# ktncktnc/diffusion-forcing-transformer

Hardware: AMD Instinct MI355X
Metric: denoised latent frames/sec, DFoT RE10K 8f & 200f rollout @1/2/4/8 GPU (higher is better)
Workload: dtype bf16

## Files before the change

### diffusion-forcing-transformer_amd/backbone.py

```python
from __future__ import annotations

import ctypes as C
import math
from typing import Dict, Optional, Sequence, Tuple

import torch
from torch import nn

from . import capi, ops


def _get(cfg, key, default=None):
    if isinstance(cfg, dict):
        return cfg.get(key, default)
    return getattr(cfg, key, default) if not hasattr(cfg, "get") else cfg.get(key, default)


class _Node(nn.Module):
    """Anonymous container so that dotted reference key names map onto a module tree."""


class UViT3DPose(nn.Module):
    def __init__(self, cfg, x_shape: Sequence[int], max_tokens: int, external_cond_dim: int = 0,
                 external_cond_type: str = "action", external_cond_num_classes: Optional[int] = None,
                 use_causal_mask: bool = False, **kwargs):
        super().__init__()
        block_types = list(_get(cfg, "block_types", ["ResBlock", "ResBlock", "TransformerBlock", "TransformerBlock"]))
        if block_types != ["ResBlock", "ResBlock", "TransformerBlock", "TransformerBlock"]:
            raise ValueError(f"unsupported block_types {block_types}")
        if _get(cfg, "pos_emb_type", "rope") != "rope":
            raise ValueError("only pos_emb_type='rope' is supported")
        if not _get(cfg, "use_fourier_noise_embedding", True):
            raise ValueError("only the Fourier noise-level embedding (continuous diffusion) is supported")
        cond = _get(cfg, "conditioning", None)
        cond_dim = _get(cond, "dim", None) if cond is not None else None
        self.cfg = cfg
        self.x_shape = tuple(x_shape)
        self.max_tokens = self.temporal_length = int(max_tokens)
        self.external_cond_dim = int(cond_dim or 180)
        self.use_causal_mask = use_causal_mask
        c = capi.UViTConfig()
        c.channels[:] = list(_get(cfg, "channels"))
        c.emb_channels = int(_get(cfg, "emb_channels"))
        c.num_updown_blocks[:] = list(_get(cfg, "num_updown_blocks"))
        c.num_mid_blocks = int(_get(cfg, "num_mid_blocks"))
        c.num_heads = int(_get(cfg, "num_heads"))
        c.in_channels = int(self.x_shape[0])
        c.resolution = int(self.x_shape[-1])
        c.max_tokens = self.max_tokens
        c.cond_dim = self.external_cond_dim
        c.noise_dim = 256
        c.rope_theta = 10000.0
        c.eps = 1e-6
        if int(_get(cfg, "patch_size", 2)) != 2:
            raise ValueError("only patch_size=2 is supported")
        self._ccfg = c
        self._handle = C.c_void_p()
        capi.check(capi.lib.dfot_uvit_create(C.byref(c), C.byref(self._handle)))
        self._names = []
        self._persistent_buffers = {"noise_level_pos_embedding.timesteps.freqs",
                                    "noise_level_pos_embedding.timesteps.phases"}
        shape = (C.c_int64 * 4)()
        ndim = C.c_int()
        for i in range(capi.lib.dfot_uvit_num_params(self._handle)):
            name = capi.lib.dfot_uvit_param_name(self._handle, i).decode()
            capi.check(capi.lib.dfot_uvit_param_shape(self._handle, i, shape, C.byref(ndim)))
            self._register(name, tuple(shape[k] for k in range(ndim.value)))
            self._names.append(name)
        self._synced: Optional[Tuple] = None
        self._reserved = 0
        self._op_key: Optional[int] = None
        self._cond_key = None
        self._cond_refs = None
        self._cond_gen = None
        self._cond_flag = None
        self.cond_cache_stats = {"builds": 0, "identity_hits": 0, "content_hits": 0}
        self._train_names = None
        self._trainer = None
        self._trainer_sig = None
        self.live_frames = None
        self.fresh_frames = None
        self._fresh_key = None
        self._train_stamp = 0
        self._dropout_generator: Optional[torch.Generator] = None

    def _register(self, name: str, shape: Tuple[int, ...]) -> None:
        *path, leaf = name.split(".")
        node: nn.Module = self
        for part in path:
            if part not in node._modules:
                node.add_module(part, _Node())
            node = node._modules[part]
        t = torch.zeros(shape, dtype=torch.float32)
        if name in self._persistent_buffers:
            node.register_buffer(leaf, t, persistent=True)
        else:
            node.register_parameter(leaf, nn.Parameter(t))

    def _tensors(self) -> Dict[str, torch.Tensor]:
        sd = dict(self.named_parameters())
        sd.update(dict(self.named_buffers()))
        return sd

    def reset_parameters(self, seed: int = 0) -> None:
        g = torch.Generator().manual_seed(seed)
        with torch.no_grad():
            for name, t in self._tensors().items():
                leaf = name.rsplit(".", 1)[-1]
                if leaf == "freqs":
                    t.copy_(2 * math.pi * torch.randn(t.shape, generator=g))
                elif leaf == "phases":
                    t.copy_(2 * math.pi * torch.rand(t.shape, generator=g))
                elif any(s in name for s in (".attn_out.", ".mlp_out.2.", ".out_rest.1.", "project_output")):
                    t.zero_()
                elif leaf == "bias":
                    t.zero_()
                elif t.ndim == 1:
                    t.fill_(1.0)
                else:
                    fan_in = math.prod(t.shape[1:])
                    bound = 1.0 / math.sqrt(fan_in)
                    t.copy_((torch.rand(t.shape, generator=g) * 2 - 1) * bound)

    def _signature(self) -> Tuple:
        return tuple((t.data_ptr(), t._version) for t in self._tensors().values())

    def sync_weights(self, force: bool = False) -> None:
        sig = self._signature()
        if not force and sig == self._synced:
            return
        tensors = self._tensors()
        s = capi.stream_ptr()
        for name in self._names:
            t = tensors[name]
            if not t.is_cuda:
                raise RuntimeError(f"parameter {name} is on {t.device}; move the module to the GPU first")
            src = t.detach().to(torch.float32).contiguous()
            shape = (C.c_int64 * src.ndim)(*src.shape)
            capi.check(capi.lib.dfot_uvit_load_weight(self._handle, name.encode(), capi.ptr(src), shape, src.ndim, s))
        capi.check(capi.lib.dfot_uvit_finalize(self._handle, s))
        self._synced = sig
        self.reserve_generation = getattr(self, "reserve_generation", 0) + 1

    def set_option(self, key: str, value: int) -> None:
        self.reserve_generation = getattr(self, "reserve_generation", 0) + 1
        capi.check(capi.lib.dfot_uvit_set_option(self._handle, key.encode(), int(value)))

    def query(self, key: str) -> float:
        self.sync_weights()
        val = C.c_double()
        capi.check(capi.lib.dfot_uvit_query(self._handle, key.encode(), C.byref(val)))
        return float(val.value)

    def attn_timing(self):
        tot, n = C.c_double(), C.c_int64()
        capi.check(capi.lib.dfot_uvit_attn_timing(self._handle, C.byref(tot), C.byref(n)))
        return tot.value, n.value

    def init_random(self, seed: int = 0, zero_init_scale: float = 0.3) -> None:
        g = torch.Generator().manual_seed(seed)
        with torch.no_grad():
            for name, t in self._tensors().items():
                leaf = name.rsplit(".", 1)[-1]
                if leaf == "freqs":
                    v = 2 * math.pi * torch.randn(t.shape, generator=g)
                elif leaf == "phases":
                    v = 2 * math.pi * torch.rand(t.shape, generator=g)
                elif leaf == "bias":
                    v = 0.02 * torch.randn(t.shape, generator=g)
                elif t.ndim == 1:
                    v = 1.0 + 0.1 * torch.randn(t.shape, generator=g)
                else:
                    fan_in = t.shape[0] if name.startswith("project_output") else math.prod(t.shape[1:])
                    v = torch.randn(t.shape, generator=g) / math.sqrt(fan_in)
                    if any(s in name for s in (".attn_out.", ".mlp_out.2.", ".out_rest.1.", "project_output")):
                        v = v * zero_init_scale
                t.copy_(v.to(t.device))

    def reserve(self, batch: int) -> None:
        if batch > self._reserved:
            torch.cuda.synchronize()
            capi.check(capi.lib.dfot_uvit_reserve(self._handle, int(batch)))
            self._reserved = batch
            self.reserve_generation = getattr(self, "reserve_generation", 0) + 1
            self._cond_key = None

    def forward(self, x: torch.Tensor, noise_levels: torch.Tensor, external_cond: Optional[torch.Tensor] = None,
                external_cond_mask: Optional[torch.Tensor] = None) -> torch.Tensor:
        assert external_cond is not None, "External condition (camera pose) is required for U-ViT3DPose model."
        if self._op_key is None:
            self._op_key = ops.register_model(self)
        if torch.is_grad_enabled() and (x.requires_grad or any(p.requires_grad for p in self.parameters())):
            if self._train_names is None:
                self._train_names = [n for n, _ in self.named_parameters()]
            params = [p for _, p in self.named_parameters()]
            return torch.ops.dfot.uvit3d_pose_forward_train(x, noise_levels, external_cond, external_cond_mask, params, self._op_key)
        return torch.ops.dfot.uvit3d_pose_forward(x, noise_levels, external_cond, external_cond_mask, self._op_key)

    def _train_engine(self, params):
        from . import uvit_train
        sig = tuple((t.data_ptr(), t._version) for t in params) + tuple((b.data_ptr(), b._version) for _, b in self.named_buffers())
        if self._trainer is None:
            cfg = dict(channels=list(self._ccfg.channels), emb_channels=int(self._ccfg.emb_channels), patch_size=2,
                       block_types=["ResBlock", "ResBlock", "TransformerBlock", "TransformerBlock"],
                       num_updown_blocks=list(self._ccfg.num_updown_blocks), num_mid_blocks=int(self._ccfg.num_mid_blocks),
                       num_heads=int(self._ccfg.num_heads), in_channels=int(self._ccfg.in_channels), resolution=int(self._ccfg.resolution),
                       max_tokens=self.max_tokens, cond_dim=self.external_cond_dim, noise_dim=int(self._ccfg.noise_dim),
                       eps=float(self._ccfg.eps), rope_theta=float(self._ccfg.rope_theta),
                       block_dropouts=list(_get(self.cfg, "block_dropouts", [0.0] * 4) or [0.0] * 4))
            sd = {n: t for n, t in zip(self._train_names, params)}
            sd.update(dict(self.named_buffers()))
            ordered = {n: sd[n] for n in self._names}
            self._trainer = uvit_train.UViT3DPoseTrainer(ordered, cfg)
            self._trainer_sig = sig
        elif sig != self._trainer_sig:
            with torch.no_grad():
                for n, t in zip(self._train_names, params):
                    self._trainer.p[n].copy_(t)
                for n, b in self.named_buffers():
                    self._trainer.p[n].copy_(b)
            self._trainer.sync()
            self._trainer_sig = sig
        return self._trainer

    def _train_forward_impl(self, x, noise_levels, external_cond, external_cond_mask, params):
        assert x.shape[1] == self.temporal_length, (
            f"Temporal length of U-ViT is set to {self.temporal_length}, but input has temporal length {x.shape[1]}.")
        dev = params[0].device
        if dev.type != "cuda":
            raise RuntimeError(f"the backbone's parameters are on {dev}; move the module to the GPU first (there is no CPU path)")
        capi.require_device(dev, x=x, noise_levels=noise_levels, external_cond=external_cond, external_cond_mask=external_cond_mask)
        eng = self._train_engine(params)
        drop = external_cond_mask
        pdrop = float(_get(self.cfg, "external_cond_dropout", 0.0) or 0.0)
        if drop is None and self.training and pdrop > 0:
            drop = torch.rand(x.shape[0], device=dev) < pdrop
        eng.dropout_generator = self._dropout_generator if self.training else None
        self._train_stamp += 1
        with torch.no_grad():
            return eng.forward(x, noise_levels, external_cond, drop).to(x.dtype)

    def _train_backward_impl(self, grad_out, params, stamp=None, want_dx=False):
        eng = self._trainer
        if eng is None:
            raise RuntimeError("backward without a training forward")
        if stamp is not None and stamp != self._train_stamp:
            raise RuntimeError(
                f"UViT3DPose: backward of training forward #{stamp}, but forward #{self._train_stamp} has run since and overwritten the "
                "saved activations (one engine per module). Run backward after each forward (accumulate gradients as forward/backward "
                "pairs); two forwards of one module inside one loss are not supported.")
        with torch.no_grad():
            grads = eng.backward(grad_out, input_grad=want_dx)
        out = [grads[n].to(p.dtype).reshape(p.shape) if n in grads else torch.zeros_like(p) for n, p in zip(self._train_names, params)]
        if want_dx:
            out.append(eng.dx_in.to(grad_out.dtype))
        return out

    def _cond_content_equal(self, cond: torch.Tensor, mask: Optional[torch.Tensor]) -> bool:
        if self._cond_key is None or self._cond_refs is None:
            return False
        kept, kept_mask = self._cond_refs
        _, version, shape, synced, mask_key = self._cond_key
        if synced != self._synced or self._cond_gen != self.reserve_generation:
            return False
        if kept._version != version or (kept_mask is not None and kept_mask._version != mask_key[1]):
            return False
        for t in (cond, kept):
            if t.dtype != torch.float32 or not t.is_contiguous():
                return False
        if cond.device != kept.device or tuple(cond.shape) != shape:
            return False
        if (mask is None) != (kept_mask is None):
            return False
        if mask is not None and (mask.dtype != kept_mask.dtype or mask.shape != kept_mask.shape or mask.device != kept_mask.device
                                 or not mask.is_contiguous() or not kept_mask.is_contiguous()):
            return False
        if torch.cuda.is_current_stream_capturing():
            return False
        if self._cond_flag is None or self._cond_flag.device != cond.device:
            self._cond_flag = torch.zeros(1, dtype=torch.int32, device=cond.device)
        flag = self._cond_flag
        flag.zero_()
        s = capi.stream_ptr()
        capi.check(capi.lib.dfot_op_equal_bits(capi.ptr(kept), capi.ptr(cond), cond.numel() * cond.element_size(), capi.ptr(flag), s))
        if mask is not None:
            capi.check(capi.lib.dfot_op_equal_bits(capi.ptr(kept_mask), capi.ptr(mask), mask.numel() * mask.element_size(), capi.ptr(flag), s))
        return int(flag.item()) == 0

    def _forward_impl(self, x: torch.Tensor, noise_levels: torch.Tensor, external_cond: Optional[torch.Tensor] = None,
                      external_cond_mask: Optional[torch.Tensor] = None) -> torch.Tensor:
        assert x.shape[1] == self.temporal_length, (
            f"Temporal length of U-ViT is set to {self.temporal_length}, but input has temporal length {x.shape[1]}.")
        assert external_cond is not None, "External condition (camera pose) is required for U-ViT3DPose model."
        b = x.shape[0]
        if tuple(x.shape[2:]) != self.x_shape:
            raise ValueError(f"x has frame shape {tuple(x.shape[2:])}, expected {self.x_shape}")
        if tuple(external_cond.shape) != (b, self.temporal_length, self.external_cond_dim, *self.x_shape[1:]):
            raise ValueError(f"external_cond has shape {tuple(external_cond.shape)}")
        if external_cond_mask is not None:
            assert external_cond_mask.ndim == 1, "embedding mask should be of shape (B,)"
        if tuple(noise_levels.shape) != (b, self.temporal_length):
            raise ValueError(f"noise_levels has shape {tuple(noise_levels.shape)}, expected {(b, self.temporal_length)}")
        dev = next(self.parameters()).device
        if dev.type != "cuda":
            raise RuntimeError(f"the backbone's parameters are on {dev}; move the module to the GPU first (there is no CPU path)")
        capi.require_device(dev, x=x, noise_levels=noise_levels, external_cond=external_cond, external_cond_mask=external_cond_mask)
        self.sync_weights()
        self.reserve(b)
        xf = x.detach().to(torch.float32).contiguous()
        kf = noise_levels.detach().to(torch.float32).contiguous()
        key = (external_cond.data_ptr(), external_cond._version, tuple(external_cond.shape), self._synced,
               None if external_cond_mask is None else (external_cond_mask.data_ptr(), external_cond_mask._version))
        if key == self._cond_key:
            self.cond_cache_stats["identity_hits"] += 1
        else:
            if self._cond_content_equal(external_cond, external_cond_mask):
                self.cond_cache_stats["content_hits"] += 1
            else:
                cf = external_cond.detach().to(torch.float32).contiguous()
                mf = None if external_cond_mask is None else external_cond_mask.to(torch.uint8).contiguous()
                capi.check(capi.lib.dfot_uvit_set_conditions(self._handle, capi.ptr(cf, torch.float32, "external_cond"),
                                                             capi.ptr(mf, torch.uint8, "external_cond_mask"), b, capi.stream_ptr()))
                self.cond_cache_stats["builds"] += 1
            self._cond_key = key
            self._cond_refs = (external_cond, external_cond_mask)
            self._cond_gen = self.reserve_generation
        out = torch.empty_like(xf)
        live = self.live_frames
        if live is not None:
            if tuple(live.shape) != (b, self.temporal_length) or live.dtype != torch.uint8 or not live.is_contiguous():
                raise ValueError(f"live_frames must be a contiguous uint8 tensor of shape {(b, self.temporal_length)}")
            capi.require_device(dev, live_frames=live)
        fresh = self.fresh_frames
        if fresh is not None:
            if tuple(fresh.shape) != (b, self.temporal_length) or fresh.dtype != torch.uint8 or not fresh.is_contiguous():
                raise ValueError(f"fresh_frames must be a contiguous uint8 tensor of shape {(b, self.temporal_length)}")
            capi.require_device(dev, fresh_frames=fresh)
            if key != self._fresh_key:
                fresh = None
        capi.check(capi.lib.dfot_uvit_forward_cached_masks(self._handle, capi.ptr(xf, torch.float32, "x"),
                                                           capi.ptr(kf, torch.float32, "noise_levels"), capi.ptr(out), b,
                                                           capi.ptr(live, torch.uint8, "live_frames"),
                                                           capi.ptr(fresh, torch.uint8, "fresh_frames"), capi.stream_ptr()))
        self._fresh_key = key
        return out.to(x.dtype)

    def read_tap(self, name: str, channels: int, level: int, batch: int) -> torch.Tensor:
        r = self.x_shape[-1] // 2 // (2 ** level)
        out = torch.empty(batch * self.temporal_length, channels, r, r, device="cuda", dtype=torch.float32)
        capi.check(capi.lib.dfot_uvit_read_tap(self._handle, name.encode(), capi.ptr(out), out.numel(), capi.stream_ptr()))
        return out

    def __del__(self):
        try:
            if getattr(self, "_handle", None) and self._handle.value:
                capi.lib.dfot_uvit_destroy(self._handle)
                self._handle = C.c_void_p()
        except Exception:
            pass
```

### diffusion-forcing-transformer_amd/capi.py

```python
from __future__ import annotations

import ctypes as C
import os

_HERE = os.path.dirname(os.path.abspath(__file__))
LIB_PATH = os.environ.get("DFOT_LIB", os.path.join(_HERE, "libdfot_hip.so"))

OK, ERR_ARG, ERR_SHAPE, ERR_HIP, ERR_STATE, ERR_NAME = range(6)


class DfotError(RuntimeError):
    def __init__(self, code: int, message: str):
        super().__init__(f"libdfot_hip error {code}: {message}")
        self.code = code


class UViTConfig(C.Structure):
    _fields_ = [
        ("channels", C.c_int32 * 4), ("emb_channels", C.c_int32), ("num_updown_blocks", C.c_int32 * 3),
        ("num_mid_blocks", C.c_int32), ("num_heads", C.c_int32), ("in_channels", C.c_int32),
        ("resolution", C.c_int32), ("max_tokens", C.c_int32), ("cond_dim", C.c_int32), ("noise_dim", C.c_int32),
        ("rope_theta", C.c_float), ("eps", C.c_float),
    ]


class DiTConfig(C.Structure):
    _fields_ = [
        ("hidden_size", C.c_int32), ("depth", C.c_int32), ("num_heads", C.c_int32), ("patch_size", C.c_int32),
        ("in_channels", C.c_int32), ("height", C.c_int32), ("width", C.c_int32), ("max_tokens", C.c_int32),
        ("mlp_hidden", C.c_int32), ("noise_dim", C.c_int32), ("timesteps", C.c_int32),
        ("rope_theta", C.c_float), ("eps", C.c_float),
        ("variant", C.c_int32), ("embed_col_dim", C.c_int32), ("num_col_heads", C.c_int32), ("num_row_heads", C.c_int32),
        ("temporal_mlp_hidden", C.c_int32), ("use_bias", C.c_int32),
        ("cond_type", C.c_int32), ("cond_dim", C.c_int32), ("num_classes", C.c_int32), ("cond_dropout", C.c_int32),
        ("use_temporal_rope", C.c_int32),
    ]


COND_NONE, COND_ACTION, COND_LABEL = 0, 1, 2


_P, _I, _L, _F = C.c_void_p, C.c_int, C.c_int64, C.c_float
_I32 = C.c_int32


class GemmDesc(C.Structure):
    _fields_ = [
        ("amode", _I32), ("epi", _I32), ("variant", _I32),
        ("A", _P), ("lda", _L), ("W", _P), ("ldw", _L),
        ("M", _I32), ("N", _I32), ("K", _I32), ("H", _I32), ("Wd", _I32), ("Cin", _I32),
        ("live", _P), ("bias", _P), ("bias_rows", _I32),
        ("out_f32", _P), ("out_bf16", _P), ("ldo", _L),
        ("resid", _P), ("resid_bf", _P),
        ("gate", _P), ("gate_index", _P), ("ldg", _L), ("gate_rows", _I32),
        ("act", _I32), ("pre_act", _P), ("raw", _P), ("ldraw", _L), ("tr_rows", _I32),
        ("gn_part", _P), ("gn_rows_per_bt", _I32), ("gn_cpg", _I32),
        ("out2", _P), ("ldo2", _L), ("split", _I32),
        ("q", _P), ("k", _P), ("v", _P),
        ("qw", _P), ("kw", _P), ("rope_cs", _P),
        ("heads", _I32), ("d", _I32), ("ntok", _I32), ("qscale", _F), ("dstride", _I32), ("eps", _F),
        ("ksplit", _I32), ("slice_stride", _L),
    ]


SIGNATURES = {
    "dfot_last_error": (C.c_char_p, []),
    "dfot_version": (_I, []),
    "dfot_uvit_create": (_I, [C.POINTER(UViTConfig), C.POINTER(_P)]),
    "dfot_uvit_destroy": (_I, [_P]),
    "dfot_uvit_num_params": (_I, [_P]),
    "dfot_uvit_param_name": (C.c_char_p, [_P, _I]),
    "dfot_uvit_param_shape": (_I, [_P, _I, C.POINTER(_L), C.POINTER(_I)]),
    "dfot_uvit_load_weight": (_I, [_P, C.c_char_p, _P, C.POINTER(_L), _I, _P]),
    "dfot_uvit_finalize": (_I, [_P, _P]),
    "dfot_uvit_reserve": (_I, [_P, _I]),
    "dfot_uvit_workspace_bytes": (C.c_size_t, [_P]),
    "dfot_uvit_set_option": (_I, [_P, C.c_char_p, _I]),
    "dfot_uvit_query": (_I, [_P, C.c_char_p, C.POINTER(C.c_double)]),
    "dfot_uvit_attn_timing": (_I, [_P, C.POINTER(C.c_double), C.POINTER(_L)]),
    "dfot_uvit_forward": (_I, [_P, _P, _P, _P, _P, _P, _I, _P]),
    "dfot_uvit_set_conditions": (_I, [_P, _P, _P, _I, _P]),
    "dfot_uvit_forward_cached": (_I, [_P, _P, _P, _P, _I, _P]),
    "dfot_uvit_forward_cached_live": (_I, [_P, _P, _P, _P, _I, _P, _P]),
    "dfot_uvit_forward_cached_masks": (_I, [_P, _P, _P, _P, _I, _P, _P, _P]),
    "dfot_uvit_read_tap": (_I, [_P, C.c_char_p, _P, C.c_size_t, _P]),
    "dfot_dit_create": (_I, [C.POINTER(DiTConfig), C.POINTER(_P)]),
    "dfot_dit_destroy": (_I, [_P]),
    "dfot_dit_num_params": (_I, [_P]),
    "dfot_dit_param_name": (C.c_char_p, [_P, _I]),
    "dfot_dit_param_shape": (_I, [_P, _I, C.POINTER(_L), C.POINTER(_I)]),
    "dfot_dit_load_weight": (_I, [_P, C.c_char_p, _P, C.POINTER(_L), _I, _P]),
    "dfot_dit_finalize": (_I, [_P, _P]),
    "dfot_dit_reserve": (_I, [_P, _I]),
    "dfot_dit_workspace_bytes": (C.c_size_t, [_P]),
    "dfot_dit_set_option": (_I, [_P, C.c_char_p, _I]),
    "dfot_dit_attn_timing": (_I, [_P, C.POINTER(C.c_double), C.POINTER(_L)]),
    "dfot_dit_forward": (_I, [_P, _P, _P, _P, _I, _I, _P]),
    "dfot_dit_forward_cond": (_I, [_P, _P, _P, _P, _P, _P, _P, _I, _I, _P]),
    "dfot_dit_read_tap": (_I, [_P, C.c_char_p, _P, C.c_size_t, _P]),
    "dfot_dit_train_create": (_I, [C.POINTER(DiTConfig), C.POINTER(_P)]),
    "dfot_dit_train_destroy": (_I, [_P]),
    "dfot_dit_train_num_params": (_I, [_P]),
    "dfot_dit_train_param_name": (C.c_char_p, [_P, _I]),
    "dfot_dit_train_param_shape": (_I, [_P, _I, C.POINTER(_L), C.POINTER(_I)]),
    "dfot_dit_train_param_offset": (_L, [_P, _I]),
    "dfot_dit_train_total_numel": (_L, [_P]),
    "dfot_dit_train_workspace_bytes": (C.c_size_t, [_P]),
    "dfot_dit_train_attach": (_I, [_P, _P, _P]),
    "dfot_dit_train_reserve": (_I, [_P, _I]),
    "dfot_dit_train_sync_weights": (_I, [_P, _P]),
    "dfot_dit_train_forward": (_I, [_P, _P, _P, _P, _I, _I, _P]),
    "dfot_dit_train_forward_cond": (_I, [_P, _P, _P, _P, _P, _P, _P, _I, _I, _P]),
    "dfot_dit_train_input_grad": (_I, [_P, _P, _P]),
    "dfot_dit_train_backward": (_I, [_P, _P, _P]),
    "dfot_vloss_grad": (_I, [_P] * 7 + [_I, _I, _L, _I, _P]),
    "dfot_sumsq": (_I, [_P, _L, _P, _P]),
    "dfot_adamw_step": (_I, [_P, _P, _P, _P, _L, _F, _F, _F, _F, _F, _I, _P, _F, _P, _F, _P]),
    "dfot_ray_encode": (_I, [_P, _P, _I, _I, _I, _P]),
    "dfot_ray_encode_normalized": (_I, [_P, _P, _I, _I, _I, _P]),
    "dfot_hg_prepare": (_I, [_P, _P, _P, _P, _P, _I, _I, _I, _L, _P]),
    "dfot_ddim_compose": (_I, [_P] * 11 + [_I, _I, _I, _L, _P]),
    "dfot_ddim_compose_tokw": (_I, [_P] * 11 + [_I, _I, _I, _L, _P]),
    "dfot_ddim_noise": (_I, [_P] * 5 + [_I, _I, _I, _L, _I, _P]),
    "dfot_vpred_loss": (_I, [_P] * 9 + [_I, _I, _L, _P]),
    "dfot_vpred_loss_scratch_floats": (_L, [_I, _I, _L]),
    "dfot_vspace_loss": (_I, [_P] * 9 + [_I, _I, _L, _P]),
    "dfot_op_gemm": (_I, [_P, _I, _P, _P, _P, _I, _I, _I, _I, _P]),
    "dfot_op_conv3x3": (_I, [_P, _P, _P, _P, _I, _I, _I, _I, _I, _I, _P]),
    "dfot_op_gemm_ex": (_I, [C.POINTER(GemmDesc), _P]),
    "dfot_op_gemm_desc_bytes": (_L, []),
    "dfot_op_attention": (_I, [_P, _P, _P, _P, _I, _I, _I, _I, _I, _I, _P]),
    "dfot_op_attention_padded": (_I, [_P, _P, _P, _P, _I, _I, _I, _I, _I, _P]),
    "dfot_op_attention_temporal": (_I, [_P, _P, _P, _P, _I, _I, _I, _I, _I, _I, _P]),
    "dfot_op_matrix_attention_rope": (_I, [_P, _P, _P, _I, _I, _I, _I, _I, _I, _F, _P]),
    "dfot_op_matrix_attention": (_I, [_P, _P, _I, _I, _I, _I, _I, _I, _F, _P]),
    "dfot_op_attention_bwd": (_I, [_P, _P, _P, _P, _P, _I, _P, _P, _P, _I, _I, _I, _I, _P]),
    "dfot_op_conv3x3_bwd": (_I, [_P, _P, _P, _P, _P, _P, _I, _I, _I, _I, _I, _P]),
    "dfot_op_conv3x3_bwd2": (_I, [_P, _P, _P, _P, _P, _P, _P, _I, _I, _I, _I, _I, _P]),
    "dfot_op_gn_silu_bwd": (_I, [_P, _P, _P, _P, _P, _F, _P, _P, _P, _P, _I, _I, _I, _P]),
    "dfot_op_rms_film_bwd": (_I, [_P, _P, _P, _P, _F, _P, _P, _P, _L, _I, _I, _P]),
    "dfot_op_rms_film_bwd_res": (_I, [_P, _P, _P, _P, _F, _P, _P, _P, _P, _P, _L, _I, _P]),
    "dfot_op_qknorm_rope_bwd": (_I, [_P, _I, _P, _P, _P, _P, _P, _P, _F, _P, _I, _P, _P, _L, _I, _I, _I, _P]),
    "dfot_op_wgrad_nt": (_I, [_P, _I, _P, _I, _P, _I, _I, _L, _I, _P]),
    "dfot_op_gemm_bf16": (_I, [_P, _I, _P, _P, _P, _I, _I, _I, _I, _P]),
    "dfot_op_gemm_f32": (_I, [_P, _I, _P, _P, _P, _P, _I, _I, _I, _I, _P]),
    "dfot_op_transpose_bf16": (_I, [_P, _P, _I, _I, _P]),
    "dfot_op_colsum_bf16": (_I, [_P, _I, _P, _L, _I, _P]),
    "dfot_op_rms_film_fwd": (_I, [_P, _P, _P, _F, _P, _L, _I, _P]),
    "dfot_op_qknorm_rope_fwd": (_I, [_P, _I, _P, _P, _P, _F, _F, _P, _P, _P, _L, _I, _I, _I, _P]),
    "dfot_op_fused_proj_train": (_I, [_P, _I, _P, _P, _P, _P, _P, _F, _F, _P, _P, _P, _P, _P, _I, _I, _L, _I, _I, _I, _P]),
    "dfot_op_silu_cols": (_I, [_P, _I, _I, _P, _I, _I, _P, _I, _I, _L, _I, _P]),
    "dfot_op_attention_fwd_lse": (_I, [_P, _P, _P, _P, _I, _P, _I, _I, _I, _I, _P]),
    "dfot_op_attention_fwd_lse_bounded": (_I, [_P, _P, _P, _P, _I, _P, _I, _I, _I, _I, C.c_float, _P, C.c_size_t, _P]),
    "dfot_op_attention_scratch_bytes": (C.c_size_t, [_I, _I, _I, _I]),
    "dfot_op_attention_bwd_lse": (_I, [_P, _P, _P, _P, _P, _I, _P, _P, _P, _P, _P, _I, _I, _I, _I, _P]),
    "dfot_op_gn_silu_fwd": (_I, [_P, _P, _P, _P, _F, _P, _P, _I, _I, _I, _P]),
    "dfot_op_gn_silu_bwd5": (_I, [_P, _P, _P, _P, _P, _P, _P, _P, _P, _P, _L, _P, _P, _I, _I, _I, _P]),
    "dfot_op_gn_silu_fwd2": (_I, [_P, _P, _P, _P, _L, _F, _P, _P, _I, _I, _I, _P]),
    "dfot_op_gn_silu_bwd6": (_I, [_P, _P, _P, _P, _P, _P, _L, _P, _P, _P, _P, _L, _P, _P, _I, _I, _I, _P]),
    "dfot_op_gemm_bf16_frame_bias": (_I, [_P, _I, _P, _P, _I, _P, _I, _I, _I, _I, _P]),
    "dfot_op_split_bf16": (_I, [_P, _P, _P, _L, _P]),
    "dfot_op_frame_sums_bf16": (_I, [_P, _L, _P, _I, _I, _I, _P]),
    "dfot_op_sgemm": (_I, [_P, _L, _L, _P, _L, _L, _P, _L, _I, _I, _I, _I, _P]),
    "dfot_op_pack_conv3": (_I, [_P, _P, _I, _I, _I, _P]),
    "dfot_op_conv3x3_f32": (_I, [_P, _P, _P, _P, _P, _I, _I, _I, _I, _I, _P]),
    "dfot_op_pool2_bf16": (_I, [_P, _P, _I, _I, _I, _I, _P]),
    "dfot_op_pool2_bwd": (_I, [_P, _P, _I, _I, _I, _I, _P]),
    "dfot_op_sub_bf16": (_I, [_P, _P, _P, _L, _P]),
    "dfot_op_upsample_add": (_I, [_P, _P, _P, _I, _I, _I, _I, _P]),
    "dfot_op_upsample_bwd": (_I, [_P, _P, _I, _I, _I, _I, _P]),
    "dfot_op_axpy": (_I, [_P, _P, _F, _L, _P]),
    "dfot_op_mul_cols": (_I, [_P, _I, _I, _P, _L, _I, _P]),
    "dfot_op_emb_pyramid": (_I, [_P, _P, _P, _P, _I, _I, _I, _P]),
    "dfot_op_cond_repack": (_I, [_P, _P, _I, _I, _I, _I, _P]),
    "dfot_op_embed_input": (_I, [_P, _P, _P, _P, _I, _I, _I, _I, _P]),
    "dfot_op_embed_input_wgrad": (_I, [_P, _P, _P, _P, _I, _I, _I, _I, _I, _P]),
    "dfot_op_embed_input_dgrad": (_I, [_P, _P, _P, _I, _I, _I, _I, _I, _P]),
    "dfot_op_project_output": (_I, [_P, _P, _P, _P, _I, _I, _I, _I, _P]),
    "dfot_op_outgrad_gather": (_I, [_P, _P, _I, _I, _I, _I, _P]),
    "dfot_op_groupnorm_scratch_floats": (_L, [_I, _I]),
    "dfot_op_groupnorm": (_I, [_P, _P, _P, _F, _P, _P, _I, _I, _I, _I, _P]),
    "dfot_op_frame_shift": (_I, [_P, _P, _I, _I, _L, _I, _P]),
    "dfot_op_upsample3d": (_I, [_P, _P, _I, _I, _I, _I, _I, _I, _P]),
    "dfot_op_softmax_rows": (_I, [_P, _P, _L, _I, _F, _P]),
    "dfot_op_conv3t_f32": (_I, [_P, _P, _P, _P, _P] + [_I] * 9 + [_P]),
    "dfot_op_vae_pixels": (_I, [_P, _L, _L, _L, _L, _L, _F, _F, _P, _I, _I, _I, _I, _P]),
    "dfot_op_vae_posterior": (_I, [_P, _I, _P, _P, _P, _P, _P, _P, _P, _I, _I, _I, _I, _P]),
    "dfot_op_f32_to_bf16": (_I, [_P, _P, _L, _P]),
    "dfot_op_bf16_to_f32": (_I, [_P, _P, _L, _P]),
    "dfot_op_equal_bits": (_I, [_P, _P, _L, _P, _P]),
}


def _load() -> C.CDLL:
    import torch
    if not os.path.exists(LIB_PATH):
        raise ImportError(
            f"{LIB_PATH} is missing: the HIP extension has not been built. There is no CPU fallback; "
            "run `python -c 'import __graft_entry__ as g; g.build()'` (needs hipcc).")
    lib = C.CDLL(LIB_PATH)
    for name, (res, args) in SIGNATURES.items():
        fn = getattr(lib, name)
        fn.restype, fn.argtypes = res, args
    return lib


lib = _load()


def check(code: int) -> None:
    if code != OK:
        raise DfotError(code, (lib.dfot_last_error() or b"").decode())


def ptr(t, dtype=None, name: str = "tensor") -> C.c_void_p:
    if t is None:
        return C.c_void_p(0)
    if not t.is_cuda:
        raise ValueError(f"{name} is on {t.device}: libdfot_hip takes GPU memory only (there is no CPU path)")
    if not t.is_contiguous():
        raise ValueError(f"{name} with shape {tuple(t.shape)} and strides {tuple(t.stride())} is not contiguous")
    if dtype is not None and t.dtype != dtype:
        raise ValueError(f"{name} has dtype {t.dtype}, expected {dtype}")
    return C.c_void_p(t.data_ptr())


def ptr_rows(t, dtype=None, name: str = "tensor") -> C.c_void_p:
    if t is None:
        return C.c_void_p(0)
    if not t.is_cuda:
        raise ValueError(f"{name} is on {t.device}: libdfot_hip takes GPU memory only (there is no CPU path)")
    if t.dim() != 2 or t.stride(1) != 1 or t.stride(0) < t.shape[1]:
        raise ValueError(f"{name} with shape {tuple(t.shape)} and strides {tuple(t.stride())} is not a row-strided matrix")
    if dtype is not None and t.dtype != dtype:
        raise ValueError(f"{name} has dtype {t.dtype}, expected {dtype}")
    return C.c_void_p(t.data_ptr())

# ... 11 lines not shown
```

### diffusion-forcing-transformer_amd/csrc/kernels.h

```cpp
#pragma once
#include "common.h"

namespace dfot {

int launch_noise_emb(const float* k, const float* freqs, const float* phases, const float* w1, const float* b1,
                     const float* w2, const float* b2, float* hidden, float* out, int bt, int ndim, int e, hipStream_t s);
int launch_embed_input(const float* x, const float* w, const float* b, float* out, int bt, int res, int cin, int c0,
                       hipStream_t s);
int launch_cond_repack(const float* cond, bf16* a, int bt, int res, int cdim, int kpad, hipStream_t s);
int launch_emb_pyramid(const bf16* emb0, bf16* emb1, bf16* emb2, bf16* emb3, int bt, int r0, int e, hipStream_t s);
int launch_project_output(const float* x0, const float* w, const float* b, float* out, int bt, int res, int c0, int cout,
                          hipStream_t s, const uint8_t* live = nullptr);
int launch_gn_partial_f32(const float* x, float* partial, int bt, int pixels, int c, hipStream_t s);
int launch_gn_partial_bf16(const bf16* x, float* partial, int bt, int pixels, int c, hipStream_t s);
int launch_gn_finalize(const float* partial, float* stats, int bt, int nblk, int pixels, int c, float eps, hipStream_t s);
int gn_partial_blocks(int pixels);
int launch_gn_apply_silu(const float* x, const float* stats, const float* gamma, const float* beta, bf16* out, int bt,
                         int pixels, int c, hipStream_t s, const uint8_t* live = nullptr);
struct FilmChunk {
  const bf16* w;
  const float* b;
  long out_off;
  int rows;
};
int launch_film_vec(const FilmChunk* table, int chunks, const float* nemb, float* sv, int bt, int e, hipStream_t s);
int launch_gn_film_silu(const bf16* h, const float* stats, const float* gamma, const float* beta, const bf16* fcache,
                        const float* sv, const uint8_t* cond_mask, bf16* out, int bt, int pixels, int c, int tokens,
                        hipStream_t s, const uint8_t* live = nullptr);
struct RmsPending {
  void* x;
  const float* bias;
  const float* s0;
  const float* s1;
  const float* s2;
};
int launch_rms_film(const float* x, const float* w, const bf16* fcache, const float* sv, const uint8_t* cond_mask, bf16* out,
                    long m, int c, int rows_per_bt, int tokens, float eps, hipStream_t s, const RmsPending* pend = nullptr);
int launch_rms_film_bf16(const bf16* x, const float* w, const bf16* fcache, const float* sv, const uint8_t* cond_mask, bf16* out,
                         long m, int c, int rows_per_bt, int tokens, float eps, hipStream_t s, const RmsPending* pend = nullptr);

int launch_pool2_bf16(const float* x, bf16* out, int bt, int h, int w, int c, hipStream_t s);
int launch_pool2_bf16_bf16in(const bf16* x, bf16* out, int bt, int h, int w, int c, hipStream_t s);
int launch_sub_bf16_bf16in(const bf16* a, const float* b, bf16* out, long n, hipStream_t s, const uint8_t* live = nullptr, long frame_elems = 0);
int launch_upsample_add_bf16(const float* t, const bf16* skip, bf16* out, int bt, int h, int w, int c, hipStream_t s, const uint8_t* live = nullptr);
int launch_gn_apply_silu_bf16in(const bf16* x, const float* stats, const float* gamma, const float* beta, bf16* out, int bt, int pixels, int c,
                                hipStream_t s, const uint8_t* live = nullptr);
int launch_embed_input_bf16(const float* x, const float* w, const float* b, bf16* out, int bt, int res, int cin, int c0, hipStream_t s);
int launch_project_output_bf16(const bf16* x0, const float* w, const float* b, float* out, int bt, int res, int c0, int cout, hipStream_t s,
                               const uint8_t* live = nullptr);
int launch_sub_bf16(const float* a, const float* b, bf16* out, long n, hipStream_t s, const uint8_t* live = nullptr, long frame_elems = 0);
int launch_upsample_add(const float* t, const float* skip, float* out, int bt, int h, int w, int c, hipStream_t s, const uint8_t* live = nullptr);
int launch_ray_encode(const float* poses, float* out, int b, int t, int res, int normalized, hipStream_t s);
int launch_hg_prepare(const float* x, const float* noise, const float* qa, const float* qb, float* x_in, int batch,
                      int nfe, int tokens, long f, hipStream_t s);
int launch_ddim_compose(const float* x, const float* x_in, const float* v, const float* sa, const float* s1,
                        const float* an, const float* cn, const float* keep, const float* weight, const uint8_t* gen,
                        float* x_next, int batch, int nfe, int tokens, long f, bool weight_per_token, hipStream_t s);
int launch_ddim_noise(const float* noise, const float* sigma, const float* weight, const uint8_t* gen, float* x_next, int batch, int nfe,
                      int tokens, long f, bool weight_per_token, hipStream_t s);
int vloss_chunks(long f);
int launch_vloss(const float* x, const float* noise, const float* v, const float* a, const float* sg, const float* w,
                 float* x_pred, float* partial, float* loss, int bt, long f, bool vspace, hipStream_t s);
int launch_wgrad_nt(const bf16* a, long lda, const bf16* b, long ldb, float* out, int m, int n, long rows, int slices, hipStream_t s, int img_h = 0,
                    int img_w = 0, int sdy = 0, int sdx = 0, int all_taps = 0);
struct WgradPlan {
  int form, slices;
};
WgradPlan wgrad_plan(int m, int n, long rows, long max_slices);
int launch_wgrad_conv_taps(const bf16* dy, const bf16* x, float* out, int co, int ci, long pix, int slices, int img_h, int img_w, hipStream_t s);
int wgrad_conv_tiles(int co, int ci, int* target);
int launch_wgrad_nt_plan(const bf16* a, long lda, const bf16* b, long ldb, float* out, int m, int n, long rows, WgradPlan plan, hipStream_t s);
int launch_vloss_grad(const float* x, const float* noise, const float* v, const float* a, const float* sg, const float* coef, float* dv,
                      int bt, long f, bool vspace, hipStream_t s);
int launch_sumsq(const float* x, long n, float* out, hipStream_t s);
int launch_adamw(float* p, const float* g, float* m, float* v, long n, float lr, float b1, float b2, float eps, float wd, int step,
                 const float* sumsq, float max_norm, float* ema, float ema_decay, hipStream_t s);
int launch_f32_to_bf16(const float* src, bf16* dst, long n, hipStream_t s);
int launch_bf16_to_f32(const bf16* src, float* dst, long n, hipStream_t s);
int launch_equal_bits(const void* a, const void* b, long bytes, int* differs, hipStream_t s);
int launch_pack_rows(const float* src, bf16* dst, const int* map, int rows, int k, int kpad, long ldd, int col0,
                     hipStream_t s);
int launch_pack_conv3(const float* src, bf16* dst, int co, int ci, hipStream_t s);
int launch_gather_f32(const float* src, float* dst, const int* map, int n, hipStream_t s);
int launch_nhwc_to_nchw(const float* src, float* dst, int bt, int p, int c, hipStream_t s);
int launch_bf16_nhwc_to_nchw(const bf16* src, float* dst, int bt, int p, int c, hipStream_t s);

struct AttnScratch {
  float* p = nullptr;
  size_t bytes = 0;
};
int launch_attention(const bf16* q, const bf16* k, const bf16* v, bf16* o, long ldo, int batch, int heads, int n, int d,
                     int variant, hipStream_t stream, AttnScratch* scratch = nullptr);
int launch_attention_v3(const bf16* q, const bf16* k, const bf16* v, bf16* o, long ldo, int batch, int heads, int n, bool nomax,
                        hipStream_t stream, AttnScratch* scratch = nullptr);
bool attention_v5_applies(int n, int d, float score_bound);
int launch_attention_v5(const bf16* q, const bf16* k, const bf16* v, bf16* o, long ldo, int batch, int heads, int n, hipStream_t stream,
                        AttnScratch* scratch = nullptr, float* lse = nullptr);
bool attention_ks_applies(int batch, int heads, int n, int d);
size_t attention_ks_scratch_bytes(int batch, int heads, int n, int d);
int launch_attention_ks(const bf16* q, const bf16* k, const bf16* v, bf16* o, long ldo, int batch, int heads, int n, hipStream_t stream,
                        AttnScratch* scratch = nullptr);
int attention_dstride(int d);
int launch_attention_padded(const bf16* q, const bf16* k, const bf16* v, bf16* o, long ldo, int batch, int heads, int n, int d,
                            hipStream_t stream, float* lse = nullptr);
int launch_attention_temporal(const bf16* q, const bf16* k, const bf16* v, bf16* o, long ldo, int batch, int tokens, int patches, int heads,
                              int d, hipStream_t s);
int launch_matrix_attn_rope(const bf16* z, bf16* o, const float* rope_cs, int batch, int L, int E, int h, int cc, int rr, float scale,
                            hipStream_t s);
struct AttnSplit {
  int tiles, full, rem, nsplit;
  int slots;
};
AttnSplit attn_plan_split(int batch, int heads, int n, int qrows, int wgs_per_cu);
size_t attn_partial_bytes(const AttnSplit& sp, int qrows, int dcols);
size_t attention_scratch_bytes(int batch, int heads, int n, int d);
int attn_partials(const AttnSplit& sp, int qrows, int dcols, float** po, float** pml, AttnScratch* scratch);
int attn_launch_merge(const AttnSplit& sp, int qrows, int dcols, const float* po, const float* pml, bf16* o, long ldo, int n, int heads,
                      hipStream_t stream, float* lse = nullptr);
int launch_attention_bwd_delta(const bf16* o, const bf16* d_o, long ldo, float* delta, int batch, int heads, int n, int d, hipStream_t s);
int launch_attention_bwd(const bf16* q, const bf16* k, const bf16* v, const bf16* d_o, long ldo, const float* l2, const float* delta,
                         bf16* dq, bf16* dk, bf16* dv, int batch, int heads, int n, int d, hipStream_t s);

}
```

### diffusion-forcing-transformer_amd/csrc/kernels.hip

```cpp
#include "kernels.h"
#include "dfot_hip.h"

namespace dfot {

typedef __attribute__((ext_vector_type(4))) float float4v;
typedef __attribute__((ext_vector_type(2))) float float2v;

__device__ __forceinline__ float wave_sum(float v) {
#pragma unroll
  for (int o = 32; o > 0; o >>= 1) v += __shfl_xor(v, o);
  return v;
}

template <bool FOURIER>
__global__ __launch_bounds__(256) void noise_mlp_kernel(const float* __restrict__ in, const float* __restrict__ freqs,
                                                        const float* __restrict__ phases, const float* __restrict__ w,
                                                        const float* __restrict__ b, float* __restrict__ out, int kdim,
                                                        int e) {
  const int lane = threadIdx.x & 63, wave = threadIdx.x >> 6;
  const int row = blockIdx.x * 4 + wave;
  const int bt = blockIdx.y;
  if (row >= e) return;
  float acc = 0.f;
  for (int i = lane; i < kdim; i += 64) {
    float f;
    if constexpr (FOURIER) {
      f = cosf(__fadd_rn(__fmul_rn(in[bt], freqs[i]), phases[i])) * 1.41421356237309515f;
    } else {
      f = in[(long)bt * kdim + i];
    }
    acc += w[(long)row * kdim + i] * f;
  }
  acc = wave_sum(acc);
  if (lane == 0) out[(long)bt * e + row] = FOURIER ? silu_f(acc + b[row]) : acc + b[row];
}

int launch_noise_emb(const float* k, const float* freqs, const float* phases, const float* w1, const float* b1,
                     const float* w2, const float* b2, float* hidden, float* out, int bt, int ndim, int e, hipStream_t s) {
  hipLaunchKernelGGL(noise_mlp_kernel<true>, dim3(cdiv(e, 4), bt), dim3(256), 0, s, k, freqs, phases, w1, b1, hidden, ndim, e);
  DFOT_CHECK_HIP(hipGetLastError());
  hipLaunchKernelGGL(noise_mlp_kernel<false>, dim3(cdiv(e, 4), bt), dim3(256), 0, s, hidden, nullptr, nullptr, w2, b2, out, e, e);
  DFOT_CHECK_HIP(hipGetLastError());
  return DFOT_OK;
}

template <typename T>
__device__ __forceinline__ void stream_ld8(const T* p, float (&v)[8]) {
  if constexpr (sizeof(T) == 4) {
    const float4v a = *reinterpret_cast<const float4v*>(p), b = *reinterpret_cast<const float4v*>(p + 4);
#pragma unroll
    for (int j = 0; j < 4; ++j) { v[j] = a[j]; v[4 + j] = b[j]; }
  } else {
    const bf16x8 a = *reinterpret_cast<const bf16x8*>(p);
#pragma unroll
    for (int j = 0; j < 8; ++j) v[j] = bf2f(a[j]);
  }
}
template <typename T>
__device__ __forceinline__ float4v stream_ld4(const T* p) {
  if constexpr (sizeof(T) == 4) {
    return *reinterpret_cast<const float4v*>(p);
  } else {
    const bf16x4 a = *reinterpret_cast<const bf16x4*>(p);
    return float4v{bf2f(a[0]), bf2f(a[1]), bf2f(a[2]), bf2f(a[3])};
  }
}
template <typename T>
__device__ __forceinline__ void stream_st8(T* p, const float (&v)[8]) {
  if constexpr (sizeof(T) == 4) {
    *reinterpret_cast<float4v*>(p) = float4v{v[0], v[1], v[2], v[3]};
    *reinterpret_cast<float4v*>(p + 4) = float4v{v[4], v[5], v[6], v[7]};
  } else {
    bf16x8 o;
#pragma unroll
    for (int j = 0; j < 8; ++j) o[j] = f2bf(v[j]);
    *reinterpret_cast<bf16x8*>(p) = o;
  }
}
template <typename T>
__device__ __forceinline__ void stream_st4(T* p, float4v v) {
  if constexpr (sizeof(T) == 4) {
    *reinterpret_cast<float4v*>(p) = v;
  } else {
    *reinterpret_cast<bf16x4*>(p) = bf16x4{f2bf(v[0]), f2bf(v[1]), f2bf(v[2]), f2bf(v[3])};
  }
}

__global__ __launch_bounds__(256) void embed_input_kernel(const float* __restrict__ x, const float* __restrict__ w,
                                                          const float* __restrict__ b, float* __restrict__ out, long total4,
                                                          int res, int cin, int c0) {
  extern __shared__ float wt[];
  const int taps = cin * 4;
  for (int i = threadIdx.x; i < taps * c0; i += blockDim.x) {
    const int c = i % c0, t = i / c0;
    wt[i] = w[(long)c * taps + t];
  }
  __syncthreads();
  const long idx = (long)blockIdx.x * blockDim.x + threadIdx.x;
  if (idx >= total4) return;
  const unsigned q = c0 / 4, r0 = res / 2, iu = (unsigned)idx;
  const int c4 = (int)(iu % q) * 4;
  const unsigned pix = iu / q;
  const int px = (int)(pix % r0), py = (int)((pix / r0) % r0);
  const long bt = pix / (r0 * r0);
  float4v acc = *reinterpret_cast<const float4v*>(b + c4);
  for (int ci = 0; ci < cin; ++ci) {
    const float* xp = x + ((bt * cin + ci) * res + 2 * py) * (long)res + 2 * px;
    const float2v top = *reinterpret_cast<const float2v*>(xp);
    const float2v bot = *reinterpret_cast<const float2v*>(xp + res);
    const float* wp = wt + (ci * 4) * c0 + c4;
    acc += *reinterpret_cast<const float4v*>(wp) * top[0] + *reinterpret_cast<const float4v*>(wp + c0) * top[1] +
           *reinterpret_cast<const float4v*>(wp + 2 * c0) * bot[0] + *reinterpret_cast<const float4v*>(wp + 3 * c0) * bot[1];
  }
  *reinterpret_cast<float4v*>(out + (long)pix * c0 + c4) = acc;
}

template <int CIN, typename TOUT>
__global__ __launch_bounds__(256) void embed_input_reg_kernel(const float* __restrict__ x, const float* __restrict__ w,
                                                              const float* __restrict__ b, TOUT* __restrict__ out, unsigned total4,
                                                              int res, int c0) {
  constexpr int TAPS = CIN * 4;
  const unsigned q = c0 / 4, r0 = res / 2;
  const unsigned nthreads = gridDim.x * 256u;
  unsigned iu = blockIdx.x * 256u + threadIdx.x;
  const int c4 = (int)(iu % q) * 4;
  float4v wt[TAPS];
#pragma unroll
  for (int t = 0; t < TAPS; ++t)
#pragma unroll
    for (int j = 0; j < 4; ++j) wt[t][j] = w[(long)(c4 + j) * TAPS + t];
  const float4v bias = *reinterpret_cast<const float4v*>(b + c4);
  for (; iu < total4; iu += nthreads) {
    const unsigned pix = iu / q;
    const int px = (int)(pix % r0), py = (int)((pix / r0) % r0);
    const long bt = pix / (r0 * r0);
    float4v acc = bias;
#pragma unroll
    for (int ci = 0; ci < CIN; ++ci) {
      const float* xp = x + ((bt * CIN + ci) * res + 2 * py) * (long)res + 2 * px;
      const float2v top = *reinterpret_cast<const float2v*>(xp);
      const float2v bot = *reinterpret_cast<const float2v*>(xp + res);
      acc += wt[ci * 4] * top[0] + wt[ci * 4 + 1] * top[1] + wt[ci * 4 + 2] * bot[0] + wt[ci * 4 + 3] * bot[1];
    }
    stream_st4(out + (long)pix * c0 + c4, acc);
  }
}

int launch_embed_input(const float* x, const float* w, const float* b, float* out, int bt, int res, int cin, int c0,
                       hipStream_t s) {
  DFOT_REQUIRE(c0 % 4 == 0 && res % 2 == 0, DFOT_ERR_SHAPE, "embed_input: channels %d / resolution %d unsupported", c0, res);
  const long total4 = (long)bt * (res / 2) * (res / 2) * (c0 / 4);
  DFOT_REQUIRE(total4 < (1L << 31), DFOT_ERR_SHAPE, "embed_input: %ld work items exceed the 32-bit index range", total4);
  if (cin == 3 && 256 % (c0 / 4) == 0) {
    const long wgs = cdiv(total4, 256);
    hipLaunchKernelGGL((embed_input_reg_kernel<3, float>), dim3((unsigned)(wgs < 4096 ? wgs : 4096)), dim3(256), 0, s, x, w, b, out, (unsigned)total4, res, c0);
    DFOT_CHECK_HIP(hipGetLastError());
    return DFOT_OK;
  }
  hipLaunchKernelGGL(embed_input_kernel, dim3(cdiv(total4, 256)), dim3(256), (size_t)cin * 4 * c0 * sizeof(float), s, x, w, b,
                     out, total4, res, cin, c0);
  DFOT_CHECK_HIP(hipGetLastError());
  return DFOT_OK;
}
int launch_embed_input_bf16(const float* x, const float* w, const float* b, bf16* out, int bt, int res, int cin, int c0, hipStream_t s) {
  DFOT_REQUIRE(c0 % 4 == 0 && res % 2 == 0 && cin == 3 && 256 % (c0 / 4) == 0, DFOT_ERR_SHAPE,
               "embed_input (bf16 stream): %d input channels / %d channels / resolution %d unsupported", cin, c0, res);
  const long total4 = (long)bt * (res / 2) * (res / 2) * (c0 / 4);
  DFOT_REQUIRE(total4 < (1L << 31), DFOT_ERR_SHAPE, "embed_input: %ld work items exceed the 32-bit index range", total4);
  const long wgs = cdiv(total4, 256);
  hipLaunchKernelGGL((embed_input_reg_kernel<3, bf16>), dim3((unsigned)(wgs < 4096 ? wgs : 4096)), dim3(256), 0, s, x, w, b, out, (unsigned)total4, res, c0);
  DFOT_CHECK_HIP(hipGetLastError());
  return DFOT_OK;
}

constexpr int RP_CC = 20;
__global__ __launch_bounds__(256) void cond_repack_kernel(const float* __restrict__ cond, bf16* __restrict__ a, int res,
                                                          int cdim, int kpad) {
  extern __shared__ __attribute__((aligned(16))) bf16 tile[];
  const int r0 = res / 2;
  constexpr int ld = RP_CC * 4 + 4;
  const int chunk = blockIdx.x, py = blockIdx.y, bt = blockIdx.z;
  const int c0 = chunk * RP_CC;
  const int xq = res / 4;
  for (int e = threadIdx.x; e < RP_CC * 2 * xq; e += blockDim.x) {
    const int x4 = e % xq;
    const int dy = (e / xq) & 1;
    const int cc = e / (2 * xq);
    const float4v v = *reinterpret_cast<const float4v*>(cond + (((long)bt * cdim + c0 + cc) * res + 2 * py + dy) * res + x4 * 4);
    typedef __attribute__((ext_vector_type(2))) __bf16 bf16x2;
    bf16x2 lo, hi;
    lo[0] = f2bf(v[0]); lo[1] = f2bf(v[1]); hi[0] = f2bf(v[2]); hi[1] = f2bf(v[3]);
// ... 235 lines not shown

__global__ __launch_bounds__(256) void gn_finalize_kernel(const float* __restrict__ partial, float* __restrict__ stats,
                                                          int nblk, float inv_count, float eps) {
  const int bt = blockIdx.x >> 2, g = (blockIdx.x & 3) * 8 + (threadIdx.x >> 5), part = threadIdx.x & 31;
  float s = 0.f, ss = 0.f;
  for (int b = part; b < nblk; b += 32) {
    const float2 v = *reinterpret_cast<const float2*>(partial + (((long)bt * nblk + b) * 32 + g) * 2);
    s += v.x;
    ss += v.y;
  }
#pragma unroll
  for (int o = 1; o < 32; o <<= 1) {
    s += __shfl_xor(s, o);
    ss += __shfl_xor(ss, o);
  }
  if (part == 0) {
    const float mean = s * inv_count;
    const float var = fmaxf(ss * inv_count - mean * mean, 0.f);
    stats[(bt * 32 + g) * 2 + 0] = mean;
    stats[(bt * 32 + g) * 2 + 1] = rsqrtf(var + eps);
  }
}

int launch_gn_finalize(const float* partial, float* stats, int bt, int nblk, int pixels, int c, float eps, hipStream_t s) {
  const float inv = 1.f / ((float)pixels * (float)(c / 32));
  hipLaunchKernelGGL(gn_finalize_kernel, dim3(bt * 4), dim3(256), 0, s, partial, stats, nblk, inv, eps);
  DFOT_CHECK_HIP(hipGetLastError());
  return DFOT_OK;
}

template <typename T>
static int launch_gn_partial_t(const T* x, float* partial, int bt, int pixels, int c, hipStream_t s) {
  DFOT_REQUIRE(c == 128 || c == 256 || c == 512 || c == 1024, DFOT_ERR_SHAPE, "group_norm: channels %d not in {128,256,512,1024}", c);
  hipLaunchKernelGGL(gn_partial_kernel<T>, dim3(gn_partial_blocks(pixels), bt), dim3(256), 0, s, x, partial, pixels, c);
  DFOT_CHECK_HIP(hipGetLastError());
  return DFOT_OK;
}
int launch_gn_partial_f32(const float* x, float* partial, int bt, int pixels, int c, hipStream_t s) {
  return launch_gn_partial_t<float>(x, partial, bt, pixels, c, s);
}
int launch_gn_partial_bf16(const bf16* x, float* partial, int bt, int pixels, int c, hipStream_t s) {
  return launch_gn_partial_t<bf16>(x, partial, bt, pixels, c, s);
}

__global__ void gn_apply_silu_kernel(const float* __restrict__ x, const float* __restrict__ stats,
                                     const float* __restrict__ gamma, const float* __restrict__ beta,
                                     bf16* __restrict__ out, long total8, int pixels, int c, const uint8_t* __restrict__ live) {
  const long idx = (long)blockIdx.x * blockDim.x + threadIdx.x;
  if (idx >= total8) return;
  const unsigned iu = (unsigned)idx, cq = (unsigned)(c / 8);
  const int c8 = (int)(iu % cq);
  const long pix = iu / cq;
  const int bt = (int)((unsigned)pix / (unsigned)pixels);
  if (live && !live[bt]) return;
  const int cpg = c / 32;
  const float* src = x + pix * c + c8 * 8;
  const float4v a = *reinterpret_cast<const float4v*>(src);
  const float4v b = *reinterpret_cast<const float4v*>(src + 4);
  float v[8] = {a[0], a[1], a[2], a[3], b[0], b[1], b[2], b[3]};
  bf16x8 o;
#pragma unroll
  for (int j = 0; j < 8; ++j) {
    const int ch = c8 * 8 + j;
    const int g = ch / cpg;
    const float mean = stats[(bt * 32 + g) * 2], rs = stats[(bt * 32 + g) * 2 + 1];
    const float y = (v[j] - mean) * rs * gamma[ch] + beta[ch];
    o[j] = f2bf(silu_f(y));
  }
  *reinterpret_cast<bf16x8*>(out + pix * c + c8 * 8) = o;
}

constexpr int GN_ROWS_IT = 8;
template <int C>
struct GnRowConsts {
  float mean[8], rsg[8], gam[8], bet[8];
  __device__ __forceinline__ void load(const float* __restrict__ stats, const float* __restrict__ gamma, const float* __restrict__ beta, int bt,
                                       int c0) {
    constexpr int CPG = C / 32;
    const float4v g0 = *reinterpret_cast<const float4v*>(gamma + c0), g1 = *reinterpret_cast<const float4v*>(gamma + c0 + 4);
    const float4v b0 = *reinterpret_cast<const float4v*>(beta + c0), b1 = *reinterpret_cast<const float4v*>(beta + c0 + 4);
    const float* st = stats + ((long)bt * 32 + c0 / CPG) * 2;
    float m0, r0, m1, r1;
    if constexpr (CPG == 4) {
      const float4v t = *reinterpret_cast<const float4v*>(st);
      m0 = t[0], r0 = t[1], m1 = t[2], r1 = t[3];
    } else {
      m0 = m1 = st[0];
      r0 = r1 = st[1];
    }
#pragma unroll
    for (int j = 0; j < 8; ++j) {
      mean[j] = j < 4 ? m0 : m1;
      rsg[j] = j < 4 ? r0 : r1;
      gam[j] = j < 4 ? g0[j] : g1[j - 4];
      bet[j] = j < 4 ? b0[j] : b1[j - 4];
    }
  }
  __device__ __forceinline__ float norm(float v, int j) const { return (v - mean[j]) * rsg[j] * gam[j] + bet[j]; }
};

template <int C, typename TIN>
__global__ __launch_bounds__(256) void gn_apply_silu_rows_kernel(const TIN* __restrict__ x, const float* __restrict__ stats,
                                                                 const float* __restrict__ gamma, const float* __restrict__ beta,
                                                                 bf16* __restrict__ out, int pixels, const uint8_t* __restrict__ live) {
  constexpr int TPP = C / 8, PPI = 256 / TPP;
  const int wg_per_bt = pixels / (PPI * GN_ROWS_IT);
  const int bt = blockIdx.x / wg_per_bt;
  if (live && !live[bt]) return;
  const int c0 = (threadIdx.x % TPP) * 8;
  GnRowConsts<C> k;
  k.load(stats, gamma, beta, bt, c0);
  long pix = (long)bt * pixels + (long)(blockIdx.x % wg_per_bt) * (PPI * GN_ROWS_IT) + threadIdx.x / TPP;
#pragma unroll 4
  for (int it = 0; it < GN_ROWS_IT; ++it, pix += PPI) {
    float v[8];
    stream_ld8(x + pix * C + c0, v);
    bf16x8 o;
#pragma unroll
    for (int j = 0; j < 8; ++j) o[j] = f2bf(silu_f(k.norm(v[j], j)));
    *reinterpret_cast<bf16x8*>(out + pix * C + c0) = o;
  }
}

int launch_gn_apply_silu_bf16in(const bf16* x, const float* stats, const float* gamma, const float* beta, bf16* out, int bt, int pixels, int c,
                                hipStream_t s, const uint8_t* live) {
  DFOT_REQUIRE((c == 128 || c == 256) && pixels % ((256 / (c / 8)) * GN_ROWS_IT) == 0, DFOT_ERR_SHAPE,
               "groupnorm apply (bf16 stream): %d channels / %d pixels per frame unsupported", c, pixels);
  const int grid = bt * (pixels / ((256 / (c / 8)) * GN_ROWS_IT));
  if (c == 128) hipLaunchKernelGGL((gn_apply_silu_rows_kernel<128, bf16>), dim3(grid), dim3(256), 0, s, x, stats, gamma, beta, out, pixels, live);
  else hipLaunchKernelGGL((gn_apply_silu_rows_kernel<256, bf16>), dim3(grid), dim3(256), 0, s, x, stats, gamma, beta, out, pixels, live);
  DFOT_CHECK_HIP(hipGetLastError());
  return DFOT_OK;
}

int launch_gn_apply_silu(const float* x, const float* stats, const float* gamma, const float* beta, bf16* out, int bt,
                         int pixels, int c, hipStream_t s, const uint8_t* live) {
  if ((c == 128 || c == 256) && pixels % ((256 / (c / 8)) * GN_ROWS_IT) == 0) {
    const int grid = bt * (pixels / ((256 / (c / 8)) * GN_ROWS_IT));
    if (c == 128) hipLaunchKernelGGL((gn_apply_silu_rows_kernel<128, float>), dim3(grid), dim3(256), 0, s, x, stats, gamma, beta, out, pixels, live);
    else hipLaunchKernelGGL((gn_apply_silu_rows_kernel<256, float>), dim3(grid), dim3(256), 0, s, x, stats, gamma, beta, out, pixels, live);
    DFOT_CHECK_HIP(hipGetLastError());
    return DFOT_OK;
  }
  const long total8 = (long)bt * pixels * (c / 8);
  DFOT_REQUIRE(total8 < (1L << 31), DFOT_ERR_SHAPE, "groupnorm apply: %ld work items exceed the 32-bit index range", total8);
  hipLaunchKernelGGL(gn_apply_silu_kernel, dim3(cdiv(total8, 256)), dim3(256), 0, s, x, stats, gamma, beta, out, total8,
                     pixels, c, live);
  DFOT_CHECK_HIP(hipGetLastError());
  return DFOT_OK;
}


__global__ __launch_bounds__(256) void film_vec_kernel(const FilmChunk* __restrict__ table, const float* __restrict__ nemb,
                                                       float* __restrict__ sv, int e, int nbt) {
  const FilmChunk ck = table[blockIdx.x >> 4];
  const int lane = threadIdx.x & 63, wave = threadIdx.x >> 6;
  const int r = (blockIdx.x & 15) * 4 + wave;
  const bf16* wr = ck.w + (long)r * e;
  float wv[2][8];
#pragma unroll
  for (int k = 0; k < 2; ++k) {
    const int i = lane * 8 + k * 512;
    if (i < e) {
      const bf16x8 t = *reinterpret_cast<const bf16x8*>(wr + i);
#pragma unroll
      for (int j = 0; j < 8; ++j) wv[k][j] = bf2f(t[j]);
    } else {
#pragma unroll
      for (int j = 0; j < 8; ++j) wv[k][j] = 0.f;
    }
  }
  const float bias = ck.b[r];
  for (int bt = 0; bt < nbt; ++bt) {
    const float* ne = nemb + (long)bt * e;
    float acc = 0.f;
#pragma unroll
    for (int k = 0; k < 2; ++k) {
      const int i = lane * 8 + k * 512;
      if (i < e) {
        const float4v a = *reinterpret_cast<const float4v*>(ne + i);
        const float4v b = *reinterpret_cast<const float4v*>(ne + i + 4);
        acc += wv[k][0] * a[0] + wv[k][1] * a[1] + wv[k][2] * a[2] + wv[k][3] * a[3] + wv[k][4] * b[0] + wv[k][5] * b[1] +
               wv[k][6] * b[2] + wv[k][7] * b[3];
      }
    }
    acc = wave_sum(acc);
    if (lane == 0) sv[ck.out_off + (long)bt * ck.rows + r] = acc + bias;
  }
}
template <int EQ>
__global__ __launch_bounds__(256, 2) void film_vec_lds_kernel(const FilmChunk* __restrict__ table, const float* __restrict__ nemb,
                                                           float* __restrict__ sv, int nbt) {
  constexpr int E = EQ * 256;
  __shared__ float4v ne[16][E / 4];
  const FilmChunk ck = table[blockIdx.x >> 1];
  const int lane = threadIdx.x & 63, wave = threadIdx.x >> 6;
  for (int bt0 = 0; bt0 < nbt; bt0 += 16) {
    __syncthreads();
    for (int i = threadIdx.x; i < 16 * (E / 4); i += 256) {
      const int f = i / (E / 4);
      float4v v = {0.f, 0.f, 0.f, 0.f};
      if (bt0 + f < nbt) v = reinterpret_cast<const float4v*>(nemb + (long)(bt0 + f) * E)[i % (E / 4)];
      ne[f][i % (E / 4)] = v;
    }
    __syncthreads();
#pragma unroll 1
    for (int pass = 0; pass < 4; ++pass) {
      const int r0 = (blockIdx.x & 1) * 32 + pass * 8 + wave * 2;
      float wv[2][EQ][4];
#pragma unroll
      for (int r = 0; r < 2; ++r)
#pragma unroll
        for (int k = 0; k < EQ; ++k) {
          const bf16x4 t = *reinterpret_cast<const bf16x4*>(ck.w + (long)(r0 + r) * E + k * 256 + lane * 4);
#pragma unroll
          for (int j = 0; j < 4; ++j) wv[r][k][j] = bf2f(t[j]);
        }
      float acc[32];
#pragma unroll
      for (int f = 0; f < 16; ++f) {
        float4v x[EQ];
#pragma unroll
        for (int k = 0; k < EQ; ++k) x[k] = ne[f][k * 64 + lane];
#pragma unroll
        for (int r = 0; r < 2; ++r) {
          float a = 0.f;
#pragma unroll
          for (int k = 0; k < EQ; ++k) a += wv[r][k][0] * x[k][0] + wv[r][k][1] * x[k][1] + wv[r][k][2] * x[k][2] + wv[r][k][3] * x[k][3];
          acc[r * 16 + f] = a;
        }
        if ((f & 3) == 3) __builtin_amdgcn_sched_barrier(0);
      }
      halve_exchange<16, 32>(acc, lane);
      halve_exchange<8, 16>(acc, lane);
      halve_exchange<4, 8>(acc, lane);
      halve_exchange<2, 4>(acc, lane);
      halve_exchange<1, 2>(acc, lane);
      const float v = acc[0] + __shfl_xor(acc[0], 1);
      const int r = r0 + (lane >> 5), f = bt0 + ((lane >> 1) & 15);
      if (f < nbt && (lane & 1) == 0) sv[ck.out_off + (long)f * ck.rows + r] = v + ck.b[r];
    }
  }
}
int launch_film_vec(const FilmChunk* table, int chunks, const float* nemb, float* sv, int bt, int e, hipStream_t s) {
  DFOT_REQUIRE(e % 8 == 0 && e <= 1024, DFOT_ERR_SHAPE, "film_vec: emb dim %d must be a multiple of 8 and <= 1024", e);
  if (e == 1024 || e == 512) {
    if (e == 1024) hipLaunchKernelGGL(film_vec_lds_kernel<4>, dim3(chunks * 2), dim3(256), 0, s, table, nemb, sv, bt);
    else hipLaunchKernelGGL(film_vec_lds_kernel<2>, dim3(chunks * 2), dim3(256), 0, s, table, nemb, sv, bt);
    DFOT_CHECK_HIP(hipGetLastError());
    return DFOT_OK;
  }
  hipLaunchKernelGGL(film_vec_kernel, dim3(chunks * 16), dim3(256), 0, s, table, nemb, sv, e, bt);
  DFOT_CHECK_HIP(hipGetLastError());
  return DFOT_OK;
}

__global__ void gn_film_silu_kernel(const bf16* __restrict__ h, const float* __restrict__ stats,
                                    const float* __restrict__ gamma, const float* __restrict__ beta,
                                    const bf16* __restrict__ fcache, const float* __restrict__ sv,
                                    const uint8_t* __restrict__ cond_mask, bf16* __restrict__ out, long total8, int pixels,
                                    int c, int tokens, const uint8_t* __restrict__ live) {
  const long idx = (long)blockIdx.x * blockDim.x + threadIdx.x;
  if (idx >= total8) return;
  const unsigned iu = (unsigned)idx, cq = (unsigned)(c / 8);
  const int c8 = (int)(iu % cq);
  const long pix = iu / cq;
  const int bt = (int)((unsigned)pix / (unsigned)pixels);
  if (live && !live[bt]) return;
  const int cpg = c / 32;
  const int c0 = c8 * 8;
  const int col = (c0 >> 5) * 64 + (c0 & 31);
  const bf16x8 hv = *reinterpret_cast<const bf16x8*>(h + pix * c + c0);
  const float* svp = sv + (long)bt * 2 * c + col;
  float sc[8], sh[8];
#pragma unroll
  for (int j = 0; j < 8; ++j) {
    sc[j] = svp[j];
    sh[j] = svp[32 + j];
  }
  const bool use_pose = !(cond_mask && cond_mask[(unsigned)bt / (unsigned)tokens]);
  if (use_pose) {
    const bf16x8 fs = *reinterpret_cast<const bf16x8*>(fcache + pix * 2 * c + col);
    const bf16x8 fh = *reinterpret_cast<const bf16x8*>(fcache + pix * 2 * c + col + 32);
#pragma unroll
    for (int j = 0; j < 8; ++j) {
      sc[j] += bf2f(fs[j]);
      sh[j] += bf2f(fh[j]);
    }
  }
  bf16x8 o;
#pragma unroll
  for (int j = 0; j < 8; ++j) {
    const int ch = c0 + j;
    const int g = ch / cpg;
    const float mean = stats[(bt * 32 + g) * 2], rs = stats[(bt * 32 + g) * 2 + 1];
    const float y = ((bf2f(hv[j]) - mean) * rs * gamma[ch] + beta[ch]) * (1.f + sc[j]) + sh[j];
    o[j] = f2bf(silu_f(y));
  }
  *reinterpret_cast<bf16x8*>(out + pix * c + c0) = o;
}
template <int C>
__global__ __launch_bounds__(256) void gn_film_silu_rows_kernel(const bf16* __restrict__ h, const float* __restrict__ stats,
                                                                const float* __restrict__ gamma, const float* __restrict__ beta,
                                                                const bf16* __restrict__ fcache, const float* __restrict__ sv,
                                                                const uint8_t* __restrict__ cond_mask, bf16* __restrict__ out, int pixels,
                                                                int tokens, const uint8_t* __restrict__ live) {
  constexpr int TPP = C / 8, PPI = 256 / TPP;
  const int wg_per_bt = pixels / (PPI * GN_ROWS_IT);
  const int bt = blockIdx.x / wg_per_bt;
  if (live && !live[bt]) return;
  const int c0 = (threadIdx.x % TPP) * 8;
  const int col = (c0 >> 5) * 64 + (c0 & 31);
  GnRowConsts<C> k;
  k.load(stats, gamma, beta, bt, c0);
  const float* svp = sv + (long)bt * 2 * C + col;
  float svs[8], svh[8];
  {
    const float4v s0 = *reinterpret_cast<const float4v*>(svp), s1 = *reinterpret_cast<const float4v*>(svp + 4);
    const float4v h0 = *reinterpret_cast<const float4v*>(svp + 32), h1 = *reinterpret_cast<const float4v*>(svp + 36);
#pragma unroll
    for (int j = 0; j < 8; ++j) {
      svs[j] = j < 4 ? s0[j] : s1[j - 4];
      svh[j] = j < 4 ? h0[j] : h1[j - 4];
    }
  }
  const bool use_pose = !(cond_mask && cond_mask[(unsigned)bt / (unsigned)tokens]);
  long pix = (long)bt * pixels + (long)(blockIdx.x % wg_per_bt) * (PPI * GN_ROWS_IT) + threadIdx.x / TPP;
  if (use_pose) {
#pragma unroll 4
    for (int it = 0; it < GN_ROWS_IT; ++it, pix += PPI) {
      const bf16x8 hv = *reinterpret_cast<const bf16x8*>(h + pix * C + c0);
      const bf16x8 fs = *reinterpret_cast<const bf16x8*>(fcache + pix * 2 * C + col);
      const bf16x8 fh = *reinterpret_cast<const bf16x8*>(fcache + pix * 2 * C + col + 32);
      bf16x8 o;
#pragma unroll
      for (int j = 0; j < 8; ++j) {
        const float sc = svs[j] + bf2f(fs[j]), sh = svh[j] + bf2f(fh[j]);
        o[j] = f2bf(silu_f(k.norm(bf2f(hv[j]), j) * (1.f + sc) + sh));
      }
      *reinterpret_cast<bf16x8*>(out + pix * C + c0) = o;
    }
  } else {
#pragma unroll 4
    for (int it = 0; it < GN_ROWS_IT; ++it, pix += PPI) {
      const bf16x8 hv = *reinterpret_cast<const bf16x8*>(h + pix * C + c0);
      bf16x8 o;
#pragma unroll
      for (int j = 0; j < 8; ++j) o[j] = f2bf(silu_f(k.norm(bf2f(hv[j]), j) * (1.f + svs[j]) + svh[j]));
      *reinterpret_cast<bf16x8*>(out + pix * C + c0) = o;
    }
  }
}

int launch_gn_film_silu(const bf16* h, const float* stats, const float* gamma, const float* beta, const bf16* fcache,
                        const float* sv, const uint8_t* cond_mask, bf16* out, int bt, int pixels, int c, int tokens,
                        hipStream_t s, const uint8_t* live) {
  if ((c == 128 || c == 256) && pixels % ((256 / (c / 8)) * GN_ROWS_IT) == 0) {
    const int grid = bt * (pixels / ((256 / (c / 8)) * GN_ROWS_IT));
    if (c == 128)
      hipLaunchKernelGGL(gn_film_silu_rows_kernel<128>, dim3(grid), dim3(256), 0, s, h, stats, gamma, beta, fcache, sv, cond_mask, out, pixels, tokens, live);
    else
      hipLaunchKernelGGL(gn_film_silu_rows_kernel<256>, dim3(grid), dim3(256), 0, s, h, stats, gamma, beta, fcache, sv, cond_mask, out, pixels, tokens, live);
    DFOT_CHECK_HIP(hipGetLastError());
    return DFOT_OK;
  }
  const long total8 = (long)bt * pixels * (c / 8);
  DFOT_REQUIRE(total8 < (1L << 31), DFOT_ERR_SHAPE, "groupnorm apply: %ld work items exceed the 32-bit index range", total8);
  hipLaunchKernelGGL(gn_film_silu_kernel, dim3(cdiv(total8, 256)), dim3(256), 0, s, h, stats, gamma, beta, fcache, sv,
                     cond_mask, out, total8, pixels, c, tokens, live);
  DFOT_CHECK_HIP(hipGetLastError());
  return DFOT_OK;
}

template <int MAXCH, bool PEND, typename TS>
__global__ __launch_bounds__(256) void rms_film_kernel(const TS* x, const float* __restrict__ w,
                                                       const bf16* __restrict__ fcache, const float* __restrict__ sv,
                                                       const uint8_t* __restrict__ cond_mask, bf16* __restrict__ out,
                                                       long m, int c, int rows_per_bt, int tokens, float eps, TS* xw,
                                                       const float* __restrict__ pbias, const float* __restrict__ p0,
                                                       const float* __restrict__ p1, const float* __restrict__ p2) {
  const long row = (long)blockIdx.x * 4 + (threadIdx.x >> 6);
  if (row >= m) return;
  const int lane = threadIdx.x & 63;
  const int nch = c / 8;
  const TS* src = x + row * c;
  float v[MAXCH][8];
  float ss = 0.f;
#pragma unroll
  for (int k = 0; k < MAXCH; ++k) {
    const int ch = lane + 64 * k;
    if (ch < nch) {
      stream_ld8(src + ch * 8, v[k]);
      if constexpr (PEND) {
        const long o = row * c + ch * 8;
#pragma unroll
        for (int hf = 0; hf < 2; ++hf) {
          float4v add = *reinterpret_cast<const float4v*>(pbias + ch * 8 + 4 * hf) + *reinterpret_cast<const float4v*>(p0 + o + 4 * hf) +
                        *reinterpret_cast<const float4v*>(p1 + o + 4 * hf);
          if (p2) add += *reinterpret_cast<const float4v*>(p2 + o + 4 * hf);
#pragma unroll
          for (int j = 0; j < 4; ++j) v[k][4 * hf + j] += add[j];
        }
        stream_st8(xw + o, v[k]);
        if constexpr (sizeof(TS) == 2) {
#pragma unroll
          for (int j = 0; j < 8; ++j) v[k][j] = bf2f(f2bf(v[k][j]));
        }
// ... 630 lines not shown
```

### diffusion-forcing-transformer_amd/csrc/uvit.hip

```cpp
#include <algorithm>
#include <cmath>
#include <cstdarg>
#include <cstdlib>
#include <cstring>
#include <functional>
#include <map>
#include <string>
#include <vector>

#include "dfot_hip.h"
#include "gemm.h"
#include "kernels.h"

namespace dfot {

static thread_local char g_err[1024] = "";
void set_error(const char* fmt, ...) {
  va_list ap;
  va_start(ap, fmt);
  vsnprintf(g_err, sizeof(g_err), fmt, ap);
  va_end(ap);
}
const char* get_error() { return g_err; }

int tuning_flag(const char* name, int dflt) {
  std::string key = std::string("DFOT_") + name;
  const char* v = getenv(key.c_str());
  return v ? atoi(v) : dflt;
}

struct ResW {
  int c = 0;
  bf16* fcache = nullptr;
  long sv_off = 0;
  bf16 *w_film = nullptr, *w1 = nullptr, *w2 = nullptr;
  float *b_film_raw = nullptr, *b_film = nullptr, *g1 = nullptr, *be1 = nullptr, *bias1 = nullptr, *g2 = nullptr,
        *be2 = nullptr, *bias2 = nullptr;
};
struct TrW {
  int c = 0;
  bf16* fcache = nullptr;
  long sv_off = 0;
  bf16 *w_film = nullptr, *w_fused = nullptr, *w_out = nullptr;
  float *b_film_raw = nullptr, *b_film = nullptr, *nw = nullptr, *b_fused = nullptr, *qw = nullptr, *kw = nullptr,
        *b_attn = nullptr, *b_mlp = nullptr, *b_out = nullptr;
  float score_bound = INFINITY;
};
struct ConvW {
  int cin = 0, cout = 0;
  bf16* w = nullptr;
  float* b = nullptr;
};

struct Param {
  std::string name;
  std::vector<int64_t> shape;
  std::function<int(const float*, hipStream_t)> load;
  bool loaded = false;
};

}

using namespace dfot;

struct dfot_uvit_s {
  dfot_uvit_config cfg{};
  int T = 0, E = 0, heads = 0, r[4] = {0, 0, 0, 0}, ch[4] = {0, 0, 0, 0};
  int kpose = 0;
  std::vector<Param> params;
  std::map<std::string, int> index;
  std::vector<void*> owned;

  float *ne_freqs = nullptr, *ne_phases = nullptr, *ne_w1 = nullptr, *ne_b1 = nullptr, *ne_w2 = nullptr, *ne_b2 = nullptr;
  bf16* pose_w = nullptr;
  float* pose_b = nullptr;
  float *ein_w = nullptr, *ein_b = nullptr, *pout_w = nullptr, *pout_b = nullptr;
  std::vector<ResW> down_res[2], up_res[2];
  std::vector<TrW> down_tr, mid_tr, up_tr;
  ConvW down_conv[3], up_conv[3];
  int* film_map[4] = {nullptr, nullptr, nullptr, nullptr};
  float* rope_cs[4] = {nullptr, nullptr, nullptr, nullptr};
  bf16* zeros = nullptr;
  bool finalized = false;

  int max_batch = 0;
  size_t ws_bytes = 0;
  std::vector<void*> ws_owned;
  float *nemb = nullptr, *nhid = nullptr, *X[4] = {nullptr, nullptr, nullptr, nullptr}, *HSA[3] = {nullptr, nullptr, nullptr}, *tmp = nullptr,
        *gn_partial = nullptr, *gn_partial2 = nullptr, *gn_stats = nullptr, *sv = nullptr;
  int gn1_nblk = 0;
  FilmChunk* film_table = nullptr;
  int film_chunks = 0;
  uint8_t* cond_mask = nullptr;
  bool have_mask = false;
  int cond_batch = 0;
  int64_t cond_builds = 0;
  bf16 *acond = nullptr, *emb[4] = {nullptr, nullptr, nullptr, nullptr}, *s1 = nullptr, *hbf = nullptr,
       *cat = nullptr, *q = nullptr, *k = nullptr, *v = nullptr;
  AttnScratch attn_scratch;
  const float* pend_part = nullptr;
  float* out_part = nullptr;
  size_t out_part_elems = 0;
  const float* pend_bias = nullptr;
  int pend_lvl = 0, pend_c = 0, pend_slices = 2;
  long pend_m = 0;
  int last_batch = 0;
  const float* xin[4] = {nullptr, nullptr, nullptr, nullptr};
  bf16* XB[4] = {nullptr, nullptr, nullptr, nullptr};
  bool xin_bf[4] = {false, false, false, false};
  int gemm_variant = GEMM_AUTO;
  int attn_variant = 2;
  bool attn_force_safe = false;
  bool time_attn = false;
  std::vector<hipEvent_t> ev_start, ev_stop;
  size_t ev_used = 0;
};

namespace dfot {

template <typename T>
static int dev_alloc(dfot_uvit_s* h, T** out, size_t count, bool workspace = false) {
  void* p = nullptr;
  const size_t bytes = count * sizeof(T);
  DFOT_CHECK_HIP(hipMalloc(&p, bytes ? bytes : 16));
  (workspace ? h->ws_owned : h->owned).push_back(p);
  if (workspace) h->ws_bytes += bytes;
  *out = reinterpret_cast<T*>(p);
  return DFOT_OK;
}

static int copy_f32(float* dst, const float* src, size_t n, hipStream_t s) {
  DFOT_CHECK_HIP(hipMemcpyAsync(dst, src, n * sizeof(float), hipMemcpyDeviceToDevice, s));
  return DFOT_OK;
}

static void add_param(dfot_uvit_s* h, const std::string& name, std::vector<int64_t> shape,
                      std::function<int(const float*, hipStream_t)> load) {
  h->index[name] = (int)h->params.size();
  h->params.push_back(Param{name, std::move(shape), std::move(load), false});
}

static int add_f32(dfot_uvit_s* h, const std::string& name, std::vector<int64_t> shape, float** dst) {
  size_t n = 1;
  for (auto d : shape) n *= (size_t)d;
  int rc = dev_alloc(h, dst, n);
  if (rc) return rc;
  float* d = *dst;
  add_param(h, name, shape, [d, n](const float* src, hipStream_t s) { return copy_f32(d, src, n, s); });
  return DFOT_OK;
}

static int add_res_block(dfot_uvit_s* h, const std::string& pre, int c, ResW* w) {
  const int e = h->E;
  w->c = c;
  int rc = 0;
  if ((rc = dev_alloc(h, &w->w_film, (size_t)2 * c * e))) return rc;
  if ((rc = dev_alloc(h, &w->b_film_raw, (size_t)2 * c))) return rc;
  if ((rc = dev_alloc(h, &w->b_film, (size_t)2 * c))) return rc;
  if ((rc = dev_alloc(h, &w->w1, (size_t)c * 9 * c))) return rc;
  if ((rc = dev_alloc(h, &w->w2, (size_t)c * 9 * c))) return rc;
  const int lvl = c == h->ch[0] ? 0 : 1;
  int* map = h->film_map[lvl];
  bf16* wf = w->w_film;
  add_param(h, pre + ".emb_layer.weight", {2 * c, e, 1, 1}, [=](const float* src, hipStream_t s) {
    return launch_pack_rows(src, wf, map, 2 * c, e, e, e, 0, s);
  });
  float *braw = w->b_film_raw, *bre = w->b_film;
  add_param(h, pre + ".emb_layer.bias", {2 * c}, [=](const float* src, hipStream_t s) {
    int r2 = copy_f32(braw, src, 2 * c, s);
    return r2 ? r2 : launch_gather_f32(braw, bre, map, 2 * c, s);
  });
  if ((rc = add_f32(h, pre + ".in_layers.0.weight", {c}, &w->g1))) return rc;
  if ((rc = add_f32(h, pre + ".in_layers.0.bias", {c}, &w->be1))) return rc;
  bf16* w1 = w->w1;
  add_param(h, pre + ".in_layers.2.weight", {c, c, 3, 3}, [=](const float* src, hipStream_t s) { return launch_pack_conv3(src, w1, c, c, s); });
  if ((rc = add_f32(h, pre + ".in_layers.2.bias", {c}, &w->bias1))) return rc;
  if ((rc = add_f32(h, pre + ".out_norm.weight", {c}, &w->g2))) return rc;
  if ((rc = add_f32(h, pre + ".out_norm.bias", {c}, &w->be2))) return rc;
  bf16* w2 = w->w2;
  add_param(h, pre + ".out_rest.1.weight", {c, c, 3, 3}, [=](const float* src, hipStream_t s) { return launch_pack_conv3(src, w2, c, c, s); });
  if ((rc = add_f32(h, pre + ".out_rest.1.bias", {c}, &w->bias2))) return rc;
  return DFOT_OK;
}

static int add_tr_block(dfot_uvit_s* h, const std::string& pre, int lvl, TrW* w) {
  const int e = h->E, c = h->ch[lvl], d = c / h->heads;
  w->c = c;
  int rc = 0;
  if ((rc = dev_alloc(h, &w->w_film, (size_t)2 * c * e))) return rc;
  if ((rc = dev_alloc(h, &w->b_film_raw, (size_t)2 * c))) return rc;
  if ((rc = dev_alloc(h, &w->b_film, (size_t)2 * c))) return rc;
  if ((rc = dev_alloc(h, &w->w_fused, (size_t)7 * c * c))) return rc;
  if ((rc = dev_alloc(h, &w->w_out, (size_t)c * 5 * c))) return rc;
  if ((rc = dev_alloc(h, &w->b_out, (size_t)c))) return rc;
  int* map = h->film_map[lvl];
  bf16* wf = w->w_film;
  add_param(h, pre + ".norm.emb_layer.weight", {2 * c, e}, [=](const float* src, hipStream_t s) {
    return launch_pack_rows(src, wf, map, 2 * c, e, e, e, 0, s);
  });
  float *braw = w->b_film_raw, *bre = w->b_film;
  add_param(h, pre + ".norm.emb_layer.bias", {2 * c}, [=](const float* src, hipStream_t s) {
    int r2 = copy_f32(braw, src, 2 * c, s);
    return r2 ? r2 : launch_gather_f32(braw, bre, map, 2 * c, s);
  });
  if ((rc = add_f32(h, pre + ".norm.norm.weight", {c}, &w->nw))) return rc;
  bf16* wfu = w->w_fused;
  add_param(h, pre + ".fused_attn_mlp_proj.weight", {7 * c, c}, [=](const float* src, hipStream_t s) {
    return launch_pack_rows(src, wfu, nullptr, 7 * c, c, c, c, 0, s);
  });
  if ((rc = add_f32(h, pre + ".fused_attn_mlp_proj.bias", {7 * c}, &w->b_fused))) return rc;
  if ((rc = add_f32(h, pre + ".q_norm.weight", {d}, &w->qw))) return rc;
  if ((rc = add_f32(h, pre + ".k_norm.weight", {d}, &w->kw))) return rc;
  bf16* wo = w->w_out;
  add_param(h, pre + ".attn_out.weight", {c, c}, [=](const float* src, hipStream_t s) {
    return launch_pack_rows(src, wo, nullptr, c, c, c, 5 * c, 0, s);
  });
  if ((rc = add_f32(h, pre + ".attn_out.bias", {c}, &w->b_attn))) return rc;
  add_param(h, pre + ".mlp_out.2.weight", {c, 4 * c}, [=](const float* src, hipStream_t s) {
    return launch_pack_rows(src, wo, nullptr, c, 4 * c, 4 * c, 5 * c, c, s);
  });
  if ((rc = add_f32(h, pre + ".mlp_out.2.bias", {c}, &w->b_mlp))) return rc;
  return DFOT_OK;
}

static int add_conv(dfot_uvit_s* h, const std::string& pre, int cin, int cout, ConvW* w) {
  w->cin = cin;
  w->cout = cout;
  int rc = 0;
  if ((rc = dev_alloc(h, &w->w, (size_t)cout * 9 * cin))) return rc;
  bf16* dst = w->w;
  add_param(h, pre + ".weight", {cout, cin, 3, 3}, [=](const float* src, hipStream_t s) { return launch_pack_conv3(src, dst, cout, cin, s); });
  return add_f32(h, pre + ".bias", {cout}, &w->b);
}

static int build(dfot_uvit_s* h) {
  const dfot_uvit_config& c = h->cfg;
  h->T = c.max_tokens;
  h->E = c.emb_channels;
  h->heads = c.num_heads;
  for (int l = 0; l < 4; ++l) {
    h->ch[l] = c.channels[l];
    h->r[l] = c.resolution / 2 / (1 << l);
  }
  h->kpose = ((c.cond_dim * 4 + 63) / 64) * 64;
  int rc = 0;
  for (int l = 0; l < 4; ++l) {
    const int cc = h->ch[l];
    std::vector<int> m(2 * cc);
    for (int n = 0; n < 2 * cc; ++n) {
      const int g = n / 64, t = n % 64;
      m[n] = t < 32 ? 32 * g + t : cc + 32 * g + (t - 32);
    }
    if ((rc = dev_alloc(h, &h->film_map[l], (size_t)2 * cc))) return rc;
    DFOT_CHECK_HIP(hipMemcpy(h->film_map[l], m.data(), m.size() * sizeof(int), hipMemcpyHostToDevice));
  }
  if ((rc = dev_alloc(h, &h->zeros, 256))) return rc;
  DFOT_CHECK_HIP(hipMemset(h->zeros, 0, 256 * sizeof(bf16)));

  const int e = h->E, nd = c.noise_dim;
  const std::string ne = "noise_level_pos_embedding.";
  if ((rc = add_f32(h, ne + "timesteps.freqs", {nd}, &h->ne_freqs))) return rc;
  if ((rc = add_f32(h, ne + "timesteps.phases", {nd}, &h->ne_phases))) return rc;
  if ((rc = add_f32(h, ne + "embedding.linear_1.weight", {e, nd}, &h->ne_w1))) return rc;
  if ((rc = add_f32(h, ne + "embedding.linear_1.bias", {e}, &h->ne_b1))) return rc;
  if ((rc = add_f32(h, ne + "embedding.linear_2.weight", {e, e}, &h->ne_w2))) return rc;
  if ((rc = add_f32(h, ne + "embedding.linear_2.bias", {e}, &h->ne_b2))) return rc;
  if ((rc = dev_alloc(h, &h->pose_w, (size_t)e * h->kpose))) return rc;
  {
    bf16* pw = h->pose_w;
    const int k = c.cond_dim * 4, kp = h->kpose;
    add_param(h, "external_cond_embedding.patch_embedder.proj.weight", {e, c.cond_dim, 2, 2},
              [=](const float* src, hipStream_t s) { return launch_pack_rows(src, pw, nullptr, e, k, kp, kp, 0, s); });
  }
  if ((rc = add_f32(h, "external_cond_embedding.patch_embedder.proj.bias", {e}, &h->pose_b))) return rc;
  if ((rc = add_f32(h, "embed_input.proj.weight", {h->ch[0], c.in_channels, 2, 2}, &h->ein_w))) return rc;
  if ((rc = add_f32(h, "embed_input.proj.bias", {h->ch[0]}, &h->ein_b))) return rc;
  if ((rc = add_f32(h, "project_output.proj.weight", {h->ch[0], c.in_channels, 2, 2}, &h->pout_w))) return rc;
  if ((rc = add_f32(h, "project_output.proj.bias", {c.in_channels}, &h->pout_b))) return rc;

  for (int l = 0; l < 3; ++l) {
    const int n = c.num_updown_blocks[l];
    const std::string pre = "down_blocks." + std::to_string(l) + ".";
    if (l < 2) {
      h->down_res[l].resize(n);
      for (int i = 0; i < n; ++i)
        if ((rc = add_res_block(h, pre + std::to_string(i), h->ch[l], &h->down_res[l][i]))) return rc;
    } else {
      h->down_tr.resize(n);
      for (int i = 0; i < n; ++i)
        if ((rc = add_tr_block(h, pre + std::to_string(i), l, &h->down_tr[i]))) return rc;
    }
    if ((rc = add_conv(h, pre + std::to_string(n) + ".conv", h->ch[l], h->ch[l + 1], &h->down_conv[l]))) return rc;
  }
  h->mid_tr.resize(c.num_mid_blocks);
  for (int i = 0; i < c.num_mid_blocks; ++i)
    if ((rc = add_tr_block(h, "mid_blocks." + std::to_string(i), 3, &h->mid_tr[i]))) return rc;
  for (int j = 0; j < 3; ++j) {
    const int l = 2 - j;
    const int n = c.num_updown_blocks[l];
    const std::string pre = "up_blocks." + std::to_string(j) + ".";
    if ((rc = add_conv(h, pre + "0.conv", h->ch[l + 1], h->ch[l], &h->up_conv[l]))) return rc;
    if (l < 2) {
      h->up_res[l].resize(n);
      for (int i = 0; i < n; ++i)
        if ((rc = add_res_block(h, pre + std::to_string(i + 1), h->ch[l], &h->up_res[l][i]))) return rc;
    } else {
      h->up_tr.resize(n);
      for (int i = 0; i < n; ++i)
        if ((rc = add_tr_block(h, pre + std::to_string(i + 1), l, &h->up_tr[i]))) return rc;
    }
  }
  return DFOT_OK;
}

static int build_rope(dfot_uvit_s* h, int lvl) {
  const int d = h->ch[lvl] / h->heads, half = d / 2;
  const int q = half / 3, rem = half % 3;
  int parts[3] = {q, q, q};
  if (rem == 1) parts[0] = q + 1;
  if (rem == 2) parts[1] = parts[2] = q + 1;
  const int rr = h->r[lvl], n = h->T * rr * rr;
  std::vector<float> cs((size_t)n * half * 2);
  for (int tok = 0; tok < n; ++tok) {
    const int pos[3] = {tok / (rr * rr), (tok / rr) % rr, tok % rr};
    int pair = 0;
    for (int ax = 0; ax < 3; ++ax) {
      const int dim = 2 * parts[ax];
      for (int j = 0; j < parts[ax]; ++j, ++pair) {
        const float inv = 1.0f / powf(h->cfg.rope_theta, (float)(2 * j) / (float)dim);
        const float ang = (float)pos[ax] * inv;
        cs[((size_t)tok * half + pair) * 2 + 0] = cosf(ang);
        cs[((size_t)tok * half + pair) * 2 + 1] = sinf(ang);
      }
    }
  }
  int rc = dev_alloc(h, &h->rope_cs[lvl], cs.size());
  if (rc) return rc;
  DFOT_CHECK_HIP(hipMemcpy(h->rope_cs[lvl], cs.data(), cs.size() * sizeof(float), hipMemcpyHostToDevice));
  return DFOT_OK;
}

__global__ void add_vec_kernel(const float* a, const float* b, float* o, int n) {
  const int i = blockIdx.x * blockDim.x + threadIdx.x;
  if (i < n) o[i] = a[i] + b[i];
}

static int run_res_block(dfot_uvit_s* h, const ResW& w, int lvl, int bt, hipStream_t s, const uint8_t* live = nullptr) {
  const int c = w.c, rr = h->r[lvl], pix = rr * rr;
  const int m = bt * pix;
  const int slots = pix / 64;
  bf16* xb = h->XB[lvl];
  int rc = 0;
  if (!h->xin_bf[lvl]) {
    if ((rc = launch_f32_to_bf16(h->xin[lvl], xb, (long)m * c, s))) return rc;
    h->xin_bf[lvl] = true;
  }
  if (h->gn1_nblk == 0) {
    if ((rc = launch_gn_partial_bf16(xb, h->gn_partial, bt, pix, c, s))) return rc;
    h->gn1_nblk = gn_partial_blocks(pix);
  }
  if ((rc = launch_gn_finalize(h->gn_partial, h->gn_stats, bt, h->gn1_nblk, pix, c, h->cfg.eps, s))) return rc;
  h->gn1_nblk = 0;
  if ((rc = launch_gn_apply_silu_bf16in(xb, h->gn_stats, w.g1, w.be1, h->s1, bt, pix, c, s, live))) return rc;
  GemmArgs g;
  g.A = h->s1; g.W = w.w1; g.M = m; g.N = c; g.K = 9 * c; g.H = rr; g.Wd = rr; g.Cin = c; g.zeros = h->zeros;
  g.bias = w.bias1; g.out_bf16 = h->hbf; g.ldo = c; g.live = live;
  g.gn_part = h->gn_partial2; g.gn_rows_per_bt = pix; g.gn_cpg = c / 32;
  if ((rc = launch_gemm(A_CONV3, E_BF16, h->gemm_variant, g, s))) return rc;
  if ((rc = launch_gn_finalize(h->gn_partial2, h->gn_stats, bt, slots, pix, c, h->cfg.eps, s))) return rc;
  if ((rc = launch_gn_film_silu(h->hbf, h->gn_stats, w.g2, w.be2, w.fcache, h->sv + w.sv_off,
                                h->have_mask ? h->cond_mask : nullptr, h->s1, bt, pix, c, h->T, s, live)))
    return rc;
  GemmArgs o;
  o.A = h->s1; o.W = w.w2; o.M = m; o.N = c; o.K = 9 * c; o.H = rr; o.Wd = rr; o.Cin = c; o.zeros = h->zeros;
  o.bias = w.bias2; o.out_bf16 = xb; o.ldo = c; o.live = live;
  o.resid_bf = xb;
  o.gn_part = h->gn_partial; o.gn_rows_per_bt = pix; o.gn_cpg = c / 32;
  if ((rc = launch_gemm(A_CONV3, E_BF16, h->gemm_variant, o, s))) return rc;
  h->xin_bf[lvl] = true;
  h->gn1_nblk = slots;
  return DFOT_OK;
}

__global__ void out_reduce_kernel(bf16* x, const float* __restrict__ bias, const float* __restrict__ s0, const float* __restrict__ s1,
                                  const float* __restrict__ s2, long total4, int cq) {
  typedef __attribute__((ext_vector_type(4))) float f4;
  const long i = (long)blockIdx.x * blockDim.x + threadIdx.x;
  if (i >= total4) return;
  f4 b = reinterpret_cast<const f4*>(bias)[i % cq] + reinterpret_cast<const f4*>(s0)[i] + reinterpret_cast<const f4*>(s1)[i];
  if (s2) b += reinterpret_cast<const f4*>(s2)[i];
  const bf16x4 xv = reinterpret_cast<const bf16x4*>(x)[i];
  reinterpret_cast<bf16x4*>(x)[i] = bf16x4{f2bf(bf2f(xv[0]) + b[0]), f2bf(bf2f(xv[1]) + b[1]), f2bf(bf2f(xv[2]) + b[2]), f2bf(bf2f(xv[3]) + b[3])};
}
__global__ void add_f32_into_bf16_kernel(bf16* x, const float* __restrict__ y, long total4) {
  typedef __attribute__((ext_vector_type(4))) float f4;
  const long i = (long)blockIdx.x * blockDim.x + threadIdx.x;
  if (i >= total4) return;
  const f4 b = reinterpret_cast<const f4*>(y)[i];
  const bf16x4 xv = reinterpret_cast<const bf16x4*>(x)[i];
  reinterpret_cast<bf16x4*>(x)[i] = bf16x4{f2bf(bf2f(xv[0]) + b[0]), f2bf(bf2f(xv[1]) + b[1]), f2bf(bf2f(xv[2]) + b[2]), f2bf(bf2f(xv[3]) + b[3])};
}

static void swap_out_part(dfot_uvit_s* h) { h->pend_part = h->out_part; }

static int flush_pending(dfot_uvit_s* h, hipStream_t s) {
  if (!h->pend_bias) return DFOT_OK;
  const long total4 = h->pend_m * h->pend_c / 4;
  hipLaunchKernelGGL(out_reduce_kernel, dim3(cdiv(total4, 256)), dim3(256), 0, s, h->XB[h->pend_lvl], h->pend_bias, h->pend_part,
                     h->pend_part + h->pend_m * h->pend_c, h->pend_slices == 3 ? h->pend_part + 2 * h->pend_m * h->pend_c : nullptr, total4,
                     h->pend_c / 4);
  h->pend_bias = nullptr;
  DFOT_CHECK_HIP(hipGetLastError());
  return DFOT_OK;
}

static int run_tr_block(dfot_uvit_s* h, const TrW& w, int lvl, int batch, hipStream_t s) {
  const int c = w.c, rr = h->r[lvl], n = h->T * rr * rr, d = c / h->heads;
  const int m = batch * n;
  bf16* xb = h->XB[lvl];
  int rc = 0;
  if (h->pend_bias && (h->pend_lvl != lvl || h->pend_m != m || h->pend_c != c) && (rc = flush_pending(h, s))) return rc;
  if (!h->xin_bf[lvl]) {
    if ((rc = launch_f32_to_bf16(h->xin[lvl], xb, (long)m * c, s))) return rc;
    h->xin_bf[lvl] = true;
  }
  RmsPending pend{xb, h->pend_bias, h->pend_part, h->pend_part + (long)m * c, h->pend_slices == 3 ? h->pend_part + 2L * m * c : nullptr};
  if ((rc = launch_rms_film_bf16(xb, w.nw, w.fcache, h->sv + w.sv_off, h->have_mask ? h->cond_mask : nullptr, h->s1, m, c, rr * rr, h->T,
                                 h->cfg.eps, s, h->pend_bias ? &pend : nullptr)))
    return rc;
  h->pend_bias = nullptr;
  GemmArgs p;
  p.A = h->s1; p.lda = c; p.W = w.w_fused; p.M = m; p.N = 7 * c; p.K = c; p.bias = w.b_fused;
  p.out2 = h->cat + c; p.ldo2 = 5 * c; p.split = 3 * c;
  p.q = h->q; p.k = h->k; p.v = h->v; p.qw = w.qw; p.kw = w.kw; p.rope_cs = h->rope_cs[lvl]; p.heads = h->heads; p.d = d;
  p.ntok = n; p.qscale = 1.4426950408889634f / sqrtf((float)d); p.eps = h->cfg.eps;
  if ((rc = launch_gemm(A_DENSE, E_QKV, h->gemm_variant, p, s))) return rc;
  const bool timed = h->time_attn && lvl == 2 && h->ev_used < h->ev_start.size();
  if (timed) DFOT_CHECK_HIP(hipEventRecord(h->ev_start[h->ev_used], s));
  int av = h->attn_variant;
  if (av == 2 && d == 64 && n % 256 == 0) av = (attention_v5_applies(n, d, w.score_bound) && !h->attn_force_safe) ? 14 : 5;
  if ((rc = launch_attention(h->q, h->k, h->v, h->cat, 5 * c, batch, h->heads, n, d, av, s, &h->attn_scratch))) return rc;
  if (timed) DFOT_CHECK_HIP(hipEventRecord(h->ev_stop[h->ev_used++], s));
  GemmArgs o;
  o.A = h->cat; o.lda = 5 * c; o.W = w.w_out; o.M = m; o.N = c; o.K = 5 * c; o.bias = w.b_out; o.ldo = c;
  if (h->gemm_variant == GEMM_AUTO && h->out_part && (size_t)2 * m * c <= h->out_part_elems && m % 256 == 0 && c % 144 == 0 &&
      (long)(m / 256) * (c / 144) * 2 <= 256 && (5 * c / 64) >= 8) {
    GemmArgs p2 = o;
    p2.bias = nullptr; p2.out_f32 = h->out_part; p2.ksplit = 2; p2.slice_stride = (long)m * c;
    if ((rc = launch_gemm(A_DENSE, E_F32, GEMM_DMA3_256x144, p2, s))) return rc;
    h->pend_bias = w.b_out;
    h->pend_lvl = lvl; h->pend_m = m; h->pend_c = c; h->pend_slices = 2;
    swap_out_part(h);
    return DFOT_OK;
  }
  if (h->gemm_variant == GEMM_AUTO && c % 144 == 0 && m % 256 == 0 && (long)(m / 256) * ((c + 191) / 192) < 256 &&
      (long)(m / 256) * (c / 144) >= 200 && (long)(m / 256) * (c / 144) <= 256) {
    o.out_bf16 = xb;
    o.resid_bf = xb;
    return launch_gemm(A_DENSE, E_BF16, GEMM_DMA3_256x144, o, s);
  }
  o.out_f32 = h->X[lvl];
  if ((rc = launch_gemm(A_DENSE, E_F32, h->gemm_variant, o, s))) return rc;
  hipLaunchKernelGGL(add_f32_into_bf16_kernel, dim3(cdiv((long)m * c / 4, 256)), dim3(256), 0, s, xb, h->X[lvl], (long)m * c / 4);
  DFOT_CHECK_HIP(hipGetLastError());
  return DFOT_OK;
}


__global__ void slab_reduce_kernel(float* __restrict__ out, const float* __restrict__ bias, const float* __restrict__ slabs, int nslab, long stride4,
                                   long total4, int cq, const uint8_t* __restrict__ live, unsigned img4) {
  typedef __attribute__((ext_vector_type(4))) float f4;
  const long i = (long)blockIdx.x * blockDim.x + threadIdx.x;
  if (i >= total4) return;
  if (live && !live[(unsigned)i / img4]) return;
  f4 v = reinterpret_cast<const f4*>(bias)[i % cq];
  for (int sl = 0; sl < nslab; ++sl) v += reinterpret_cast<const f4*>(slabs)[sl * stride4 + i];
  reinterpret_cast<f4*>(out)[i] = v;
}

static int conv_between_levels(dfot_uvit_s* h, GemmArgs g, hipStream_t s) {
  const long px = (long)g.H * g.Wd;
  if (h->gemm_variant == GEMM_AUTO && h->out_part && !g.gn_part && g.M % 256 == 0 && px % 256 == 0 && (g.N % 144 == 0 || g.N == 256) &&
      (long)g.M * g.N < (1L << 31)) {
    const int bn = g.N % 144 == 0 ? 144 : 256;
    const int variant = bn == 144 ? GEMM_DMA3_256x144 : GEMM_DMA_256x256;
    const int tiles = (g.M / 256) * (g.N / bn);
    int ks = 1;
    while (tiles * ks * 2 <= 256 && g.K / 64 / (ks * 2) >= 16) ks *= 2;
    if (tiles * ks >= 192 && tiles * ks <= 256) {
      if (ks == 1) return launch_gemm(A_CONV3, E_F32, variant, g, s);
      if ((size_t)ks * g.M * g.N <= h->out_part_elems) {
        GemmArgs p = g;
        float* out = g.out_f32;
        const float* bias = g.bias;
        p.bias = nullptr; p.resid = nullptr; p.out_f32 = h->out_part; p.ksplit = ks; p.slice_stride = (long)g.M * g.N;
        int rc = launch_gemm(A_CONV3, E_F32, variant, p, s);
        if (rc) return rc;
        const long total4 = (long)g.M * g.N / 4;
        hipLaunchKernelGGL(slab_reduce_kernel, dim3(cdiv(total4, 256)), dim3(256), 0, s, out, bias, h->out_part, ks, total4, total4, g.N / 4, g.live,
                           (unsigned)(px * g.N / 4));
        DFOT_CHECK_HIP(hipGetLastError());
        return DFOT_OK;
      }
    }
  }
  return launch_gemm(A_CONV3, E_F32, h->gemm_variant, g, s);
}

static int run_down(dfot_uvit_s* h, int l, int bt, hipStream_t s, const uint8_t* live = nullptr) {
  const int rr = h->r[l], cin = h->ch[l], cout = h->ch[l + 1];
  int rc = 0;
  if ((rc = h->xin_bf[l] ? launch_pool2_bf16_bf16in(h->XB[l], h->s1, bt, rr, rr, cin, s) : launch_pool2_bf16(h->xin[l], h->s1, bt, rr, rr, cin, s)))
    return rc;
  GemmArgs g;
  g.A = h->s1; g.W = h->down_conv[l].w; g.M = bt * (rr / 2) * (rr / 2); g.N = cout; g.K = 9 * cin; g.H = rr / 2; g.Wd = rr / 2;
  g.Cin = cin; g.zeros = h->zeros; g.bias = h->down_conv[l].b; g.out_f32 = h->HSA[l]; g.ldo = cout;
  g.live = live;
  const bool next_is_res = l + 1 < 2;
  if (next_is_res) {
    g.gn_part = h->gn_partial; g.gn_rows_per_bt = (rr / 2) * (rr / 2); g.gn_cpg = cout / 32;
  }
  if ((rc = conv_between_levels(h, g, s))) return rc;
  h->gn1_nblk = next_is_res ? g.gn_rows_per_bt / 64 : 0;
  h->xin[l + 1] = h->HSA[l];
  h->xin_bf[l + 1] = false;
  return DFOT_OK;
}

static int run_up(dfot_uvit_s* h, int l, int bt, hipStream_t s, const uint8_t* live = nullptr) {
  const int rr = h->r[l + 1], cin = h->ch[l + 1], cout = h->ch[l];
  const long n_in = (long)bt * rr * rr * cin;
  int rc = 0;
  if ((rc = h->xin_bf[l + 1] ? launch_sub_bf16_bf16in(h->XB[l + 1], h->HSA[l], h->s1, n_in, s, live, (long)rr * rr * cin)
                             : launch_sub_bf16(h->xin[l + 1], h->HSA[l], h->s1, n_in, s, live, (long)rr * rr * cin)))
    return rc;
  GemmArgs g;
  g.A = h->s1; g.W = h->up_conv[l].w; g.M = bt * rr * rr; g.N = cout; g.K = 9 * cin; g.H = rr; g.Wd = rr; g.Cin = cin;
  g.zeros = h->zeros; g.bias = h->up_conv[l].b; g.out_f32 = h->tmp; g.ldo = cout;
  if (live && (rr * rr) % 256 == 0 && h->gemm_variant == GEMM_AUTO) g.live = live;
  if ((rc = conv_between_levels(h, g, s))) return rc;
  h->gn1_nblk = 0;
  if (!h->xin_bf[l]) {
    set_error("run_up: level %d stream is not in its bf16 buffer", l);
    return DFOT_ERR_STATE;
  }
  return launch_upsample_add_bf16(h->tmp, h->XB[l], h->XB[l], bt, rr, rr, cout, s, live);
}

}

extern "C" {

const char* dfot_last_error(void) { return get_error(); }
int dfot_version(void) { return 1; }

int dfot_uvit_create(const dfot_uvit_config* cfg, dfot_uvit_t* out) {
  DFOT_REQUIRE(cfg && out, DFOT_ERR_ARG, "dfot_uvit_create: null argument");
  DFOT_REQUIRE(cfg->resolution % 16 == 0 && cfg->resolution >= 32, DFOT_ERR_SHAPE, "resolution %d must be a multiple of 16", cfg->resolution);
  DFOT_REQUIRE(cfg->emb_channels % 64 == 0, DFOT_ERR_SHAPE, "emb_channels %d must be a multiple of 64", cfg->emb_channels);
  DFOT_REQUIRE(cfg->in_channels <= 3 && cfg->cond_dim % 20 == 0, DFOT_ERR_SHAPE, "in_channels %d / cond_dim %d unsupported", cfg->in_channels, cfg->cond_dim);
  for (int l = 0; l < 4; ++l)
    DFOT_REQUIRE(cfg->channels[l] % 64 == 0, DFOT_ERR_SHAPE, "channels[%d]=%d must be a multiple of 64", l, cfg->channels[l]);
  DFOT_REQUIRE(cfg->channels[0] % 128 == 0 && cfg->channels[1] % 128 == 0, DFOT_ERR_SHAPE, "ResBlock channels must be multiples of 128");
  for (int l = 2; l < 4; ++l) {
    const int d = cfg->channels[l] / cfg->num_heads;
    DFOT_REQUIRE(d * cfg->num_heads == cfg->channels[l] && (d == 64 || d == 128), DFOT_ERR_SHAPE,
                 "level %d head dim %d must be 64 or 128", l, d);
  }
  const int r3 = cfg->resolution / 16;
  DFOT_REQUIRE((cfg->max_tokens * r3 * r3) % 128 == 0, DFOT_ERR_SHAPE, "tokens at the coarsest level (%d) must be a multiple of 128", cfg->max_tokens * r3 * r3);
  auto* h = new dfot_uvit_s();
  h->cfg = *cfg;
  int rc = build(h);
  if (rc) {
    dfot_uvit_destroy(h);
    return rc;
  }
  *out = h;
  return DFOT_OK;
}

int dfot_uvit_destroy(dfot_uvit_t h) {
  if (!h) return DFOT_OK;
  for (void* p : h->owned) (void)hipFree(p);
  for (void* p : h->ws_owned) (void)hipFree(p);
  for (hipEvent_t e : h->ev_start) (void)hipEventDestroy(e);
  for (hipEvent_t e : h->ev_stop) (void)hipEventDestroy(e);
  delete h;
  return DFOT_OK;
}

int dfot_uvit_num_params(dfot_uvit_t h) { return h ? (int)h->params.size() : 0; }
const char* dfot_uvit_param_name(dfot_uvit_t h, int i) {
  return (h && i >= 0 && i < (int)h->params.size()) ? h->params[i].name.c_str() : nullptr;
}
int dfot_uvit_param_shape(dfot_uvit_t h, int i, int64_t shape[4], int* ndim) {
  DFOT_REQUIRE(h && shape && ndim && i >= 0 && i < (int)h->params.size(), DFOT_ERR_ARG, "param_shape: bad argument");
  *ndim = (int)h->params[i].shape.size();
  for (int k = 0; k < *ndim; ++k) shape[k] = h->params[i].shape[k];
  return DFOT_OK;
}

int dfot_uvit_load_weight(dfot_uvit_t h, const char* name, const float* data, const int64_t* shape, int ndim, void* stream) {
  DFOT_REQUIRE(h && name && data && shape, DFOT_ERR_ARG, "load_weight: null argument");
  auto it = h->index.find(name);
  DFOT_REQUIRE(it != h->index.end(), DFOT_ERR_NAME, "load_weight: unexpected key '%s'", name);
  Param& p = h->params[it->second];
  bool same = (int)p.shape.size() == ndim;
  for (int k = 0; same && k < ndim; ++k) same = p.shape[k] == shape[k];
  DFOT_REQUIRE(same, DFOT_ERR_SHAPE, "load_weight: size mismatch for '%s'", name);
  int rc = p.load(data, (hipStream_t)stream);
  if (rc) return rc;
  p.loaded = true;
  h->finalized = false;
  return DFOT_OK;
}

int dfot_uvit_finalize(dfot_uvit_t h, void* stream) {
  DFOT_REQUIRE(h, DFOT_ERR_ARG, "finalize: null handle");
  for (const Param& p : h->params) DFOT_REQUIRE(p.loaded, DFOT_ERR_STATE, "finalize: missing key '%s'", p.name.c_str());
  hipStream_t s = (hipStream_t)stream;
  auto fuse = [&](std::vector<TrW>& v) -> int {
    for (TrW& w : v) {
      hipLaunchKernelGGL(add_vec_kernel, dim3(cdiv(w.c, 256)), dim3(256), 0, s, w.b_attn, w.b_mlp, w.b_out, w.c);
      DFOT_CHECK_HIP(hipGetLastError());
    }
    return DFOT_OK;
  };
  int rc = 0;
  if ((rc = fuse(h->down_tr)) || (rc = fuse(h->mid_tr)) || (rc = fuse(h->up_tr))) return rc;
  for (int l = 2; l < 4; ++l)
    if (!h->rope_cs[l] && (rc = build_rope(h, l))) return rc;
  DFOT_CHECK_HIP(hipStreamSynchronize(s));
  auto bound = [&](std::vector<TrW>& v) -> int {
    std::vector<float> qk;
    for (TrW& w : v) {
      const int d = w.c / h->heads;
      qk.resize(2 * d);
      DFOT_CHECK_HIP(hipMemcpy(qk.data(), w.qw, d * sizeof(float), hipMemcpyDeviceToHost));
      DFOT_CHECK_HIP(hipMemcpy(qk.data() + d, w.kw, d * sizeof(float), hipMemcpyDeviceToHost));
      float mqk = 0.f;
      for (int i = 0; i + 1 < d; i += 2)
        mqk = fmaxf(mqk, fmaxf(fabsf(qk[i]), fabsf(qk[i + 1])) * fmaxf(fabsf(qk[d + i]), fabsf(qk[d + i + 1])));
      w.score_bound = sqrtf((float)d) * mqk * 1.4426950408889634f;
      if (!(w.score_bound == w.score_bound)) w.score_bound = INFINITY;
    }
    return DFOT_OK;
  };
  if ((rc = bound(h->down_tr)) || (rc = bound(h->mid_tr)) || (rc = bound(h->up_tr))) return rc;
  h->finalized = true;
  return DFOT_OK;
}

int dfot_uvit_reserve(dfot_uvit_t h, int max_batch) {
  DFOT_REQUIRE(h && max_batch > 0, DFOT_ERR_ARG, "reserve: bad argument");
  if (max_batch <= h->max_batch) return DFOT_OK;
  for (void* p : h->ws_owned) (void)hipFree(p);
  h->ws_owned.clear();
  h->ws_bytes = 0;
  h->max_batch = 0;
  h->out_part = nullptr;
  h->pend_part = nullptr;
  h->out_part_elems = 0;
  h->attn_scratch = AttnScratch{};
  const size_t bt = (size_t)max_batch * h->T;
  size_t pix[4];
  for (int l = 0; l < 4; ++l) pix[l] = (size_t)h->r[l] * h->r[l];
  int rc = 0;
  if ((rc = dev_alloc(h, &h->nemb, bt * h->E, true))) return rc;
  if ((rc = dev_alloc(h, &h->nhid, bt * h->E, true))) return rc;
  for (int l = 0; l < 4; ++l) {
    if ((rc = dev_alloc(h, &h->XB[l], bt * pix[l] * h->ch[l], true))) return rc;
    if (l >= 2 && (rc = dev_alloc(h, &h->X[l], bt * pix[l] * h->ch[l], true))) return rc;
    if ((rc = dev_alloc(h, &h->emb[l], bt * pix[l] * h->E, true))) return rc;
  }
  for (int l = 0; l < 3; ++l)
    if ((rc = dev_alloc(h, &h->HSA[l], bt * pix[l + 1] * h->ch[l + 1], true))) return rc;
  if ((rc = dev_alloc(h, &h->acond, bt * pix[0] * h->kpose, true))) return rc;
  DFOT_CHECK_HIP(hipMemset(h->acond, 0, bt * pix[0] * h->kpose * sizeof(bf16)));
  size_t act = 0, tmpn = 0;
  for (int l = 0; l < 4; ++l) act = std::max(act, bt * pix[l] * h->ch[l]);
  for (int l = 0; l < 3; ++l) tmpn = std::max(tmpn, bt * pix[l + 1] * h->ch[l]);
  if ((rc = dev_alloc(h, &h->s1, act, true))) return rc;
  if ((rc = dev_alloc(h, &h->hbf, act, true))) return rc;
  if ((rc = dev_alloc(h, &h->tmp, tmpn, true))) return rc;
  if ((rc = dev_alloc(h, &h->gn_partial, bt * (pix[0] / 64) * 64, true))) return rc;
  if ((rc = dev_alloc(h, &h->gn_partial2, bt * (pix[0] / 64) * 64, true))) return rc;
  if ((rc = dev_alloc(h, &h->gn_stats, bt * 64, true))) return rc;
  size_t mtr = 0, mc = 0;
  for (int l = 2; l < 4; ++l) {
    mtr = std::max(mtr, bt * pix[l]);
    mc = std::max(mc, bt * pix[l] * h->ch[l]);
  }
  (void)mtr;
  {
    std::vector<FilmChunk> table;
    long sv_off = 0;
    auto add = [&](bf16** fc, long* off, const bf16* wf, const float* bf_, int c, int lvl) -> int {
      int r2 = dev_alloc(h, fc, bt * pix[lvl] * 2 * c, true);
      if (r2) return r2;
      *off = sv_off;
      for (int r0 = 0; r0 < 2 * c; r0 += 64) table.push_back(FilmChunk{wf + (long)r0 * h->E, bf_ + r0, sv_off + r0, 2 * c});
      sv_off += (long)bt * 2 * c;
      return DFOT_OK;
    };
    for (int l = 0; l < 2; ++l) {
      for (ResW& w : h->down_res[l]) if ((rc = add(&w.fcache, &w.sv_off, w.w_film, w.b_film, w.c, l))) return rc;
      for (ResW& w : h->up_res[l]) if ((rc = add(&w.fcache, &w.sv_off, w.w_film, w.b_film, w.c, l))) return rc;
    }
    for (TrW& w : h->down_tr) if ((rc = add(&w.fcache, &w.sv_off, w.w_film, w.b_film, w.c, 2))) return rc;
    for (TrW& w : h->up_tr) if ((rc = add(&w.fcache, &w.sv_off, w.w_film, w.b_film, w.c, 2))) return rc;
    for (TrW& w : h->mid_tr) if ((rc = add(&w.fcache, &w.sv_off, w.w_film, w.b_film, w.c, 3))) return rc;
    if ((rc = dev_alloc(h, &h->sv, (size_t)sv_off, true))) return rc;
    if ((rc = dev_alloc(h, &h->film_table, table.size(), true))) return rc;
    DFOT_CHECK_HIP(hipMemcpy(h->film_table, table.data(), table.size() * sizeof(FilmChunk), hipMemcpyHostToDevice));
    h->film_chunks = (int)table.size();
    if ((rc = dev_alloc(h, &h->cond_mask, (size_t)max_batch, true))) return rc;
    h->cond_batch = 0;
  }
  if ((rc = dev_alloc(h, &h->cat, mc * 5, true))) return rc;
  if ((rc = dev_alloc(h, &h->q, mc, true))) return rc;
  if ((rc = dev_alloc(h, &h->k, mc, true))) return rc;
  if ((rc = dev_alloc(h, &h->v, mc, true))) return rc;
  {
    const size_t e2 = bt * pix[2] * h->ch[2], e3 = bt * pix[3] * h->ch[3];
    h->out_part_elems = 3 * (e2 > e3 ? e2 : e3);
    if ((rc = dev_alloc(h, &h->out_part, h->out_part_elems, true))) return rc;
  }
  {
    size_t need = 16;
    for (int b = 1; b <= max_batch; ++b)
      for (int l = 2; l < 4; ++l) need = std::max(need, attention_scratch_bytes(b, h->heads, h->T * h->r[l] * h->r[l], h->ch[l] / h->heads));
    if ((rc = dev_alloc(h, &h->attn_scratch.p, need / sizeof(float), true))) return rc;
    h->attn_scratch.bytes = need;
  }
  h->max_batch = max_batch;
  return DFOT_OK;
}

size_t dfot_uvit_workspace_bytes(dfot_uvit_t h) { return h ? h->ws_bytes : 0; }

int dfot_uvit_attn_timing(dfot_uvit_t h, double* total_ms, int64_t* launches) {
  DFOT_REQUIRE(h && total_ms && launches, DFOT_ERR_ARG, "attn_timing: null argument");
  double tot = 0.0;
  for (size_t i = 0; i < h->ev_used; ++i) {
    DFOT_CHECK_HIP(hipEventSynchronize(h->ev_stop[i]));
    float ms = 0.f;
    DFOT_CHECK_HIP(hipEventElapsedTime(&ms, h->ev_start[i], h->ev_stop[i]));
    tot += ms;
  }
  *total_ms = tot;
  *launches = (int64_t)h->ev_used;
  h->ev_used = 0;
  return DFOT_OK;
}

int dfot_uvit_set_option(dfot_uvit_t h, const char* key, int value) {
  DFOT_REQUIRE(h && key, DFOT_ERR_ARG, "set_option: null argument");
  if (!strcmp(key, "gemm_variant")) h->gemm_variant = value;
  else if (!strcmp(key, "attn_variant")) h->attn_variant = value;
  else if (!strcmp(key, "attn_force_safe")) h->attn_force_safe = value != 0;
  else if (!strcmp(key, "time_attn")) {
    h->time_attn = value > 0;
    h->ev_used = 0;
    while ((int)h->ev_start.size() < value) {
      hipEvent_t a, b;
      DFOT_CHECK_HIP(hipEventCreate(&a));
      DFOT_CHECK_HIP(hipEventCreate(&b));
      h->ev_start.push_back(a);
      h->ev_stop.push_back(b);
    }
  }
  else {
    set_error("set_option: unknown key '%s'", key);
    return DFOT_ERR_ARG;
  }
  return DFOT_OK;
}

int dfot_uvit_query(dfot_uvit_t h, const char* key, double* value) {
  DFOT_REQUIRE(h && key && value, DFOT_ERR_ARG, "query: null argument");
  DFOT_REQUIRE(h->finalized, DFOT_ERR_STATE, "query: weights not finalized");
  float bound = 0.f;
  for (const TrW& w : h->down_tr) bound = fmaxf(bound, w.score_bound);
  for (const TrW& w : h->up_tr) bound = fmaxf(bound, w.score_bound);
  if (!strcmp(key, "score_bound_l2")) *value = bound;
  else if (!strcmp(key, "attn_kernel_l2")) *value = (bound < 64.0f && !h->attn_force_safe) ? 14 : 5;
  else if (!strcmp(key, "cond_builds")) *value = (double)h->cond_builds;
  else {
    set_error("query: unknown key '%s'", key);
    return DFOT_ERR_ARG;
  }
  return DFOT_OK;
}

int dfot_uvit_set_conditions(dfot_uvit_t h, const float* external_cond, const uint8_t* external_cond_mask, int batch,
                             void* stream) {
  DFOT_REQUIRE(h, DFOT_ERR_ARG, "set_conditions: null handle");
  DFOT_REQUIRE(external_cond != nullptr, DFOT_ERR_ARG, "External condition (camera pose) is required for U-ViT3DPose model.");
  DFOT_REQUIRE(h->finalized, DFOT_ERR_STATE, "set_conditions: weights not finalized");
  DFOT_REQUIRE(batch > 0 && batch <= h->max_batch, DFOT_ERR_STATE, "set_conditions: batch %d exceeds reserved %d", batch, h->max_batch);
  hipStream_t s = (hipStream_t)stream;
  const dfot_uvit_config& c = h->cfg;
  const int bt = batch * h->T, e = h->E;
  int rc = 0;
  h->cond_batch = 0;
  ++h->cond_builds;
  if ((rc = launch_cond_repack(external_cond, h->acond, bt, c.resolution, c.cond_dim, h->kpose, s))) return rc;
  {
    GemmArgs g;
    g.A = h->acond; g.lda = h->kpose; g.W = h->pose_w; g.M = bt * h->r[0] * h->r[0]; g.N = e; g.K = h->kpose;
    g.bias = h->pose_b; g.out_bf16 = h->emb[0]; g.ldo = e;
    if ((rc = launch_gemm(A_DENSE, E_BF16, h->gemm_variant, g, s))) return rc;
  }
  if ((rc = launch_emb_pyramid(h->emb[0], h->emb[1], h->emb[2], h->emb[3], bt, h->r[0], e, s))) return rc;
  auto fill = [&](bf16* fcache, const bf16* wf, int cc, int lvl) -> int {
    GemmArgs g;
    g.A = h->emb[lvl]; g.lda = e; g.W = wf; g.M = bt * h->r[lvl] * h->r[lvl]; g.N = 2 * cc; g.K = e;
    g.out_bf16 = fcache; g.ldo = 2 * cc;
    return launch_gemm(A_DENSE, E_BF16, h->gemm_variant, g, s);
  };
  for (int l = 0; l < 2; ++l) {
    for (ResW& w : h->down_res[l]) if ((rc = fill(w.fcache, w.w_film, w.c, l))) return rc;
    for (ResW& w : h->up_res[l]) if ((rc = fill(w.fcache, w.w_film, w.c, l))) return rc;
  }
  for (TrW& w : h->down_tr) if ((rc = fill(w.fcache, w.w_film, w.c, 2))) return rc;
  for (TrW& w : h->up_tr) if ((rc = fill(w.fcache, w.w_film, w.c, 2))) return rc;
  for (TrW& w : h->mid_tr) if ((rc = fill(w.fcache, w.w_film, w.c, 3))) return rc;
  h->have_mask = external_cond_mask != nullptr;
  if (h->have_mask) DFOT_CHECK_HIP(hipMemcpyAsync(h->cond_mask, external_cond_mask, batch, hipMemcpyDeviceToDevice, s));
  h->cond_batch = batch;
  return DFOT_OK;
}

int dfot_uvit_forward_cached(dfot_uvit_t h, const float* x, const float* noise_levels, float* out, int batch, void* stream) {
  return dfot_uvit_forward_cached_live(h, x, noise_levels, out, batch, nullptr, stream);
}

int dfot_uvit_forward_cached_live(dfot_uvit_t h, const float* x, const float* noise_levels, float* out, int batch, const uint8_t* live_frames,
                                  void* stream) {
  return dfot_uvit_forward_cached_masks(h, x, noise_levels, out, batch, live_frames, nullptr, stream);
}

int dfot_uvit_forward_cached_masks(dfot_uvit_t h, const float* x, const float* noise_levels, float* out, int batch, const uint8_t* live_frames,
                                   const uint8_t* fresh_frames, void* stream) {
  DFOT_REQUIRE(h && x && noise_levels && out, DFOT_ERR_ARG, "forward: null argument");
  DFOT_REQUIRE(!fresh_frames || h->last_batch == batch, DFOT_ERR_STATE,
               "forward: frozen frames need the previous forward of this handle to have run the same batch (%d, now %d)", h->last_batch, batch);
  DFOT_REQUIRE(!fresh_frames || live_frames, DFOT_ERR_ARG, "forward: frozen frames must also be dead frames (live_frames is null)");
  DFOT_REQUIRE(h->finalized, DFOT_ERR_STATE, "forward: weights not finalized");
  DFOT_REQUIRE(batch > 0 && batch == h->cond_batch, DFOT_ERR_STATE,
               "forward_cached: batch %d does not match the cached conditions (%d)", batch, h->cond_batch);
  hipStream_t s = (hipStream_t)stream;
  const dfot_uvit_config& c = h->cfg;
  const int bt = batch * h->T, e = h->E;
  int rc = 0;
  if ((rc = launch_noise_emb(noise_levels, h->ne_freqs, h->ne_phases, h->ne_w1, h->ne_b1, h->ne_w2, h->ne_b2, h->nhid,
                             h->nemb, bt, c.noise_dim, e, s)))
    return rc;
  if ((rc = launch_film_vec(h->film_table, h->film_chunks, h->nemb, h->sv, bt, e, s))) return rc;
  if ((rc = launch_embed_input_bf16(x, h->ein_w, h->ein_b, h->XB[0], bt, c.resolution, c.in_channels, h->ch[0], s))) return rc;
  h->gn1_nblk = 0;
  for (int l = 0; l < 4; ++l) h->xin[l] = h->X[l];
  h->xin_bf[0] = true;
  h->xin_bf[1] = h->xin_bf[2] = h->xin_bf[3] = false;

  if (fresh_frames && (h->gemm_variant != GEMM_AUTO || (h->r[2] * h->r[2]) % 512 != 0)) fresh_frames = nullptr;
  for (int l = 0; l < 2; ++l) {
    for (const ResW& w : h->down_res[l])
      if ((rc = run_res_block(h, w, l, bt, s, fresh_frames))) return rc;
    if ((rc = run_down(h, l, bt, s, fresh_frames))) return rc;
  }
  h->pend_bias = nullptr;
  for (const TrW& w : h->down_tr)
    if ((rc = run_tr_block(h, w, 2, batch, s))) return rc;
  if ((rc = flush_pending(h, s))) return rc;
  if ((rc = run_down(h, 2, bt, s))) return rc;
  for (const TrW& w : h->mid_tr)
    if ((rc = run_tr_block(h, w, 3, batch, s))) return rc;
  if ((rc = flush_pending(h, s))) return rc;
  if ((rc = run_up(h, 2, bt, s))) return rc;
  for (const TrW& w : h->up_tr)
    if ((rc = run_tr_block(h, w, 2, batch, s))) return rc;
  if ((rc = flush_pending(h, s))) return rc;
  for (int l = 1; l >= 0; --l) {
    if ((rc = run_up(h, l, bt, s, live_frames))) return rc;
    for (const ResW& w : h->up_res[l])
      if ((rc = run_res_block(h, w, l, bt, s, live_frames))) return rc;
  }
  h->last_batch = batch;
  return launch_project_output_bf16(h->XB[0], h->pout_w, h->pout_b, out, bt, c.resolution, h->ch[0], c.in_channels, s, live_frames);
}

int dfot_uvit_forward(dfot_uvit_t h, const float* x, const float* noise_levels, const float* external_cond,
                      const uint8_t* external_cond_mask, float* out, int batch, void* stream) {
  DFOT_REQUIRE(h && x && noise_levels && out, DFOT_ERR_ARG, "forward: null argument");
  int rc = dfot_uvit_set_conditions(h, external_cond, external_cond_mask, batch, stream);
  if (rc) return rc;
  return dfot_uvit_forward_cached(h, x, noise_levels, out, batch, stream);
}

int dfot_uvit_read_tap(dfot_uvit_t h, const char* name, float* out, size_t capacity, void* stream) {
  DFOT_REQUIRE(h && name && out, DFOT_ERR_ARG, "read_tap: null argument");
  DFOT_REQUIRE(h->last_batch > 0, DFOT_ERR_STATE, "read_tap: no forward has run");
  hipStream_t s = (hipStream_t)stream;
  const int bt = h->last_batch * h->T;
  auto pixels = [&](int l) { return h->r[l] * h->r[l]; };
  struct Tap { const char* n; int lvl; int c; const float* f; const bf16* b; };
  const Tap taps[] = {
      {"pose_emb0", 0, h->E, nullptr, h->emb[0]}, {"down0", 1, h->ch[1], h->HSA[0], nullptr},
      {"down1", 2, h->ch[2], h->HSA[1], nullptr}, {"down2", 3, h->ch[3], h->HSA[2], nullptr},
      {"mid", 3, h->ch[3], nullptr, h->XB[3]}, {"up2", 2, h->ch[2], nullptr, h->XB[2]},
      {"up1", 1, h->ch[1], nullptr, h->XB[1]}, {"up0", 0, h->ch[0], nullptr, h->XB[0]},
  };
  for (const Tap& t : taps) {
    if (strcmp(t.n, name)) continue;
    const size_t need = (size_t)bt * pixels(t.lvl) * t.c;
    DFOT_REQUIRE(capacity >= need, DFOT_ERR_SHAPE, "read_tap: need %zu floats, got %zu", need, capacity);
    return t.f ? launch_nhwc_to_nchw(t.f, out, bt, pixels(t.lvl), t.c, s)
               : launch_bf16_nhwc_to_nchw(t.b, out, bt, pixels(t.lvl), t.c, s);
  }
  set_error("read_tap: unknown tap '%s'", name);
  return DFOT_ERR_NAME;
}

int dfot_ray_encode(const float* raw_poses, float* out, int batch, int tokens, int resolution, void* stream) {
  DFOT_REQUIRE(raw_poses && out && batch > 0 && tokens > 0 && resolution > 0, DFOT_ERR_ARG, "ray_encode: bad argument");
  return launch_ray_encode(raw_poses, out, batch, tokens, resolution, 0, (hipStream_t)stream);
}

int dfot_ray_encode_normalized(const float* poses, float* out, int batch, int tokens, int resolution, void* stream) {
  DFOT_REQUIRE(poses && out && batch > 0 && tokens > 0 && resolution > 0, DFOT_ERR_ARG, "ray_encode_normalized: bad argument");
  return launch_ray_encode(poses, out, batch, tokens, resolution, 1, (hipStream_t)stream);
}

int dfot_hg_prepare(const float* x, const float* noise, const float* qa, const float* qb, float* x_in, int batch, int nfe,
                    int tokens, int64_t frame_elems, void* stream) {
  DFOT_REQUIRE(x && qa && qb && x_in, DFOT_ERR_ARG, "hg_prepare: null argument");
  return launch_hg_prepare(x, noise, qa, qb, x_in, batch, nfe, tokens, (long)frame_elems, (hipStream_t)stream);
}

int dfot_ddim_compose(const float* x, const float* x_in, const float* v, const float* sa, const float* s1, const float* an,
                      const float* cn, const float* keep, const float* weight, const uint8_t* gen, float* x_next, int batch,
                      int nfe, int tokens, int64_t frame_elems, void* stream) {
  DFOT_REQUIRE(x && x_in && v && sa && s1 && an && cn && keep && weight && gen && x_next, DFOT_ERR_ARG, "ddim_compose: null argument");
  return launch_ddim_compose(x, x_in, v, sa, s1, an, cn, keep, weight, gen, x_next, batch, nfe, tokens, (long)frame_elems, false,
                             (hipStream_t)stream);
}
int dfot_ddim_compose_tokw(const float* x, const float* x_in, const float* v, const float* sa, const float* s1, const float* an,
                           const float* cn, const float* keep, const float* weight, const uint8_t* gen, float* x_next, int batch,
                           int nfe, int tokens, int64_t frame_elems, void* stream) {
  DFOT_REQUIRE(x && x_in && v && sa && s1 && an && cn && keep && weight && gen && x_next, DFOT_ERR_ARG, "ddim_compose_tokw: null argument");
  return launch_ddim_compose(x, x_in, v, sa, s1, an, cn, keep, weight, gen, x_next, batch, nfe, tokens, (long)frame_elems, true,
                             (hipStream_t)stream);
}

int dfot_ddim_noise(const float* noise, const float* sigma, const float* weight, const uint8_t* gen, float* x_next, int batch, int nfe,
                    int tokens, int64_t frame_elems, int weight_per_token, void* stream) {
  DFOT_REQUIRE(noise && sigma && weight && gen && x_next, DFOT_ERR_ARG, "ddim_noise: null argument");
  return launch_ddim_noise(noise, sigma, weight, gen, x_next, batch, nfe, tokens, (long)frame_elems, weight_per_token != 0, (hipStream_t)stream);
}

int dfot_vpred_loss(const float* x, const float* noise, const float* v, const float* alpha, const float* sigma,
                    const float* weight, float* x_pred, float* scratch, float* loss, int batch, int tokens, int64_t frame_elems,
                    void* stream) {
  DFOT_REQUIRE(x && noise && v && alpha && sigma && weight && scratch && loss, DFOT_ERR_ARG, "vpred_loss: null argument");
  return launch_vloss(x, noise, v, alpha, sigma, weight, x_pred, scratch, loss, batch * tokens, (long)frame_elems, false,
                      (hipStream_t)stream);
}
int dfot_vspace_loss(const float* x, const float* noise, const float* v, const float* alpha, const float* sigma,
                     const float* weight, float* x_pred, float* scratch, float* loss, int batch, int tokens, int64_t frame_elems,
                     void* stream) {
  DFOT_REQUIRE(x && noise && v && alpha && sigma && weight && scratch && loss, DFOT_ERR_ARG, "vspace_loss: null argument");
  return launch_vloss(x, noise, v, alpha, sigma, weight, x_pred, scratch, loss, batch * tokens, (long)frame_elems, true,
                      (hipStream_t)stream);
}
int64_t dfot_vpred_loss_scratch_floats(int batch, int tokens, int64_t frame_elems) {
  return (int64_t)batch * tokens * vloss_chunks((long)frame_elems);
}

static bf16* g_zero_page = nullptr;
static int zero_page(bf16** out) {
  if (!g_zero_page) {
    DFOT_CHECK_HIP(hipMalloc((void**)&g_zero_page, 512));
    DFOT_CHECK_HIP(hipMemset(g_zero_page, 0, 512));
  }
  *out = g_zero_page;
  return DFOT_OK;
}

int dfot_op_gemm(const void* a, int lda, const void* w, const float* bias, float* c, int m, int n, int k, int variant,
                 void* stream) {
  GemmArgs g;
  g.A = (const bf16*)a; g.lda = lda; g.W = (const bf16*)w; g.M = m; g.N = n; g.K = k; g.bias = bias; g.out_f32 = c; g.ldo = n;
  DFOT_REQUIRE(c, DFOT_ERR_ARG, "op_gemm: null output");
  return launch_gemm(A_DENSE, E_F32, variant, g, (hipStream_t)stream);
}

int dfot_op_conv3x3(const void* a, const void* w, const float* bias, float* y, int bt, int hh, int ww, int cin, int cout,
                    int variant, void* stream) {
  GemmArgs g;
  int rc = zero_page(const_cast<bf16**>(&g.zeros));
  if (rc) return rc;
  g.A = (const bf16*)a; g.W = (const bf16*)w; g.M = bt * hh * ww; g.N = cout; g.K = 9 * cin; g.H = hh; g.Wd = ww; g.Cin = cin;
  g.bias = bias; g.out_f32 = y; g.ldo = cout;
  DFOT_REQUIRE(y, DFOT_ERR_ARG, "op_conv3x3: null output");
  return launch_gemm(A_CONV3, E_F32, variant, g, (hipStream_t)stream);
}

int dfot_op_gemm_ex(const dfot_gemm_desc* d, void* stream) {
  DFOT_REQUIRE(d, DFOT_ERR_ARG, "op_gemm_ex: null descriptor");
  GemmArgs g;
  if (d->amode == A_CONV3) {
    int rc = zero_page(const_cast<bf16**>(&g.zeros));
    if (rc) return rc;
  }
  g.A = (const bf16*)d->A; g.lda = d->lda; g.W = (const bf16*)d->W; g.ldw = d->ldw;
  g.M = d->M; g.N = d->N; g.K = d->K; g.H = d->H; g.Wd = d->Wd; g.Cin = d->Cin;
  g.live = d->live; g.bias = d->bias; g.bias_rows = d->bias_rows;
  g.out_f32 = d->out_f32; g.out_bf16 = (bf16*)d->out_bf16; g.ldo = d->ldo;
  g.resid = d->resid; g.resid_bf = (const bf16*)d->resid_bf;
  g.gate = d->gate; g.gate_index = d->gate_index; g.ldg = d->ldg; g.gate_rows = d->gate_rows;
  g.act = d->act; g.pre_act = (bf16*)d->pre_act; g.raw = (bf16*)d->raw; g.ldraw = d->ldraw; g.tr_rows = d->tr_rows;
  g.gn_part = d->gn_part; g.gn_rows_per_bt = d->gn_rows_per_bt; g.gn_cpg = d->gn_cpg;
  g.out2 = (bf16*)d->out2; g.ldo2 = d->ldo2; g.split = d->split;
  g.q = (bf16*)d->q; g.k = (bf16*)d->k; g.v = (bf16*)d->v;
  g.qw = d->qw; g.kw = d->kw; g.rope_cs = d->rope_cs;
  g.heads = d->heads; g.d = d->d; g.ntok = d->ntok; g.qscale = d->qscale; g.dstride = d->dstride; g.eps = d->eps;
  g.ksplit = d->ksplit; g.slice_stride = d->slice_stride;
  return launch_gemm(d->amode, d->epi, d->variant, g, (hipStream_t)stream);
}
int64_t dfot_op_gemm_desc_bytes(void) { return (int64_t)sizeof(dfot_gemm_desc); }

int dfot_op_attention(const void* q, const void* k, const void* v, void* o, int ldo, int batch, int heads, int n, int d,
                      int variant, void* stream) {
  return launch_attention((const bf16*)q, (const bf16*)k, (const bf16*)v, (bf16*)o, ldo, batch, heads, n, d, variant,
                          (hipStream_t)stream);
}

int dfot_op_f32_to_bf16(const float* src, void* dst, int64_t n, void* stream) {
  DFOT_REQUIRE(src && dst && n >= 0, DFOT_ERR_ARG, "op_f32_to_bf16: null argument");
  return launch_f32_to_bf16(src, (bf16*)dst, (long)n, (hipStream_t)stream);
}
int dfot_op_bf16_to_f32(const void* src, float* dst, int64_t n, void* stream) {
  DFOT_REQUIRE(src && dst && n >= 0, DFOT_ERR_ARG, "op_bf16_to_f32: null argument");
  return launch_bf16_to_f32((const bf16*)src, dst, (long)n, (hipStream_t)stream);
}

}
```

### diffusion-forcing-transformer_amd/sampler.py

```python
from __future__ import annotations

from dataclasses import dataclass, field
from typing import Callable, Dict, List, Optional, Tuple

import numpy as np
import torch

from . import capi, parallel
from .diffusion import DiffusionConfig, Schedule
from .guidance import HistoryGuidance


@dataclass
class SamplerConfig:
    x_shape: Tuple[int, int, int] = (3, 256, 256)
    max_tokens: int = 8
    diffusion: DiffusionConfig = field(default_factory=DiffusionConfig)
    scheduling_matrix: str = "full_sequence"
    is_full_sequence: bool = False
    prediction_guidance: Dict = field(default_factory=lambda: {"name": "conditional"})
    interpolation_guidance: Dict = field(default_factory=lambda: {"name": "conditional"})
    keyframe_density: Optional[float] = None
    sliding_context_len: Optional[int] = None
    interpolation_max_batch_size: Optional[int] = None
# ... 207 lines not shown
            sm = sm[int(np.argmax(changed)):]
        else:
            if cfg.scheduling_matrix != "full_sequence":
                raise ValueError("Refining only support full_sequence scheduling matrix")
            sm = sch.refine_scheduling_matrix(horizon - padding, _refine[0], _refine[1], padding)
            sm = np.repeat(sm[:, None, :], batch_size, axis=1)
            sm = np.where(mask[None] >= 1, -1, sm)
        self.trace.append({"context_mask": mask.copy(), "batch": batch_size, "rows": sm.shape[0]})

        plans = []
        for m in range(sm.shape[0] - 1):
            frm, to = sm[m], sm[m + 1]
            if _refine is not None and not frm[0, -1] > to[0, -1]:
                ac = sch.alphas_cumprod.astype(np.float32)
                with np.errstate(divide="ignore", invalid="ignore"):
                    scale = np.where(to == self.timesteps - 1, np.float32(1), ac[to] / ac[frm]).astype(np.float32)
                if not (np.isfinite(scale).all() and (scale <= 1).all()):
                    raise ValueError("refinement sampling: this window / schedule makes q_sample_from_x_k produce NaN in the reference "
                                     "(alphas_cumprod ratio not in [0, 1]); refused instead of returning NaN")
                tables = np.zeros((8, batch_size, horizon), np.float32)
                tables[0], tables[1] = np.sqrt(scale), np.sqrt(np.float32(1) - scale)
                plans.append(dict(renoise=True, nfe=1, bm=batch_size, tables=tables, gen=(mask == 0).astype(np.uint8), cmask=None))
                continue
            mask = np.where((mask == 0) & (frm == -1), 2, mask)
            plan = history_guidance.plan(mask, frm, to, replacement_only=cfg.is_full_sequence)
            bm = batch_size * plan.nfe
            lv = plan.levels.reshape(bm, horizon)
            tl = plan.to_levels.reshape(bm, horizon)
            repl = plan.replace.reshape(bm, horizon)
            qa_c, qb_c = sch.q_sample_coef(lv)
            qa = np.where(repl, qa_c, np.float32(1)).astype(np.float32)
            qb = np.where(repl, qb_c, np.float32(0)).astype(np.float32)
            excl = None
            if plan.excluded is not None:
                excl = plan.excluded.reshape(bm, horizon)
                qa, qb = np.where(excl, np.float32(0), qa), np.where(excl, np.float32(1), qb)
            sa, s1, an, cn, keepf, sigma = sch.ddim_coef(lv, tl) if sch.is_ddim_sampling else sch.ddpm_coef(lv)
            sigma = np.where(keepf != 0, np.float32(0), sigma).astype(np.float32)
            tables = np.stack([qa, qb, sa, s1, an, cn, keepf, sch.model_level(lv)]).astype(np.float32)
            plans.append(dict(plan=plan, nfe=plan.nfe, bm=bm, need_noise=bool(repl.any()) or excl is not None, excl=excl, tables=tables,
                              sigma=sigma if bool((sigma != 0).any()) else None,
                              gen=(mask == 0).astype(np.uint8),
                              cmask=None if plan.cond_masked is None else np.tile(plan.cond_masked, batch_size)))
        if not plans:
            return (xs[:, :-padding] if padding > 0 else xs), None
        strict = bool(getattr(self.noise_fn, "strict_order", False))

        def draw_noise(p_):
            nfe, bm, need = p_["nfe"], p_["bm"], p_["need_noise"]
            noise = None
            if history_guidance.is_simple:
                if nfe == 2 and (need or strict):
                    drawn = self.noise_fn("q_sample", (batch_size, horizon, *x_shape))
                    noise = torch.zeros(batch_size, 2, horizon, *x_shape, device=dev, dtype=torch.float32)
                    noise[:, 0] = drawn.to(device=dev, dtype=torch.float32)
            else:
                g = p_["plan"].n_gen
                bh = bm // g
                if need or strict:
                    noise = self.noise_fn("q_sample", (bh, horizon, *x_shape)).to(device=dev, dtype=torch.float32)
                    if g > 1:
                        noise = noise.repeat_interleave(g, dim=0)
                if strict or p_["excl"] is not None:
                    fresh = self.noise_fn("excluded", (bh, g, horizon, *x_shape))
                    if p_["excl"] is not None:
                        fresh = fresh.to(device=dev, dtype=torch.float32).reshape(bm, horizon, *x_shape)
                        em = torch.from_numpy(p_["excl"]).to(dev).view(bm, horizon, *([1] * len(x_shape)))
                        noise = torch.where(em, fresh, noise if noise is not None else torch.zeros_like(fresh))
            return None if noise is None else noise.contiguous().view(bm, horizon, *x_shape)

        split_nfe = set()
        if self._branch_split_active:
            world_n = parallel.world_info()[0]
            for n_ in sorted({p_["nfe"] for p_ in plans if not p_.get("renoise")}):
                if n_ > 1 and world_n > 1 and world_n % n_ == 0:
                    parallel.branch_group(n_)
                    split_nfe.add(n_)
        if self.dry_run:
            for p_ in plans:
                if p_["nfe"] in split_nfe:
                    hb = parallel.world_info()[1] % p_["nfe"]
                    got = parallel.exchange_branches(torch.full((batch_size, 1), float(hb)), p_["nfe"])
                    if not torch.equal(got.view(batch_size, p_["nfe"]), torch.arange(p_["nfe"], dtype=got.dtype).repeat(batch_size, 1)):
                        raise RuntimeError("branch exchange returned the branches out of (sample, branch) order")
                    self.branch_exchanges = getattr(self, "branch_exchanges", 0) + 1
                if p_.get("renoise"):
                    self.noise_fn("renoise", (batch_size, horizon, *x_shape))
                    continue
                draw_noise(p_)
                if strict or p_["sigma"] is not None:
                    self.noise_fn("ddim", (p_["bm"], horizon, *x_shape))
                    if _refine is not None:
                        self.noise_fn("refine_context", (batch_size, horizon, *x_shape))
            self.window_forwards += sum(p_["bm"] for p_ in plans if not p_.get("renoise"))
            return (xs[:, :-padding] if padding > 0 else xs), None
        flat_dev = torch.from_numpy(np.concatenate([p_["tables"].ravel() for p_ in plans])).cuda()
        gens_dev = torch.from_numpy(np.stack([p_["gen"] for p_ in plans])).cuda()
        off = 0
        cmask_cache: Dict[bytes, torch.Tensor] = {}
        weight_cache: Dict[bytes, torch.Tensor] = {}
        lives_by_nfe: Dict[int, torch.Tensor] = {}
        for i, p_ in enumerate(plans):
            n = p_["tables"].size
            p_["tables_dev"] = flat_dev[off:off + n].view(8, p_["bm"], horizon)
            off += n
            p_["gen_dev"] = gens_dev[i]
            if p_.get("renoise"):
                continue
            if p_["nfe"] not in lives_by_nfe:
                lives_by_nfe[p_["nfe"]] = gens_dev if p_["nfe"] == 1 else gens_dev.repeat_interleave(p_["nfe"], dim=1)
            p_["live_dev"] = lives_by_nfe[p_["nfe"]][i]
            wsrc = p_["plan"].weights if p_["plan"].tok_weights is None else p_["plan"].tok_weights
            wkey = wsrc.tobytes()
            if wkey not in weight_cache:
                weight_cache[wkey] = torch.from_numpy(np.ascontiguousarray(wsrc, dtype=np.float32)).cuda()
            p_["weights_dev"] = weight_cache[wkey]
            p_["tokw"] = p_["plan"].tok_weights is not None
            p_["sigma_dev"] = None if p_["sigma"] is None else torch.from_numpy(p_["sigma"]).cuda()
            p_["cmask_dev"] = None
            if p_["cmask"] is not None:
                ckey = p_["cmask"].tobytes()
                if ckey not in cmask_cache:
                    cmask_cache[ckey] = torch.from_numpy(p_["cmask"]).cuda()
                p_["cmask_dev"] = cmask_cache[ckey]

        cond_full = None if pose_interp else self._window_conditions(conditions)
        cond_rep, cond_nfe = None, 0
        if pose_interp:
            by_mask: Dict[bytes, torch.Tensor] = {}
            self._interpolate_masked_poses = True
            try:
                for p_ in plans:
                    if p_.get("renoise"):
                        continue
                    lv = p_["plan"].levels.reshape(p_["bm"], horizon)
                    key = (lv == self.timesteps - 1).tobytes() + bytes([p_["nfe"]])
                    if key not in by_mask:
                        by_mask[key] = self._process_conditions(conditions.repeat_interleave(p_["nfe"], dim=0), lv)
                    p_["cond"] = by_mask[key]
            finally:
                self._interpolate_masked_poses = False
        fresh_dev = torch.from_numpy(np.concatenate([a.ravel() for a in self._fresh_flags(plans, batch_size, horizon)])).cuda()
        foff = 0
        for p_ in plans:
            p_["fresh_dev"] = fresh_dev[foff:foff + p_["bm"] * horizon].view(p_["bm"], horizon)
            foff += p_["bm"] * horizon
        xs = xs.contiguous()
        s = capi.stream_ptr
        branch_cache: Dict[tuple, tuple] = {}

        skip_dead = self.skip_dead_frames and hasattr(self.model, "live_frames")
        skip_frozen = skip_dead and self.skip_frozen_frames and hasattr(self.model, "fresh_frames")

        def step(p_, xs, noise, tables, gen_dev, xs_next=None, live_dev=None, fresh_dev=None):
            nonlocal cond_rep, cond_nfe
            nfe, bm = p_["nfe"], p_["bm"]
            x_in = torch.empty(bm, horizon, *x_shape, device="cuda", dtype=torch.float32)
            capi.check(capi.lib.dfot_hg_prepare(capi.ptr(xs), capi.ptr(noise), capi.ptr(tables[0]), capi.ptr(tables[1]),
                                                capi.ptr(x_in), batch_size, nfe, horizon, f, s()))
            if cond_full is not None and cond_nfe != nfe:
                cond_rep = cond_full if nfe == 1 else cond_full.repeat_interleave(nfe, dim=0)
                cond_nfe = nfe
            if "cond" in p_:
                cond_rep = p_["cond"]
            lvl = tables[7] if cfg.diffusion.is_continuous else tables[7].to(torch.int32)
            world, rank = parallel.world_info()
            if nfe in split_nfe:
                hb = rank % nfe
                key = (id(cond_rep), id(p_["cmask_dev"]), hb)
                if key not in branch_cache:
                    c_h = None if cond_rep is None else cond_rep.view(batch_size, nfe, *cond_rep.shape[1:])[:, hb].contiguous()
                    m_h = None if p_["cmask_dev"] is None else p_["cmask_dev"].view(batch_size, nfe)[:, hb].contiguous()
                    branch_cache[key] = (c_h, m_h, cond_rep, p_["cmask_dev"])
                c_h, m_h = branch_cache[key][:2]
                x_h = x_in.view(batch_size, nfe, horizon, *x_shape)[:, hb].contiguous()
                l_h = lvl.view(batch_size, nfe, horizon)[:, hb].contiguous()
                if skip_dead:
                    self.model.live_frames = gen_dev
                try:
                    v = parallel.exchange_branches(self.model(x_h, l_h, c_h, m_h), nfe)
                    self.branch_exchanges = getattr(self, "branch_exchanges", 0) + 1
                finally:
                    if skip_dead:
                        self.model.live_frames = None
            elif rg > 0:
                v = self._reconstruction_guided_v(x_in, lvl, cond_rep, p_["cmask_dev"], tables, gen_dev, rg_ctx, rg, nfe)
            else:
                if skip_dead:
                    self.model.live_frames = live_dev if live_dev is not None else p_["live_dev"]
                if skip_frozen:
                    self.model.fresh_frames = fresh_dev if fresh_dev is not None else p_["fresh_dev"]
                try:
                    v = self.model(x_in, lvl, cond_rep, p_["cmask_dev"])
                finally:
                    if skip_dead:
                        self.model.live_frames = None
                    if skip_frozen:
                        self.model.fresh_frames = None
            step_noise = None
            if strict or p_["sigma"] is not None:
                step_noise = self.noise_fn("ddim", (bm, horizon, *x_shape))
            if xs_next is None:
                xs_next = torch.empty_like(xs)
            compose = capi.lib.dfot_ddim_compose_tokw if p_["tokw"] else capi.lib.dfot_ddim_compose
            capi.check(compose(capi.ptr(xs), capi.ptr(x_in), capi.ptr(v), capi.ptr(tables[2]),
                                                  capi.ptr(tables[3]), capi.ptr(tables[4]), capi.ptr(tables[5]),
                                                  capi.ptr(tables[6]), capi.ptr(p_["weights_dev"]), capi.ptr(gen_dev),
                                                  capi.ptr(xs_next), batch_size, nfe, horizon, f, s()))
            if p_["sigma"] is not None:
                nz = step_noise.to(device="cuda", dtype=torch.float32).clamp(-cfg.diffusion.clip_noise, cfg.diffusion.clip_noise).contiguous()
                capi.check(capi.lib.dfot_ddim_noise(capi.ptr(nz), capi.ptr(p_["sigma_dev"]), capi.ptr(p_["weights_dev"]), capi.ptr(gen_dev),
                                                    capi.ptr(xs_next), batch_size, nfe, horizon, f, int(p_["tokw"]), s()))
            return xs_next

        def renoise(p_, xs):
            noise = self.noise_fn("renoise", (batch_size, horizon, *x_shape)).to(device="cuda", dtype=torch.float32)
            noise = noise.clamp(-cfg.diffusion.clip_noise, cfg.diffusion.clip_noise).contiguous()
            out = torch.empty_like(xs)
            capi.check(capi.lib.dfot_hg_prepare(capi.ptr(xs), capi.ptr(noise), capi.ptr(p_["tables_dev"][0]), capi.ptr(p_["tables_dev"][1]),
                                                capi.ptr(out), batch_size, 1, horizon, f, s()))
            return out

        if _refine is not None:
            for p_ in plans:
                if p_.get("renoise"):
                    xs = renoise(p_, xs)
                    continue
                xs = step(p_, xs, draw_noise(p_), p_["tables_dev"], p_["gen_dev"])
                if strict:
                    self.noise_fn("refine_context", (batch_size, horizon, *x_shape))
            self.window_forwards += sum(p_["bm"] for p_ in plans if not p_.get("renoise"))
            return (xs[:, :-padding] if padding > 0 else xs), None
        uniform = all(p_["bm"] == plans[0]["bm"] and p_["cmask_dev"] is plans[0]["cmask_dev"]
                      and p_["weights_dev"] is plans[0]["weights_dev"] and p_.get("cond") is plans[0].get("cond") for p_ in plans)
        hook = getattr(self, "step_hook", None)
        if (self.use_graph and uniform and not strict and len(plans) > 2 and all(p_["sigma"] is None for p_ in plans) and not self._branch_split_active
                and rg == 0 and hook is None):
            if self._static_graph_cond and cond_full is not None:
                nfe0 = plans[0]["nfe"]
                plans[0]["cond_src"] = cond_full if nfe0 == 1 else cond_full.repeat_interleave(nfe0, dim=0)
            xs = self._run_steps_graph(plans, xs, draw_noise, step, flat_dev, gens_dev, horizon)
        else:
            for i, p_ in enumerate(plans):
                xs = step(p_, xs, draw_noise(p_), p_["tables_dev"], p_["gen_dev"])
                if hook is not None:
                    hook(i, xs)
        self.window_forwards += sum(p_["bm"] for p_ in plans)
        if padding > 0:
            xs = xs[:, :-padding]
        return xs, None

    @torch.no_grad()
    def _sample_sequence_refine(self, batch_size: int, goback_length: int, n_goback: int, length: Optional[int] = None,
                                context: Optional[torch.Tensor] = None, context_mask: Optional[torch.Tensor] = None,
                                conditions: Optional[torch.Tensor] = None, history_guidance: Optional[HistoryGuidance] = None,
                                **_) -> Tuple[torch.Tensor, None]:
        return self._sample_sequence(batch_size, length=length, context=context, context_mask=context_mask, conditions=conditions,
                                     history_guidance=history_guidance, _refine=(int(goback_length), int(n_goback)))

    def _window_sampler(self):
        return self._sample_sequence

    def _reconstruction_guided_v(self, x_in, lvl, cond, cmask, tables, gen_dev, ctx, rg: float, nfe: int):
        if nfe != 1:
            raise ValueError("reconstruction guidance needs one-branch history guidance (the reference's loss compares the "
                             "(B * NFE, ...) prediction with the (B, ...) context)")
        if self.cfg.diffusion.objective != "pred_v":
            raise ValueError("reconstruction guidance is implemented for the v objective")
        nd = x_in.ndim
        ext = lambda a: a.reshape(*a.shape, *([1] * (nd - a.ndim)))
        sa, s1 = ext(tables[2]), ext(tables[3])
        with torch.enable_grad():
            x = x_in.detach().requires_grad_(True)
            v = self.model(x, lvl, cond, cmask)
            pred_x0 = sa * x - s1 * v
            cm = ext((gen_dev == 0).to(torch.float32))
            loss = torch.sum((pred_x0 - ctx) ** 2 * sa * cm / cm.sum(dim=1, keepdim=True).clamp(min=1))
            grad = torch.nan_to_num(-torch.autograd.grad(-rg * 0.5 * loss, x)[0], nan=0.0)
        an, cn = ext(tables[4]), ext(tables[5])
        scale = torch.where(sa > 0, s1 / sa.clamp(min=1e-30), torch.where(an > 0, -cn / an.clamp(min=1e-30), torch.zeros_like(sa)))
        return (v.detach() + scale * grad).contiguous()

    @staticmethod
    def _fresh_flags(plans, batch_size: int, horizon: int):
        out, prev = [], None
        for p_ in plans:
            fresh = np.ones((p_["bm"], horizon), np.uint8)
            if p_.get("renoise"):
                out.append(fresh)
                prev = None
                continue
            if (prev is not None and prev["bm"] == p_["bm"] and prev["nfe"] == p_["nfe"] and prev.get("cond") is p_.get("cond")
                    and ((prev["cmask"] is None and p_["cmask"] is None)
                         or (prev["cmask"] is not None and p_["cmask"] is not None and np.array_equal(prev["cmask"], p_["cmask"])))):
                a, b = prev["tables"], p_["tables"]
                same_in = (a[0] == 1) & (a[1] == 0) & (b[0] == 1) & (b[1] == 0) & (a[7] == b[7])
                untouched = np.repeat(prev["gen"].reshape(batch_size, horizon) == 0, p_["nfe"], axis=0)
                fresh = np.where(same_in & untouched, 0, 1).astype(np.uint8)
            out.append(fresh)
            prev = p_
        return out

    def _run_steps_graph(self, plans, xs, draw_noise, step, flat_dev, gens_dev, horizon):
        p0 = plans[0]
        bm, n_steps, nfe = p0["bm"], len(plans), p0["nfe"]
        need_noise = any(p_["need_noise"] for p_ in plans)
        self.model.reserve(bm)
        if hasattr(self.model, "sync_weights"):
            self.model.sync_weights()
        gen = getattr(self.model, "reserve_generation", 0)
        if gen != self._graphs_generation:
            self._graphs.clear()
            self._graphs_generation = gen
        cond_src = p0.get("cond_src")
        key = (bm, n_steps, nfe, horizon, tuple(xs.shape), need_noise, None if p0["cmask"] is None else p0["cmask"].tobytes(),
               id(self.model), None if cond_src is None else (tuple(cond_src.shape), cond_src.dtype))
        ent = self._graphs.get(key)
        if ent is None:
            ent = dict(tables=torch.empty(n_steps, 8, bm, horizon, device="cuda", dtype=torch.float32),
                       gens=torch.empty_like(gens_dev), weights=torch.empty_like(p0["weights_dev"]),
                       lives=torch.empty(n_steps, bm, horizon, device="cuda", dtype=torch.uint8),
                       fresh=torch.empty(n_steps, bm, horizon, device="cuda", dtype=torch.uint8),
                       noise=torch.empty(n_steps, bm, *xs.shape[1:], device="cuda") if need_noise else None,
                       xs=torch.empty_like(xs), out=None, graph=None,
                       cond=None if cond_src is None else torch.empty_like(cond_src))
        ent["tables"].copy_(flat_dev.view(n_steps, 8, bm, horizon))
        ent["gens"].copy_(gens_dev)
        ent["lives"].copy_(gens_dev if nfe == 1 else gens_dev.repeat_interleave(nfe, dim=1))
        ent["fresh"].copy_(torch.stack([p_["fresh_dev"] for p_ in plans]))
        ent["weights"].copy_(p0["weights_dev"])
        if need_noise:
            for i, p_ in enumerate(plans):
                if p_["need_noise"]:
                    ent["noise"][i].copy_(draw_noise(p_))
                else:
                    ent["noise"][i].zero_()
        p_static = dict(p0, weights_dev=ent["weights"])
        if cond_src is not None:
            ent["cond"].copy_(cond_src)
            p_static["cond"] = ent["cond"]
        ent["xs"].copy_(step(p_static, xs, None if not need_noise else ent["noise"][0], ent["tables"][0], ent["gens"][0], live_dev=ent["lives"][0],
                            fresh_dev=ent["fresh"][0]))
        if ent["graph"] is None:
            torch.cuda.synchronize()
            graph = torch.cuda.CUDAGraph()
            with torch.cuda.graph(graph, capture_error_mode="thread_local"):
                x = ent["xs"]
                for i in range(1, n_steps):
                    x = step(p_static, x, ent["noise"][i] if need_noise else None, ent["tables"][i], ent["gens"][i], live_dev=ent["lives"][i],
                             fresh_dev=ent["fresh"][i])
                ent["out"] = x
            ent["graph"] = graph
            if len(self._graphs) >= 4:
                self._graphs.pop(next(iter(self._graphs)))
            self._graphs[key] = ent
            self.graph_captures += 1
        ent["graph"].replay()
        self.graph_replays += n_steps - 1
        return ent["out"].clone()

    @torch.no_grad()
    def _predict_sequence(self, context: torch.Tensor, length: Optional[int] = None,
                          conditions: Optional[torch.Tensor] = None, history_guidance: Optional[HistoryGuidance] = None,
                          sliding_context_len: Optional[int] = None, **_) -> Tuple[torch.Tensor, None]:
        mt = self.max_tokens
        if length is None:
            length = mt
        if sliding_context_len is None:
            if mt < length:
                raise ValueError("when length > max_tokens, sliding_context_len must be specified.")
            sliding_context_len = mt - 1
        if sliding_context_len == -1:
            sliding_context_len = mt - 1
        batch_size, gt_len = context.shape[:2]
        if sliding_context_len < gt_len:
            raise ValueError("sliding_context_len is expected to be >= length of initial context,"
                             f"got {sliding_context_len}. If you are trying to use max context, "
                             "consider specifying sliding_context_len=-1.")
        xs = context.to(device=self.device, dtype=torch.float32)
        cur = gt_len
        n_window = 0
        while cur < length:
            c = min(sliding_context_len, cur)
            h = min(length - cur, mt - c)
            window = torch.cat([xs[:, -c:], xs.new_zeros(batch_size, h, *self.x_shape)], 1)
            generated = cur - max(cur - c, gt_len)
            cmask = torch.ones(batch_size, c, dtype=torch.long)
            if generated > 0:
                cmask[:, -generated:] = 2
            cmask = torch.cat([cmask, torch.zeros(batch_size, h, dtype=torch.long)], 1)
            cond = self._select_conditions(conditions, slice(cur - c, cur - c + mt))
            if hasattr(self.noise_fn, "set_windows"):
                self.noise_fn.set_windows([n_window])
            n_window += 1
            new, _ = self._window_sampler()(batch_size, length=c + h, context=window, context_mask=cmask,
                                           conditions=cond, history_guidance=history_guidance)
            xs = torch.cat([xs, new[:, -h:]], 1)
            cur = xs.shape[1]
        return xs, None

    def _interpolation_plan(self, known: np.ndarray) -> List[List[np.ndarray]]:
        mt = self.max_tokens
        known = known.copy()
        plan: List[List[np.ndarray]] = []
        while not known.all():
            keys = np.where(known)[0]
            stage: List[np.ndarray] = []
            chunk: Optional[np.ndarray] = None
            for left, right in zip(keys[:-1], keys[1:]):
                left, right = int(left), int(right)
                if chunk is not None:
                    if len(chunk) + right - left <= mt:
                        chunk = np.concatenate([chunk, np.arange(left + 1, right + 1)])
                        continue
                    stage.append(chunk)
                    chunk = None
                if right - left == 1:
                    continue
                if right - left >= mt - 1:
                    stage.append(torch.linspace(left, right, mt).round().long().numpy())
                else:
                    chunk = np.arange(left, right + 1)
            if chunk is not None:
                stage.append(chunk)
            for w in stage:
                known[w] = True
            plan.append(stage)
        return plan

    @torch.no_grad()
    def _interpolate_videos(self, context: torch.Tensor, context_mask: Optional[torch.Tensor] = None,
                            conditions: Optional[torch.Tensor] = None, **_) -> torch.Tensor:
        cfg = self.cfg
        if context_mask is None:
            context_mask = torch.zeros(context.shape[0], context.shape[1], dtype=torch.bool)
            context_mask[:, [0, -1]] = True
        else:
            context_mask = context_mask.detach().cpu().bool()
            assert bool(context_mask[:, [0, -1]].all()), "The first and last frames must be known to interpolate."
        hg = HistoryGuidance.from_config(cfg.interpolation_guidance, timesteps=self.timesteps)
        xs = context.to(device=self.device, dtype=torch.float32).clone()
        known = context_mask.clone()
        for si, stage in enumerate(self._interpolation_plan(context_mask[0].numpy())):
            ctx = torch.cat([self._pad_to_max_tokens(xs[:, w]) for w in stage], 0)
            msk = torch.cat([self._pad_to_max_tokens(known[:, w]) for w in stage], 0)
            cnd = None if conditions is None else torch.cat([self._padded_conditions(conditions, w) for w in stage], 0)

            def sample_batch(ids, ctx=ctx, msk=msk, cnd=cnd, si=si):
                if not ids:
                    return ctx.new_zeros((0, *ctx.shape[1:]))
                if hasattr(self.noise_fn, "set_windows"):
                    self.noise_fn.set_windows([(si + 1) * 100000 + i for i in ids])
                o, _ = self._window_sampler()(len(ids), context=ctx[ids], context_mask=msk[ids].long(),
                                             conditions=None if cnd is None else cnd[ids], history_guidance=hg)
                return o

            mb = cfg.interpolation_max_batch_size or ctx.shape[0]
            if self.shard_windows:
                out = parallel.run_sharded(ctx.shape[0], sample_batch, mb)
            else:
                out = torch.cat([sample_batch(list(range(i, min(i + mb, ctx.shape[0])))) for i in range(0, ctx.shape[0], mb)], 0)
            for w, pred in zip(stage, out.chunk(len(stage), 0)):
                xs[:, w] = pred[:, : len(w)]
                known[:, w] = True
        return xs

    @torch.no_grad()
    def _predict_videos(self, xs: torch.Tensor, n_context_tokens: int,
                        conditions: Optional[torch.Tensor] = None) -> torch.Tensor:
        cfg = self.cfg
        out = xs.to(device=self.device, dtype=torch.float32).clone()
        hg = HistoryGuidance.from_config(cfg.prediction_guidance, timesteps=self.timesteps)
        density = cfg.keyframe_density or 1
        if density > 1:
            raise ValueError("tasks.prediction.keyframe_density must be <= 1")
        n = out.shape[1]
        keys = torch.linspace(0, n - 1, round(density * n)).round().long()
        keys = torch.cat([torch.arange(n_context_tokens), keys]).unique()
        kc = self._select_conditions(conditions, keys)
        if self.branch_parallel and parallel.world_info()[0] > 1 and not (hasattr(self.noise_fn, "set_windows") or getattr(self.noise_fn, "replicated", False)):
            raise ValueError("branch_parallel needs a rank-independent noise source: parallel.WindowKeyedNoise (set_windows) or a noise_fn "
                             "whose attribute `replicated` is True (every rank draws the same tensors)")
        self._branch_split_active = bool(self.branch_parallel)
        try:
            pred, _ = self._predict_sequence(out[:, :n_context_tokens], length=len(keys), conditions=kc, history_guidance=hg,
                                             sliding_context_len=cfg.sliding_context_len or self.max_tokens // 2)
        finally:
            self._branch_split_active = False
        out[:, keys.to(self.device)] = pred
        if len(keys) < n:
            known = torch.zeros(out.shape[0], n, dtype=torch.bool)
            known[:, keys] = True
            out = self._interpolate_videos(out, known, conditions)
        return out


class DFoTVideoSampler(DFoTVideoPoseSampler):

    _static_graph_cond = True

    def _cond_type(self) -> str:
        t = self.cfg.external_cond_type
        if t not in ("label", "action"):
# ... 68 lines not shown
```

### include/dfot_hip.h

```cpp
#ifndef DFOT_HIP_H_
#define DFOT_HIP_H_

#include <stddef.h>
#include <stdint.h>

#ifdef __cplusplus
extern "C" {
#endif

enum {
  DFOT_OK = 0,
  DFOT_ERR_ARG = 1,
  DFOT_ERR_SHAPE = 2,
  DFOT_ERR_HIP = 3,
  DFOT_ERR_STATE = 4,
  DFOT_ERR_NAME = 5
};

typedef struct dfot_uvit_s* dfot_uvit_t;

typedef struct {
  int32_t channels[4];
  int32_t emb_channels;
  int32_t num_updown_blocks[3];
  int32_t num_mid_blocks;
  int32_t num_heads;
  int32_t in_channels;
  int32_t resolution;
  int32_t max_tokens;
  int32_t cond_dim;
  int32_t noise_dim;
  float rope_theta;
  float eps;
} dfot_uvit_config;

const char* dfot_last_error(void);
int dfot_version(void);

int dfot_uvit_create(const dfot_uvit_config* cfg, dfot_uvit_t* out);
int dfot_uvit_destroy(dfot_uvit_t h);
int dfot_uvit_num_params(dfot_uvit_t h);
const char* dfot_uvit_param_name(dfot_uvit_t h, int index);
int dfot_uvit_param_shape(dfot_uvit_t h, int index, int64_t shape[4], int* ndim);
int dfot_uvit_load_weight(dfot_uvit_t h, const char* name, const float* data, const int64_t* shape, int ndim,
                          void* stream);
int dfot_uvit_finalize(dfot_uvit_t h, void* stream);
int dfot_uvit_reserve(dfot_uvit_t h, int max_batch);
size_t dfot_uvit_workspace_bytes(dfot_uvit_t h);
int dfot_uvit_set_option(dfot_uvit_t h, const char* key, int value);
int dfot_uvit_query(dfot_uvit_t h, const char* key, double* value);
int dfot_uvit_attn_timing(dfot_uvit_t h, double* total_ms, int64_t* launches);

int dfot_uvit_forward(dfot_uvit_t h, const float* x, const float* noise_levels, const float* external_cond,
                      const uint8_t* external_cond_mask, float* out, int batch, void* stream);
int dfot_uvit_set_conditions(dfot_uvit_t h, const float* external_cond, const uint8_t* external_cond_mask, int batch,
                             void* stream);
int dfot_uvit_forward_cached(dfot_uvit_t h, const float* x, const float* noise_levels, float* out, int batch,
                             void* stream);
int dfot_uvit_forward_cached_live(dfot_uvit_t h, const float* x, const float* noise_levels, float* out, int batch,
                                  const uint8_t* live_frames, void* stream);
int dfot_uvit_forward_cached_masks(dfot_uvit_t h, const float* x, const float* noise_levels, float* out, int batch,
                                   const uint8_t* live_frames, const uint8_t* fresh_frames, void* stream);
int dfot_uvit_read_tap(dfot_uvit_t h, const char* name, float* out, size_t capacity_floats, void* stream);

typedef struct dfot_dit_s* dfot_dit_t;

typedef struct {
  int32_t hidden_size;
  int32_t depth;
  int32_t num_heads;
  int32_t patch_size;
  int32_t in_channels;
  int32_t height;
  int32_t width;
  int32_t max_tokens;
  int32_t mlp_hidden;
  int32_t noise_dim;
  int32_t timesteps;
  float rope_theta;
  float eps;
  int32_t variant;
  int32_t embed_col_dim;
  int32_t num_col_heads;
  int32_t num_row_heads;
  int32_t temporal_mlp_hidden;
  int32_t use_bias;
  int32_t cond_type;
  int32_t cond_dim;
  int32_t num_classes;
  int32_t cond_dropout;
  int32_t use_temporal_rope;
} dfot_dit_config;
enum { DFOT_COND_NONE = 0, DFOT_COND_ACTION = 1, DFOT_COND_LABEL = 2 };

int dfot_dit_create(const dfot_dit_config* cfg, dfot_dit_t* out);
int dfot_dit_destroy(dfot_dit_t h);
int dfot_dit_num_params(dfot_dit_t h);
const char* dfot_dit_param_name(dfot_dit_t h, int index);
int dfot_dit_param_shape(dfot_dit_t h, int index, int64_t shape[4], int* ndim);
int dfot_dit_load_weight(dfot_dit_t h, const char* name, const float* data, const int64_t* shape, int ndim, void* stream);
int dfot_dit_finalize(dfot_dit_t h, void* stream);
int dfot_dit_reserve(dfot_dit_t h, int max_batch);
size_t dfot_dit_workspace_bytes(dfot_dit_t h);
int dfot_dit_set_option(dfot_dit_t h, const char* key, int value);
int dfot_dit_attn_timing(dfot_dit_t h, double* total_ms, int64_t* launches);
int dfot_dit_forward(dfot_dit_t h, const float* x, const int32_t* noise_levels, float* out, int batch, int tokens,
                     void* stream);
int dfot_dit_forward_cond(dfot_dit_t h, const float* x, const int32_t* noise_levels, const float* cond, const int32_t* labels,
                          const uint8_t* cond_mask, float* out, int batch, int tokens, void* stream);
int dfot_dit_read_tap(dfot_dit_t h, const char* name, float* out, size_t capacity_floats, void* stream);

typedef struct dfot_dit_train_s* dfot_dit_train_t;
int dfot_dit_train_create(const dfot_dit_config* cfg, dfot_dit_train_t* out);
int dfot_dit_train_destroy(dfot_dit_train_t h);
int dfot_dit_train_num_params(dfot_dit_train_t h);
const char* dfot_dit_train_param_name(dfot_dit_train_t h, int i);
int dfot_dit_train_param_shape(dfot_dit_train_t h, int i, int64_t shape[4], int* ndim);
int64_t dfot_dit_train_param_offset(dfot_dit_train_t h, int i);
int64_t dfot_dit_train_total_numel(dfot_dit_train_t h);
size_t dfot_dit_train_workspace_bytes(dfot_dit_train_t h);
int dfot_dit_train_attach(dfot_dit_train_t h, float* params, float* grads);
int dfot_dit_train_reserve(dfot_dit_train_t h, int max_batch);
int dfot_dit_train_sync_weights(dfot_dit_train_t h, void* stream);
int dfot_dit_train_forward(dfot_dit_train_t h, const float* x, const int32_t* noise_levels, float* out, int batch, int tokens, void* stream);
int dfot_dit_train_forward_cond(dfot_dit_train_t h, const float* x, const int32_t* noise_levels, const float* cond, const int32_t* labels,
                                const uint8_t* cond_mask, float* out, int batch, int tokens, void* stream);
int dfot_dit_train_backward(dfot_dit_train_t h, const float* d_out, void* stream);
int dfot_dit_train_input_grad(dfot_dit_train_t h, float* dx, void* stream);
int dfot_vloss_grad(const float* x, const float* noise, const float* v, const float* a, const float* sigma, const float* coef, float* dv,
                    int batch, int tokens, int64_t frame_elems, int vspace, void* stream);
int dfot_sumsq(const float* x, int64_t n, float* out, void* stream);
int dfot_adamw_step(float* params, const float* grads, float* exp_avg, float* exp_avg_sq, int64_t n, float lr, float beta1, float beta2,
                    float eps, float weight_decay, int step, const float* grad_sumsq, float max_grad_norm, float* ema, float ema_decay,
                    void* stream);

int dfot_ray_encode(const float* raw_poses, float* out, int batch, int tokens, int resolution, void* stream);
int dfot_ray_encode_normalized(const float* poses, float* out, int batch, int tokens, int resolution, void* stream);

int dfot_hg_prepare(const float* x, const float* noise, const float* qa, const float* qb, float* x_in, int batch,
                    int nfe, int tokens, int64_t frame_elems, void* stream);
int dfot_ddim_compose(const float* x, const float* x_in, const float* v, const float* sa, const float* s1,
                      const float* an, const float* cn, const float* keep, const float* weight, const uint8_t* gen,
                      float* x_next, int batch, int nfe, int tokens, int64_t frame_elems, void* stream);

int dfot_ddim_compose_tokw(const float* x, const float* x_in, const float* v, const float* sa, const float* s1,
                           const float* an, const float* cn, const float* keep, const float* weight, const uint8_t* gen,
                           float* x_next, int batch, int nfe, int tokens, int64_t frame_elems, void* stream);

int dfot_ddim_noise(const float* noise, const float* sigma, const float* weight, const uint8_t* gen, float* x_next, int batch,
                    int nfe, int tokens, int64_t frame_elems, int weight_per_token, void* stream);

int dfot_vpred_loss(const float* x, const float* noise, const float* v, const float* alpha, const float* sigma,
                    const float* weight, float* x_pred, float* scratch, float* loss, int batch, int tokens,
                    int64_t frame_elems, void* stream);
int64_t dfot_vpred_loss_scratch_floats(int batch, int tokens, int64_t frame_elems);
int dfot_vspace_loss(const float* x, const float* noise, const float* v, const float* alpha, const float* sigma,
                     const float* weight, float* x_pred, float* scratch, float* loss, int batch, int tokens,
                     int64_t frame_elems, void* stream);

int dfot_op_gemm(const void* a_bf16, int lda, const void* w_bf16, const float* bias, float* c, int m, int n, int k,
                 int variant, void* stream);
int dfot_op_conv3x3(const void* a_bf16, const void* w_bf16, const float* bias, float* y, int bt, int h, int w,
                    int cin, int cout, int variant, void* stream);
typedef struct {
  int32_t amode, epi, variant;
  const void* A; int64_t lda;
  const void* W; int64_t ldw;
  int32_t M, N, K, H, Wd, Cin;
  const uint8_t* live;
  const float* bias; int32_t bias_rows;
  float* out_f32; void* out_bf16; int64_t ldo;
  const float* resid; const void* resid_bf;
  const float* gate; const int32_t* gate_index; int64_t ldg; int32_t gate_rows;
  int32_t act; void* pre_act; void* raw; int64_t ldraw; int32_t tr_rows;
  float* gn_part; int32_t gn_rows_per_bt, gn_cpg;
  void* out2; int64_t ldo2; int32_t split;
  void *q, *k, *v;
  const float *qw, *kw, *rope_cs;
  int32_t heads, d, ntok; float qscale; int32_t dstride; float eps;
  int32_t ksplit; int64_t slice_stride;
} dfot_gemm_desc;
int dfot_op_gemm_ex(const dfot_gemm_desc* desc, void* stream);
int64_t dfot_op_gemm_desc_bytes(void);
int dfot_op_attention(const void* q, const void* k, const void* v, void* o, int ldo, int batch, int heads, int n,
                      int d, int variant, void* stream);
int dfot_op_attention_padded(const void* q, const void* k, const void* v, void* o, int ldo, int batch, int heads, int n,
                             int d, void* stream);
int dfot_op_attention_temporal(const void* q, const void* k, const void* v, void* o, int ldo, int batch, int tokens, int patches,
                               int heads, int d, void* stream);
int dfot_op_matrix_attention_rope(const void* z, void* o, const float* rope_cs, int batch, int L, int E, int h, int cc, int rr,
                                  float scale, void* stream);
int dfot_op_matrix_attention(const void* z, void* o, int batch, int L, int E, int h, int cc, int rr, float scale, void* stream);
int dfot_op_attention_bwd(const void* q, const void* k, const void* v, const void* d_o, void* o, int ldo, void* dq, void* dk, void* dv,
                          int batch, int heads, int n, int d, void* stream);
int dfot_op_conv3x3_bwd(const void* x, const void* dy, const float* w, float* dx, float* dw, float* db, int bt, int h, int w_, int cin, int cout,
                        void* stream);
int dfot_op_conv3x3_bwd2(const void* x, const void* dy, const float* w, float* dx, void* dx_bf, float* dw, float* db, int bt, int h, int w_, int cin,
                         int cout, void* stream);
int dfot_op_gn_silu_bwd(const float* x, const float* dy, const float* gamma, const float* beta, const void* film, float eps, float* dx, void* dfilm,
                        float* dgamma, float* dbeta, int bt, int pixels, int channels, void* stream);
int dfot_op_rms_film_bwd(const float* x, const float* dxn, const float* w, const void* film, float eps, float* dx, void* dfilm, float* dw,
                         int64_t rows, int channels, int accumulate_dx, void* stream);
int dfot_op_rms_film_bwd_res(const float* x, const float* dxn, const float* w, const void* film, float eps, const float* dres, float* dx, void* dx_bf,
                             void* dfilm, float* dw, int64_t rows, int channels, void* stream);
int dfot_op_qknorm_rope_bwd(const void* fused, int ld, const void* dq, const void* dk, const void* dv, const float* qw, const float* kw,
                            const float* rope_cs, float eps, void* dfused, int ldo, float* dqw, float* dkw, int64_t rows, int ntok, int heads, int d,
                            void* stream);
int dfot_op_wgrad_nt(const void* a, int lda, const void* b, int ldb, float* out, int m, int n, int64_t rows, int slices, void* stream);
int dfot_op_gemm_bf16(const void* a, int lda, const void* w, const float* bias, void* out, int ldo, int m, int n, int k, void* stream);
int dfot_op_gemm_f32(const void* a, int lda, const void* w, const float* bias, const float* resid, float* out, int ldo, int m, int n, int k,
                     void* stream);
int dfot_op_transpose_bf16(const void* src, void* dst, int rows, int cols, void* stream);
int dfot_op_colsum_bf16(const void* src, int ld, float* out, int64_t rows, int n, void* stream);
int dfot_op_rms_film_fwd(const float* x, const float* w, const void* film, float eps, void* out, int64_t rows, int channels, void* stream);
int dfot_op_fused_proj_train(const void* a, int lda, const void* w, const float* bias, const float* qw, const float* kw, const float* rope_cs, float eps,
// ... 70 lines not shown
```

Before: 10.78.

## Precompute per-step FiLM scale/shift table and fuse bf16 cast into slab reduce

Before the sampling loop, the noise-embedding MLP and FiLM vector projections are computed for every denoising step in one batched launch and stored in a per-step table. Each forward then indexes that table instead of rerunning the noise MLP and film_vec kernels. Separately, the slab-reduce kernel between levels now also writes the bf16 copy of its output, which removes a later cast pass. The cost is extra device memory for up to 64 steps of tables, plus added state that is invalidated when weights are reloaded or memory is re-reserved.

Result: no change. 10.79, median of 3 (+0.0%).

```diff
diff --git a/diffusion-forcing-transformer_amd/backbone.py b/diffusion-forcing-transformer_amd/backbone.py
--- a/diffusion-forcing-transformer_amd/backbone.py
+++ b/diffusion-forcing-transformer_amd/backbone.py
@@ -80,6 +80,7 @@
         self._trainer_sig = None
         self.live_frames = None
         self.fresh_frames = None
+        self.noise_step = None
         self._fresh_key = None
         self._train_stamp = 0
         self._dropout_generator: Optional[torch.Generator] = None
@@ -145,6 +146,22 @@
     def set_option(self, key: str, value: int) -> None:
         self.reserve_generation = getattr(self, "reserve_generation", 0) + 1
         capi.check(capi.lib.dfot_uvit_set_option(self._handle, key.encode(), int(value)))
+
+    def set_noise_steps(self, levels: torch.Tensor) -> None:
+        if levels.ndim != 3 or levels.shape[2] != self.temporal_length:
+            raise ValueError(f"levels has shape {tuple(levels.shape)}, expected (n_steps, B, {self.temporal_length})")
+        dev = next(self.parameters()).device
+        capi.require_device(dev, levels=levels)
+        self.sync_weights()
+        self.reserve(levels.shape[1])
+        lf = levels.detach().to(torch.float32).contiguous()
+        capi.check(capi.lib.dfot_uvit_set_noise_steps(self._handle, capi.ptr(lf, torch.float32, "levels"), lf.shape[0], lf.shape[1],
+                                                      capi.stream_ptr()))
+
+    def read_sv(self, step: int = -1) -> torch.Tensor:
+        out = torch.empty(capi.lib.dfot_uvit_sv_floats(self._handle), device="cuda", dtype=torch.float32)
+        capi.check(capi.lib.dfot_uvit_read_sv(self._handle, int(step), capi.ptr(out), out.numel(), capi.stream_ptr()))
+        return out
 
     def query(self, key: str) -> float:
         self.sync_weights()
@@ -338,10 +355,11 @@
             capi.require_device(dev, fresh_frames=fresh)
             if key != self._fresh_key:
                 fresh = None
-        capi.check(capi.lib.dfot_uvit_forward_cached_masks(self._handle, capi.ptr(xf, torch.float32, "x"),
-                                                           capi.ptr(kf, torch.float32, "noise_levels"), capi.ptr(out), b,
-                                                           capi.ptr(live, torch.uint8, "live_frames"),
-                                                           capi.ptr(fresh, torch.uint8, "fresh_frames"), capi.stream_ptr()))
+        step = -1 if self.noise_step is None else int(self.noise_step)
+        capi.check(capi.lib.dfot_uvit_forward_cached_step(self._handle, capi.ptr(xf, torch.float32, "x"),
+                                                          capi.ptr(kf, torch.float32, "noise_levels"), capi.ptr(out), b,
+                                                          capi.ptr(live, torch.uint8, "live_frames"),
+                                                          capi.ptr(fresh, torch.uint8, "fresh_frames"), step, capi.stream_ptr()))
         self._fresh_key = key
         return out.to(x.dtype)
 
diff --git a/diffusion-forcing-transformer_amd/capi.py b/diffusion-forcing-transformer_amd/capi.py
--- a/diffusion-forcing-transformer_amd/capi.py
+++ b/diffusion-forcing-transformer_amd/capi.py
@@ -83,6 +83,10 @@
     "dfot_uvit_forward_cached": (_I, [_P, _P, _P, _P, _I, _P]),
     "dfot_uvit_forward_cached_live": (_I, [_P, _P, _P, _P, _I, _P, _P]),
     "dfot_uvit_forward_cached_masks": (_I, [_P, _P, _P, _P, _I, _P, _P, _P]),
+    "dfot_uvit_set_noise_steps": (_I, [_P, _P, _I, _I, _P]),
+    "dfot_uvit_forward_cached_step": (_I, [_P, _P, _P, _P, _I, _P, _P, _I, _P]),
+    "dfot_uvit_read_sv": (_I, [_P, _I, _P, C.c_size_t, _P]),
+    "dfot_uvit_sv_floats": (C.c_size_t, [_P]),
     "dfot_uvit_read_tap": (_I, [_P, C.c_char_p, _P, C.c_size_t, _P]),
     "dfot_dit_create": (_I, [C.POINTER(DiTConfig), C.POINTER(_P)]),
     "dfot_dit_destroy": (_I, [_P]),
diff --git a/diffusion-forcing-transformer_amd/csrc/kernels.h b/diffusion-forcing-transformer_amd/csrc/kernels.h
--- a/diffusion-forcing-transformer_amd/csrc/kernels.h
+++ b/diffusion-forcing-transformer_amd/csrc/kernels.h
@@ -24,6 +24,8 @@
   int rows;
 };
 int launch_film_vec(const FilmChunk* table, int chunks, const float* nemb, float* sv, int bt, int e, hipStream_t s);
+int launch_film_vec_steps(const FilmChunk* table, int chunks, const float* nemb, float* sv, int bt, int e, int nsteps, long sv_stride,
+                          hipStream_t s);
 int launch_gn_film_silu(const bf16* h, const float* stats, const float* gamma, const float* beta, const bf16* fcache,
                         const float* sv, const uint8_t* cond_mask, bf16* out, int bt, int pixels, int c, int tokens,
                         hipStream_t s, const uint8_t* live = nullptr);
diff --git a/diffusion-forcing-transformer_amd/csrc/kernels.hip b/diffusion-forcing-transformer_amd/csrc/kernels.hip
--- a/diffusion-forcing-transformer_amd/csrc/kernels.hip
+++ b/diffusion-forcing-transformer_amd/csrc/kernels.hip
@@ -37,6 +37,7 @@
 
 int launch_noise_emb(const float* k, const float* freqs, const float* phases, const float* w1, const float* b1,
                      const float* w2, const float* b2, float* hidden, float* out, int bt, int ndim, int e, hipStream_t s) {
+  DFOT_REQUIRE(bt > 0 && bt <= 65535, DFOT_ERR_SHAPE, "noise_emb: %d rows exceed the grid's y range", bt);
   hipLaunchKernelGGL(noise_mlp_kernel<true>, dim3(cdiv(e, 4), bt), dim3(256), 0, s, k, freqs, phases, w1, b1, hidden, ndim, e);
   DFOT_CHECK_HIP(hipGetLastError());
   hipLaunchKernelGGL(noise_mlp_kernel<false>, dim3(cdiv(e, 4), bt), dim3(256), 0, s, hidden, nullptr, nullptr, w2, b2, out, e, e);
@@ -578,7 +579,7 @@
 
 
 __global__ __launch_bounds__(256) void film_vec_kernel(const FilmChunk* __restrict__ table, const float* __restrict__ nemb,
-                                                       float* __restrict__ sv, int e, int nbt) {
+                                                       float* __restrict__ sv, int e, int nbt, int nsteps, long sv_stride) {
   const FilmChunk ck = table[blockIdx.x >> 4];
   const int lane = threadIdx.x & 63, wave = threadIdx.x >> 6;
   const int r = (blockIdx.x & 15) * 4 + wave;
@@ -597,6 +598,7 @@
     }
   }
   const float bias = ck.b[r];
+  for (int st = 0; st < nsteps; ++st, nemb += (long)nbt * e, sv += sv_stride)
   for (int bt = 0; bt < nbt; ++bt) {
     const float* ne = nemb + (long)bt * e;
     float acc = 0.f;
@@ -616,11 +618,12 @@
 }
 template <int EQ>
 __global__ __launch_bounds__(256, 2) void film_vec_lds_kernel(const FilmChunk* __restrict__ table, const float* __restrict__ nemb,
-                                                           float* __restrict__ sv, int nbt) {
+                                                           float* __restrict__ sv, int nbt, int nsteps, long sv_stride) {
   constexpr int E = EQ * 256;
   __shared__ float4v ne[16][E / 4];
   const FilmChunk ck = table[blockIdx.x >> 1];
   const int lane = threadIdx.x & 63, wave = threadIdx.x >> 6;
+  for (int st = 0; st < nsteps; ++st, nemb += (long)nbt * E, sv += sv_stride)
   for (int bt0 = 0; bt0 < nbt; bt0 += 16) {
     __syncthreads();
     for (int i = threadIdx.x; i < 16 * (E / 4); i += 256) {
@@ -668,17 +671,21 @@
     }
   }
 }
-int launch_film_vec(const FilmChunk* table, int chunks, const float* nemb, float* sv, int bt, int e, hipStream_t s) {
+int launch_film_vec_steps(const FilmChunk* table, int chunks, const float* nemb, float* sv, int bt, int e, int nsteps, long sv_stride,
+                          hipStream_t s) {
   DFOT_REQUIRE(e % 8 == 0 && e <= 1024, DFOT_ERR_SHAPE, "film_vec: emb dim %d must be a multiple of 8 and <= 1024", e);
   if (e == 1024 || e == 512) {
-    if (e == 1024) hipLaunchKernelGGL(film_vec_lds_kernel<4>, dim3(chunks * 2), dim3(256), 0, s, table, nemb, sv, bt);
-    else hipLaunchKernelGGL(film_vec_lds_kernel<2>, dim3(chunks * 2), dim3(256), 0, s, table, nemb, sv, bt);
+    if (e == 1024) hipLaunchKernelGGL(film_vec_lds_kernel<4>, dim3(chunks * 2), dim3(256), 0, s, table, nemb, sv, bt, nsteps, sv_stride);
+    else hipLaunchKernelGGL(film_vec_lds_kernel<2>, dim3(chunks * 2), dim3(256), 0, s, table, nemb, sv, bt, nsteps, sv_stride);
     DFOT_CHECK_HIP(hipGetLastError());
     return DFOT_OK;
   }
-  hipLaunchKernelGGL(film_vec_kernel, dim3(chunks * 16), dim3(256), 0, s, table, nemb, sv, e, bt);
-  DFOT_CHECK_HIP(hipGetLastError());
-  return DFOT_OK;
+  hipLaunchKernelGGL(film_vec_kernel, dim3(chunks * 16), dim3(256), 0, s, table, nemb, sv, e, bt, nsteps, sv_stride);
+  DFOT_CHECK_HIP(hipGetLastError());
+  return DFOT_OK;
+}
+int launch_film_vec(const FilmChunk* table, int chunks, const float* nemb, float* sv, int bt, int e, hipStream_t s) {
+  return launch_film_vec_steps(table, chunks, nemb, sv, bt, e, 1, 0, s);
 }
 
 __global__ void gn_film_silu_kernel(const bf16* __restrict__ h, const float* __restrict__ stats,
diff --git a/diffusion-forcing-transformer_amd/csrc/uvit.hip b/diffusion-forcing-transformer_amd/csrc/uvit.hip
--- a/diffusion-forcing-transformer_amd/csrc/uvit.hip
+++ b/diffusion-forcing-transformer_amd/csrc/uvit.hip
@@ -89,6 +89,15 @@
   float *nemb = nullptr, *nhid = nullptr, *X[4] = {nullptr, nullptr, nullptr, nullptr}, *HSA[3] = {nullptr, nullptr, nullptr}, *tmp = nullptr,
         *gn_partial = nullptr, *gn_partial2 = nullptr, *gn_stats = nullptr, *sv = nullptr;
   int gn1_nblk = 0;
+  float *nemb_steps = nullptr, *nhid_steps = nullptr, *sv_steps = nullptr;
+  const float* sv_cur = nullptr;
+  size_t sv_elems = 0;
+  int noise_steps_cap = 64;
+  int noise_steps_reserved = 0;
+  enum { NT_NONE, NT_VALID, NT_INVALID } nt_state = NT_NONE;
+  int nt_steps = 0, nt_batch = 0;
+  int64_t noise_table_builds = 0;
+  bool opt_noise_table = true, opt_cast_fused = true;
   FilmChunk* film_table = nullptr;
   int film_chunks = 0;
   uint8_t* cond_mask = nullptr;
@@ -368,7 +377,7 @@
   g.gn_part = h->gn_partial2; g.gn_rows_per_bt = pix; g.gn_cpg = c / 32;
   if ((rc = launch_gemm(A_CONV3, E_BF16, h->gemm_variant, g, s))) return rc;
   if ((rc = launch_gn_finalize(h->gn_partial2, h->gn_stats, bt, slots, pix, c, h->cfg.eps, s))) return rc;
-  if ((rc = launch_gn_film_silu(h->hbf, h->gn_stats, w.g2, w.be2, w.fcache, h->sv + w.sv_off,
+  if ((rc = launch_gn_film_silu(h->hbf, h->gn_stats, w.g2, w.be2, w.fcache, h->sv_cur + w.sv_off,
                                 h->have_mask ? h->cond_mask : nullptr, h->s1, bt, pix, c, h->T, s, live)))
     return rc;
   GemmArgs o;
@@ -425,7 +434,7 @@
     h->xin_bf[lvl] = true;
   }
   RmsPending pend{xb, h->pend_bias, h->pend_part, h->pend_part + (long)m * c, h->pend_slices == 3 ? h->pend_part + 2L * m * c : nullptr};
-  if ((rc = launch_rms_film_bf16(xb, w.nw, w.fcache, h->sv + w.sv_off, h->have_mask ? h->cond_mask : nullptr, h->s1, m, c, rr * rr, h->T,
+  if ((rc = launch_rms_film_bf16(xb, w.nw, w.fcache, h->sv_cur + w.sv_off, h->have_mask ? h->cond_mask : nullptr, h->s1, m, c, rr * rr, h->T,
                                  h->cfg.eps, s, h->pend_bias ? &pend : nullptr)))
     return rc;
   h->pend_bias = nullptr;
@@ -468,17 +477,23 @@
 
 
 __global__ void slab_reduce_kernel(float* __restrict__ out, const float* __restrict__ bias, const float* __restrict__ slabs, int nslab, long stride4,
-                                   long total4, int cq, const uint8_t* __restrict__ live, unsigned img4) {
+                                   long total4, int cq, const uint8_t* __restrict__ live, unsigned img4, bf16* __restrict__ out_bf) {
   typedef __attribute__((ext_vector_type(4))) float f4;
   const long i = (long)blockIdx.x * blockDim.x + threadIdx.x;
   if (i >= total4) return;
-  if (live && !live[(unsigned)i / img4]) return;
-  f4 v = reinterpret_cast<const f4*>(bias)[i % cq];
-  for (int sl = 0; sl < nslab; ++sl) v += reinterpret_cast<const f4*>(slabs)[sl * stride4 + i];
-  reinterpret_cast<f4*>(out)[i] = v;
-}
-
-static int conv_between_levels(dfot_uvit_s* h, GemmArgs g, hipStream_t s) {
+  f4 v;
+  if (live && !live[(unsigned)i / img4]) {
+    if (!out_bf) return;
+    v = reinterpret_cast<const f4*>(out)[i];
+  } else {
+    v = reinterpret_cast<const f4*>(bias)[i % cq];
+    for (int sl = 0; sl < nslab; ++sl) v += reinterpret_cast<const f4*>(slabs)[sl * stride4 + i];
+    reinterpret_cast<f4*>(out)[i] = v;
+  }
+  if (out_bf) reinterpret_cast<bf16x4*>(out_bf)[i] = bf16x4{f2bf(v[0]), f2bf(v[1]), f2bf(v[2]), f2bf(v[3])};
+}
+
+static int conv_between_levels(dfot_uvit_s* h, GemmArgs g, hipStream_t s, bf16* out_bf = nullptr, bool* wrote_bf = nullptr) {
   const long px = (long)g.H * g.Wd;
   if (h->gemm_variant == GEMM_AUTO && h->out_part && !g.gn_part && g.M % 256 == 0 && px % 256 == 0 && (g.N % 144 == 0 || g.N == 256) &&
       (long)g.M * g.N < (1L << 31)) {
@@ -498,8 +513,9 @@
         if (rc) return rc;
         const long total4 = (long)g.M * g.N / 4;
         hipLaunchKernelGGL(slab_reduce_kernel, dim3(cdiv(total4, 256)), dim3(256), 0, s, out, bias, h->out_part, ks, total4, total4, g.N / 4, g.live,
-                           (unsigned)(px * g.N / 4));
+                           (unsigned)(px * g.N / 4), out_bf);
         DFOT_CHECK_HIP(hipGetLastError());
+        if (out_bf && wrote_bf) *wrote_bf = true;
         return DFOT_OK;
       }
     }
@@ -520,10 +536,11 @@
   if (next_is_res) {
     g.gn_part = h->gn_partial; g.gn_rows_per_bt = (rr / 2) * (rr / 2); g.gn_cpg = cout / 32;
   }
-  if ((rc = conv_between_levels(h, g, s))) return rc;
+  bool wrote_bf = false;
+  if ((rc = conv_between_levels(h, g, s, h->opt_cast_fused ? h->XB[l + 1] : nullptr, &wrote_bf))) return rc;
   h->gn1_nblk = next_is_res ? g.gn_rows_per_bt / 64 : 0;
   h->xin[l + 1] = h->HSA[l];
-  h->xin_bf[l + 1] = false;
+  h->xin_bf[l + 1] = wrote_bf;
   return DFOT_OK;
 }
 
@@ -613,6 +630,7 @@
   if (rc) return rc;
   p.loaded = true;
   h->finalized = false;
+  if (h->nt_state == dfot_uvit_s::NT_VALID) h->nt_state = dfot_uvit_s::NT_INVALID;
   return DFOT_OK;
 }
 
@@ -663,6 +681,8 @@
   h->pend_part = nullptr;
   h->out_part_elems = 0;
   h->attn_scratch = AttnScratch{};
+  h->noise_steps_reserved = 0;
+  if (h->nt_state == dfot_uvit_s::NT_VALID) h->nt_state = dfot_uvit_s::NT_INVALID;
   const size_t bt = (size_t)max_batch * h->T;
   size_t pix[4];
   for (int l = 0; l < 4; ++l) pix[l] = (size_t)h->r[l] * h->r[l];
@@ -712,6 +732,15 @@
     for (TrW& w : h->up_tr) if ((rc = add(&w.fcache, &w.sv_off, w.w_film, w.b_film, w.c, 2))) return rc;
     for (TrW& w : h->mid_tr) if ((rc = add(&w.fcache, &w.sv_off, w.w_film, w.b_film, w.c, 3))) return rc;
     if ((rc = dev_alloc(h, &h->sv, (size_t)sv_off, true))) return rc;
+    h->sv_elems = (size_t)sv_off;
+    h->sv_cur = h->sv;
+    if (h->noise_steps_cap > 0) {
+      const size_t ns = (size_t)h->noise_steps_cap;
+      if ((rc = dev_alloc(h, &h->sv_steps, ns * h->sv_elems, true))) return rc;
+      if ((rc = dev_alloc(h, &h->nemb_steps, ns * bt * h->E, true))) return rc;
+      if ((rc = dev_alloc(h, &h->nhid_steps, ns * bt * h->E, true))) return rc;
+      h->noise_steps_reserved = h->noise_steps_cap;
+    }
     if ((rc = dev_alloc(h, &h->film_table, table.size(), true))) return rc;
     DFOT_CHECK_HIP(hipMemcpy(h->film_table, table.data(), table.size() * sizeof(FilmChunk), hipMemcpyHostToDevice));
     h->film_chunks = (int)table.size();
@@ -760,6 +789,12 @@
   if (!strcmp(key, "gemm_variant")) h->gemm_variant = value;
   else if (!strcmp(key, "attn_variant")) h->attn_variant = value;
   else if (!strcmp(key, "attn_force_safe")) h->attn_force_safe = value != 0;
+  else if (!strcmp(key, "noise_table")) h->opt_noise_table = value != 0;
+  else if (!strcmp(key, "cast_fused")) h->opt_cast_fused = value != 0;
+  else if (!strcmp(key, "noise_table_steps")) {
+    DFOT_REQUIRE(value >= 0, DFOT_ERR_ARG, "set_option: noise_table_steps %d is negative", value);
+    h->noise_steps_cap = value;
+  }
   else if (!strcmp(key, "time_attn")) {
     h->time_attn = value > 0;
     h->ev_used = 0;
@@ -787,6 +822,10 @@
   if (!strcmp(key, "score_bound_l2")) *value = bound;
   else if (!strcmp(key, "attn_kernel_l2")) *value = (bound < 64.0f && !h->attn_force_safe) ? 14 : 5;
   else if (!strcmp(key, "cond_builds")) *value = (double)h->cond_builds;
+  else if (!strcmp(key, "noise_table_builds")) *value = (double)h->noise_table_builds;
+  else if (!strcmp(key, "noise_table")) *value = h->opt_noise_table ? 1 : 0;
+  else if (!strcmp(key, "cast_fused")) *value = h->opt_cast_fused ? 1 : 0;
+  else if (!strcmp(key, "noise_table_steps")) *value = (double)h->noise_steps_reserved;
   else {
     set_error("query: unknown key '%s'", key);
     return DFOT_ERR_ARG;
@@ -842,9 +881,42 @@
   return dfot_uvit_forward_cached_masks(h, x, noise_levels, out, batch, live_frames, nullptr, stream);
 }
 
+int dfot_uvit_set_noise_steps(dfot_uvit_t h, const float* levels, int n_steps, int batch, void* stream) {
+  DFOT_REQUIRE(h && levels, DFOT_ERR_ARG, "set_noise_steps: null argument");
+  DFOT_REQUIRE(h->finalized, DFOT_ERR_STATE, "set_noise_steps: weights not finalized");
+  DFOT_REQUIRE(batch > 0 && batch <= h->max_batch, DFOT_ERR_STATE, "set_noise_steps: batch %d exceeds reserved %d", batch, h->max_batch);
+  DFOT_REQUIRE(n_steps > 0 && n_steps <= h->noise_steps_reserved, DFOT_ERR_STATE, "set_noise_steps: %d steps exceed the %d reserved", n_steps,
+               h->noise_steps_reserved);
+  hipStream_t s = (hipStream_t)stream;
+  const int bt = batch * h->T, e = h->E;
+  h->nt_state = dfot_uvit_s::NT_NONE;
+  ++h->noise_table_builds;
+  int rc = 0;
+  if ((rc = launch_noise_emb(levels, h->ne_freqs, h->ne_phases, h->ne_w1, h->ne_b1, h->ne_w2, h->ne_b2, h->nhid_steps, h->nemb_steps,
+                             n_steps * bt, h->cfg.noise_dim, e, s)))
+    return rc;
+  if ((rc = launch_film_vec_steps(h->film_table, h->film_chunks, h->nemb_steps, h->sv_steps, bt, e, n_steps, (long)h->sv_elems, s))) return rc;
+  h->nt_state = dfot_uvit_s::NT_VALID;
+  h->nt_steps = n_steps;
+  h->nt_batch = batch;
+  return DFOT_OK;
+}
+
 int dfot_uvit_forward_cached_masks(dfot_uvit_t h, const float* x, const float* noise_levels, float* out, int batch, const uint8_t* live_frames,
                                    const uint8_t* fresh_frames, void* stream) {
+  return dfot_uvit_forward_cached_step(h, x, noise_levels, out, batch, live_frames, fresh_frames, -1, stream);
+}
+
+int dfot_uvit_forward_cached_step(dfot_uvit_t h, const float* x, const float* noise_levels, float* out, int batch, const uint8_t* live_frames,
+                                  const uint8_t* fresh_frames, int step, void* stream) {
   DFOT_REQUIRE(h && x && noise_levels && out, DFOT_ERR_ARG, "forward: null argument");
+  const bool table = step >= 0 && h->opt_noise_table && h->nt_state != dfot_uvit_s::NT_NONE;
+  if (table) {
+    DFOT_REQUIRE(h->nt_state == dfot_uvit_s::NT_VALID, DFOT_ERR_STATE,
+                 "forward: the noise table is stale (weights or workspace changed since dfot_uvit_set_noise_steps)");
+    DFOT_REQUIRE(step < h->nt_steps, DFOT_ERR_ARG, "forward: step %d is outside the noise table (%d steps)", step, h->nt_steps);
+    DFOT_REQUIRE(batch == h->nt_batch, DFOT_ERR_STATE, "forward: batch %d does not match the noise table (%d)", batch, h->nt_batch);
+  }
   DFOT_REQUIRE(!fresh_frames || h->last_batch == batch, DFOT_ERR_STATE,
                "forward: frozen frames need the previous forward of this handle to have run the same batch (%d, now %d)", h->last_batch, batch);
   DFOT_REQUIRE(!fresh_frames || live_frames, DFOT_ERR_ARG, "forward: frozen frames must also be dead frames (live_frames is null)");
@@ -855,10 +927,15 @@
   const dfot_uvit_config& c = h->cfg;
   const int bt = batch * h->T, e = h->E;
   int rc = 0;
-  if ((rc = launch_noise_emb(noise_levels, h->ne_freqs, h->ne_phases, h->ne_w1, h->ne_b1, h->ne_w2, h->ne_b2, h->nhid,
-                             h->nemb, bt, c.noise_dim, e, s)))
-    return rc;
-  if ((rc = launch_film_vec(h->film_table, h->film_chunks, h->nemb, h->sv, bt, e, s))) return rc;
+  if (table) {
+    h->sv_cur = h->sv_steps + (size_t)step * h->sv_elems;
+  } else {
+    if ((rc = launch_noise_emb(noise_levels, h->ne_freqs, h->ne_phases, h->ne_w1, h->ne_b1, h->ne_w2, h->ne_b2, h->nhid,
+                               h->nemb, bt, c.noise_dim, e, s)))
+      return rc;
+    if ((rc = launch_film_vec(h->film_table, h->film_chunks, h->nemb, h->sv, bt, e, s))) return rc;
+    h->sv_cur = h->sv;
+  }
   if ((rc = launch_embed_input_bf16(x, h->ein_w, h->ein_b, h->XB[0], bt, c.resolution, c.in_channels, h->ch[0], s))) return rc;
   h->gn1_nblk = 0;
   for (int l = 0; l < 4; ++l) h->xin[l] = h->X[l];
@@ -898,6 +975,14 @@
   int rc = dfot_uvit_set_conditions(h, external_cond, external_cond_mask, batch, stream);
   if (rc) return rc;
   return dfot_uvit_forward_cached(h, x, noise_levels, out, batch, stream);
+}
+
+size_t dfot_uvit_sv_floats(dfot_uvit_t h) { return h ? h->sv_elems : 0; }
+int dfot_uvit_read_sv(dfot_uvit_t h, int step, float* out, size_t capacity, void* stream) {
+  DFOT_REQUIRE(h && out, DFOT_ERR_ARG, "read_sv: null argument");
+  DFOT_REQUIRE(h->sv && capacity >= h->sv_elems, DFOT_ERR_SHAPE, "read_sv: need %zu floats, got %zu", h->sv_elems, capacity);
+  DFOT_REQUIRE(step < 0 || (h->nt_state == dfot_uvit_s::NT_VALID && step < h->nt_steps), DFOT_ERR_STATE, "read_sv: no valid table step %d", step);
+  return copy_f32(out, step < 0 ? h->sv : h->sv_steps + (size_t)step * h->sv_elems, h->sv_elems, (hipStream_t)stream);
 }
 
 int dfot_uvit_read_tap(dfot_uvit_t h, const char* name, float* out, size_t capacity, void* stream) {
diff --git a/diffusion-forcing-transformer_amd/sampler.py b/diffusion-forcing-transformer_amd/sampler.py
--- a/diffusion-forcing-transformer_amd/sampler.py
+++ b/diffusion-forcing-transformer_amd/sampler.py
@@ -383,7 +383,7 @@
         skip_dead = self.skip_dead_frames and hasattr(self.model, "live_frames")
         skip_frozen = skip_dead and self.skip_frozen_frames and hasattr(self.model, "fresh_frames")
 
-        def step(p_, xs, noise, tables, gen_dev, xs_next=None, live_dev=None, fresh_dev=None):
+        def step(p_, xs, noise, tables, gen_dev, xs_next=None, live_dev=None, fresh_dev=None, noise_step=None):
             nonlocal cond_rep, cond_nfe
             nfe, bm = p_["nfe"], p_["bm"]
             x_in = torch.empty(bm, horizon, *x_shape, device="cuda", dtype=torch.float32)
@@ -421,9 +421,13 @@
                     self.model.live_frames = live_dev if live_dev is not None else p_["live_dev"]
                 if skip_frozen:
                     self.model.fresh_frames = fresh_dev if fresh_dev is not None else p_["fresh_dev"]
+                if noise_step is not None:
+                    self.model.noise_step = noise_step
                 try:
                     v = self.model(x_in, lvl, cond_rep, p_["cmask_dev"])
                 finally:
+                    if noise_step is not None:
+                        self.model.noise_step = None
                     if skip_dead:
                         self.model.live_frames = None
                     if skip_frozen:
@@ -465,15 +469,18 @@
         uniform = all(p_["bm"] == plans[0]["bm"] and p_["cmask_dev"] is plans[0]["cmask_dev"]
                       and p_["weights_dev"] is plans[0]["weights_dev"] and p_.get("cond") is plans[0].get("cond") for p_ in plans)
         hook = getattr(self, "step_hook", None)
+        use_table = (uniform and not strict and rg == 0 and not self._branch_split_active and self._noise_table_fits(len(plans), plans[0]["bm"]))
         if (self.use_graph and uniform and not strict and len(plans) > 2 and all(p_["sigma"] is None for p_ in plans) and not self._branch_split_active
                 and rg == 0 and hook is None):
             if self._static_graph_cond and cond_full is not None:
                 nfe0 = plans[0]["nfe"]
                 plans[0]["cond_src"] = cond_full if nfe0 == 1 else cond_full.repeat_interleave(nfe0, dim=0)
-            xs = self._run_steps_graph(plans, xs, draw_noise, step, flat_dev, gens_dev, horizon)
+            xs = self._run_steps_graph(plans, xs, draw_noise, step, flat_dev, gens_dev, horizon, use_table)
         else:
+            if use_table:
+                self.model.set_noise_steps(flat_dev.view(len(plans), 8, plans[0]["bm"], horizon)[:, 7])
             for i, p_ in enumerate(plans):
-                xs = step(p_, xs, draw_noise(p_), p_["tables_dev"], p_["gen_dev"])
+                xs = step(p_, xs, draw_noise(p_), p_["tables_dev"], p_["gen_dev"], noise_step=i if use_table else None)
                 if hook is not None:
                     hook(i, xs)
         self.window_forwards += sum(p_["bm"] for p_ in plans)
@@ -532,7 +539,14 @@
             prev = p_
         return out
 
-    def _run_steps_graph(self, plans, xs, draw_noise, step, flat_dev, gens_dev, horizon):
+    def _noise_table_fits(self, n_steps: int, bm: int) -> bool:
+        m = self.model
+        if not (hasattr(m, "set_noise_steps") and hasattr(m, "noise_step")):
+            return False
+        m.reserve(bm)
+        return bool(m.query("noise_table")) and n_steps <= int(m.query("noise_table_steps"))
+
+    def _run_steps_graph(self, plans, xs, draw_noise, step, flat_dev, gens_dev, horizon, use_table=False):
         p0 = plans[0]
         bm, n_steps, nfe = p0["bm"], len(plans), p0["nfe"]
         need_noise = any(p_["need_noise"] for p_ in plans)
@@ -545,7 +559,7 @@
             self._graphs_generation = gen
         cond_src = p0.get("cond_src")
         key = (bm, n_steps, nfe, horizon, tuple(xs.shape), need_noise, None if p0["cmask"] is None else p0["cmask"].tobytes(),
-               id(self.model), None if cond_src is None else (tuple(cond_src.shape), cond_src.dtype))
+               id(self.model), None if cond_src is None else (tuple(cond_src.shape), cond_src.dtype), use_table)
         ent = self._graphs.get(key)
         if ent is None:
             ent = dict(tables=torch.empty(n_steps, 8, bm, horizon, device="cuda", dtype=torch.float32),
@@ -566,12 +580,15 @@
                     ent["noise"][i].copy_(draw_noise(p_))
                 else:
                     ent["noise"][i].zero_()
+        if use_table:
+            self.model.set_noise_steps(ent["tables"][:, 7])
+        ns = (lambda i: i) if use_table else (lambda i: None)
         p_static = dict(p0, weights_dev=ent["weights"])
         if cond_src is not None:
             ent["cond"].copy_(cond_src)
             p_static["cond"] = ent["cond"]
         ent["xs"].copy_(step(p_static, xs, None if not need_noise else ent["noise"][0], ent["tables"][0], ent["gens"][0], live_dev=ent["lives"][0],
-                            fresh_dev=ent["fresh"][0]))
+                            fresh_dev=ent["fresh"][0], noise_step=ns(0)))
         if ent["graph"] is None:
             torch.cuda.synchronize()
             graph = torch.cuda.CUDAGraph()
@@ -579,7 +596,7 @@
                 x = ent["xs"]
                 for i in range(1, n_steps):
                     x = step(p_static, x, ent["noise"][i] if need_noise else None, ent["tables"][i], ent["gens"][i], live_dev=ent["lives"][i],
-                             fresh_dev=ent["fresh"][i])
+                             fresh_dev=ent["fresh"][i], noise_step=ns(i))
                 ent["out"] = x
             ent["graph"] = graph
             if len(self._graphs) >= 4:
diff --git a/include/dfot_hip.h b/include/dfot_hip.h
--- a/include/dfot_hip.h
+++ b/include/dfot_hip.h
@@ -61,6 +61,11 @@
                                   const uint8_t* live_frames, void* stream);
 int dfot_uvit_forward_cached_masks(dfot_uvit_t h, const float* x, const float* noise_levels, float* out, int batch,
                                    const uint8_t* live_frames, const uint8_t* fresh_frames, void* stream);
+int dfot_uvit_set_noise_steps(dfot_uvit_t h, const float* levels, int n_steps, int batch, void* stream);
+int dfot_uvit_forward_cached_step(dfot_uvit_t h, const float* x, const float* noise_levels, float* out, int batch,
+                                  const uint8_t* live_frames, const uint8_t* fresh_frames, int step, void* stream);
+int dfot_uvit_read_sv(dfot_uvit_t h, int step, float* out, size_t capacity_floats, void* stream);
+size_t dfot_uvit_sv_floats(dfot_uvit_t h);
 int dfot_uvit_read_tap(dfot_uvit_t h, const char* name, float* out, size_t capacity_floats, void* stream);
 
 typedef struct dfot_dit_s* dfot_dit_t;
```
